# yuxiaoxiangyong/Multilateral-Temporal-view-Pyramid-Transformer-for-Video-Inpainting-Detection

Hardware: AMD Instinct MI355X
Metric: clips/sec fwd (B=8,T=5,224x224) (higher is better)
Workload: dtype f32; 1 GPU; full Mumpy forward (3 temporal views, pyramid decoder), B=8 clips/GPU, T=5, 224x224, fp32, tubelets (5,4,1); global_batch=8, launch=hipGraph replay, fork/join over HIP streams (independent branches co-scheduled), parallelism=batch-sharded x1, one metric all-reduce

## Files before the change

include/mumpy_hip.h:

```cpp
#ifndef MUMPY_HIP_H
#define MUMPY_HIP_H

#include <stdint.h>

#ifdef __cplusplus
extern "C" {
#endif

#define MUMPY_ABI_VERSION 2

#define MUMPY_EINVAL   (-1)
#define MUMPY_EALIGN   (-2)
#define MUMPY_ENULL    (-3)
#define MUMPY_ERANGE   (-4)

#define MUMPY_ACT_NONE 0
#define MUMPY_ACT_GELU 1
#define MUMPY_MATH_BF16 0x100
#define MUMPY_MATH_BF16X3 0x200
#define MUMPY_MATH_BF16X2 0x400

int         mumpy_abi_version(void);
const char* mumpy_last_error(void);
const char* mumpy_last_route(void);
int         mumpy_tuning_build(void);

int mumpy_workspace_status(const void* workspace, int* status);

int mumpy_linear_rd_fwd(const float* x, const float* W, const float* bias, const float* residual, float* y, int64_t M, int N, int K,
                        int act, void* stream);
int mumpy_window_attention_bg_fwd(const float* qkv, float* out, const float* bias, const float* mask_tab, const int32_t* mask_id,
                                  int n_mask, int B, int Hs, int W, int C, int shift, float scale, void* stream);

int mumpy_linear_ln_tiles(int64_t M, int N, int K);
int mumpy_linear_lnx_fwd(const float* x, const float* W, const float* bias, const float* residual, float* y, int64_t M, int N, int K,
                         int act, void* workspace, int64_t workspace_bytes, float* stats_out, const float* ln_stats, int ln_gn,
                         const float* ln_colsum, float ln_eps, void* stream);

int mumpy_deform_sample_kv_fwd(const float* x2, const float* pos, const float* Wkv, const float* bkv, float* kv, int B, int Hs2,
                               int W, int C, int nq, void* stream);

int mumpy_deform_out_combine_fwd(const float* o, const float* Wout, const float* bout, const float* x1, float* out, int B, int H,
                                 int W, int C, void* stream);

int mumpy_deform_sample_kv_mm16_fwd(const float* x2, const float* pos, const float* Wkv, const float* bkv, float* kv, int B, int Hs2,
                                    int W, int C, int nq, void* stream);
int mumpy_deform_out_combine_mm16_fwd(const float* o, const float* Wout, const float* bout, const float* x1, float* out, int B,
                                      int H, int W, int C, void* stream);

int mumpy_avgpool2_pad_nhwc_fwd(const float* x, float* out, int B, int H, int W, int C, int Cpad, int nchw_in, void* stream);

int mumpy_copy_rows_fwd(const float* src, int64_t src_stride, float* dst, int64_t dst_stride, int64_t rows, int cols, void* stream);

int mumpy_merge_views_fwd(const float* v1, const float* v2, const float* v3, float* out, int B, int T, int n, int C1, int C2,
                          int C3, int t1, int t2, int t3, void* stream);

int mumpy_trunk_head_fwd(const float* g, const float* f, const float* gcn, const float* freq, float* z, int B, int h, int w, int C,
                         void* stream);

int mumpy_layernorm_fwd(const float* x, const float* gamma, const float* beta, float* y,
                        int64_t rows, int C, float eps, void* stream);

int mumpy_layernorm_bf16_fwd(const float* x, const float* gamma, const float* beta, void* y,
                             int64_t rows, int C, float eps, void* stream);

int mumpy_linear_fwd(const float* x, const float* W, const float* bias, const float* residual, float* y,
                     int64_t M, int N, int K, int act, void* stream);

int64_t mumpy_linear_workspace_bytes(int64_t M, int N, int K);
int mumpy_linear_ws_fwd(const float* x, const float* W, const float* bias, const float* residual, float* y,
                        int64_t M, int N, int K, int act, void* workspace, int64_t workspace_bytes, void* stream);

int mumpy_linear_wsz_fwd(const float* x, const float* W, const float* bias, const float* residual, float* y,
                         int64_t M, int N, int K, int act, void* workspace, int64_t workspace_bytes, void* stream);

int mumpy_linear_bf16s_fwd(const void* x, const void* W, const float* bias, const float* residual, void* y,
                           int64_t M, int N, int K, int act, int out_bf16, void* stream);

int mumpy_linear_rows_fwd(const float* x, int64_t rows_per_block, int64_t block_stride, const float* W,
                          const float* bias, const float* residual, float* y, int64_t M, int N, int K, int act,
                          void* workspace, int64_t workspace_bytes, void* stream);

int mumpy_linear_rows_kseg_fwd(const float* x, int64_t rows_per_block, int64_t block_stride, int kseg, int kstride, const float* W,
                               const float* bias, const float* residual, float* y, int64_t M, int N, int K, int act,
                               void* workspace, int64_t workspace_bytes, void* stream);

int64_t mumpy_conv2d_workspace_bytes(int B, int H, int W, int Cin, int Cout, int kh, int kw);
int mumpy_conv2d_nhwc_fwd(const float* x, const float* w_krsc, const float* bias, const float* residual, float* y,
                          int B, int H, int W, int Cin, int Cout, int kh, int kw, int act, void* workspace,
                          int64_t workspace_bytes, void* stream);

int mumpy_window_attention_fwd(const float* qkv, float* out, const float* bias, const float* mask_tab,
                               const int32_t* mask_id, int n_mask, int B, int Hs, int W, int C, int shift,
                               float scale, void* stream);

int mumpy_window_attention_bf16_fwd(const void* qkv, void* out, const float* bias, const float* mask_tab,
                                    const int32_t* mask_id, int n_mask, int B, int Hs, int W, int C, int shift,
                                    float scale, void* stream);

int mumpy_window_attention_bf16mm_fwd(const void* qkv, void* out, const float* bias, const float* mask_tab,
                                      const int32_t* mask_id, int n_mask, int B, int Hs, int W, int C, int shift,
                                      float scale, void* stream);

int mumpy_window_attention_mm16_fwd(const float* qkv, float* out, const float* bias, const float* mask_tab,
                                    const int32_t* mask_id, int n_mask, int B, int Hs, int W, int C, int shift,
                                    float scale, void* stream);


int mumpy_deform_offsets_fwd(const float* q, const float* dw_w, const float* dw_b, const float* ln_g,
                             const float* ln_b, const float* pw_w, float* pos, int B, int H, int W, int C,
                             void* stream);

int mumpy_deform_sample_fwd(const float* x2, const float* pos, float* out, int B, int Hs2, int W, int C,
                            int nq, void* stream);

int mumpy_deform_attention_fwd(const float* q, const float* kv, const float* padmask, float* out, int B, int H,
                               int W, int C, int r, float scale, void* stream);

int mumpy_deform_attention_mm16_fwd(const float* q, const float* kv, const float* padmask, float* out, int B, int H,
                                    int W, int C, int r, float scale, void* stream);

int mumpy_deform_combine_fwd(const float* x1, const float* Yt, float* out, int B, int H, int W, int C,
                             void* stream);

int mumpy_faf_fwd(const float* x, const float* D, const float* Dt, float* scratch, float* out, int B, int T,
                  int frame, int lo_hi, int mid_lo, int mid_hi, void* stream);

int mumpy_patch_embed_fwd(const float* x, const float* Wt, const float* bias, const float* gamma,
                          const float* beta, float* out, int B, int T, int H, int W, int t, int C,
                          float eps, void* stream);

int mumpy_patch_merge_ln_fwd(const float* x, const float* gamma, const float* beta, float* out, int B, int Hs,
                             int W, int C, float eps, void* stream);

int mumpy_temporal_attention_fwd(const float* qkv, float* out, int64_t S, int T, int C, int heads,
                                 float scale, void* stream);
int mumpy_temporal_attention_q_fwd(const float* qkv, float* out, int64_t S, int T, int Tq, int C, int heads, float scale, void* stream);

int mumpy_attention_probs_fwd(const float* q, const float* k, float* out, int64_t outer, int heads, int nq, int nk, int d,
                              int64_t q_outer_stride, int64_t q_row_stride, int64_t k_outer_stride, int64_t k_row_stride,
                              int64_t q_mod, float scale, void* stream);

int mumpy_gn_stats_nhwc_fwd(const float* x, float* partial, int B, int64_t HW, int C, int G, int nsplit,
                            void* stream);

int mumpy_gn_apply_resample_nhwc_fwd(const float* x, const float* partial, int nsplit, const float* gamma,
                                     const float* beta, int G, float eps, int act, int mean4, int scale,
                                     int align_corners, int ep_mode, const float* ep_a, const float* ep_b,
                                     float* out, int out_ctot, int out_coff, int B, int H, int W, int C,
                                     void* stream);

int mumpy_final_conv_fwd(const float* x, const float* w_krsc, const float* bias, float* logits, uint8_t* mask, int B,
                         int H, int W, int C, float thr, void* stream);

int64_t mumpy_final_conv_bwd_workspace_bytes(int B, int H, int W);
int mumpy_final_conv_bwd(const float* x, const float* w_krsc, const float* dy, float* dx, float* dw, float* db, void* workspace,
                         int64_t workspace_bytes, int B, int H, int W, int C, void* stream);

int mumpy_sigmoid_threshold_fwd(const float* logits, uint8_t* mask, int64_t n, float thr, void* stream);

int mumpy_normalize_u8_fwd(const uint8_t* frames, float* out, int64_t nframes, int H, int W, const float* mean3,
                           const float* std3, void* stream);

int mumpy_resize_nearest_table(int src, int dst, int32_t* table_host);
int mumpy_resize_normalize_u8_fwd(const uint8_t* frames, float* out, const int32_t* ytab, const int32_t* xtab,
                                  int64_t nframes, int Hs, int Ws, int H, int W, const float* mean3, const float* std3,
                                  void* stream);

int mumpy_add_fwd(const float* a, const float* b, float* out, int64_t n, void* stream);

int64_t mumpy_mask_loss_workspace_bytes(int B, int64_t P);
int mumpy_mask_loss_fwd_bwd(const float* logits, const float* target, float* dlogits, float* loss3, void* workspace,
                            int64_t workspace_bytes, int B, int64_t P, float eps, float loss_scale, void* stream);

int mumpy_adamw_step(float* param, const float* grad, float* exp_avg, float* exp_avg_sq, int64_t n, double lr,
                     double beta1, double beta2, double eps, double weight_decay, int step, double grad_scale,
                     void* stream);

int mumpy_adamw_hyper(float* out8_host, double lr, double beta1, double beta2, double eps, double weight_decay, int step,
                      double grad_scale);
int mumpy_adamw_step_dev(float* param, const float* grad, float* exp_avg, float* exp_avg_sq, int64_t n,
                         const float* hyper_dev, void* stream);

int mumpy_sgd_step(float* param, const float* grad, float* momentum_buf, int64_t n, double lr, double momentum,
                   double dampening, double weight_decay, int nesterov, double grad_scale, void* stream);
int mumpy_sgd_hyper(float* out4_host, double lr, double momentum, double dampening, double weight_decay, int nesterov,
                    double grad_scale);
int mumpy_sgd_step_dev(float* param, const float* grad, float* momentum_buf, int64_t n, const float* hyper_dev, int nesterov,
                       void* stream);

int mumpy_rmsprop_step(float* param, const float* grad, float* square_avg, float* momentum_buf, int64_t n, double lr,
                       double alpha, double eps, double weight_decay, double momentum, double grad_scale, void* stream);
int mumpy_rmsprop_hyper(float* out8_host, double lr, double alpha, double eps, double weight_decay, double momentum,
                        double grad_scale);
int mumpy_rmsprop_step_dev(float* param, const float* grad, float* square_avg, float* momentum_buf, int64_t n,
                           const float* hyper_dev, void* stream);

int64_t mumpy_layernorm_bwd_workspace_bytes(int64_t rows, int C);
int mumpy_layernorm_bwd(const float* x, const float* gamma, const float* dy, const float* dx_add, float* dx, float* dgamma,
                        float* dbeta, void* workspace, int64_t workspace_bytes, int64_t rows, int C, float eps, int accumulate,
                        void* stream);

int mumpy_gelu_fwd(const float* x, float* y, int64_t n, void* stream);
int mumpy_gelu_bwd(const float* x, const float* dy, float* dx, int64_t n, void* stream);

int mumpy_transpose_fwd(const float* in, float* out, int64_t R, int64_t C, void* stream);

int64_t mumpy_col_sum_workspace_bytes(int64_t R, int C);
int mumpy_col_sum_fwd(const float* x, float* out, void* workspace, int64_t workspace_bytes, int64_t R, int C, void* stream);

int64_t mumpy_linear_bwd_workspace_bytes(int64_t M, int N, int K);
int mumpy_linear_bwd(const float* x, const float* W, const float* dy, float* dx, float* dW, float* db, int64_t M, int N, int K,
                     int accumulate, void* workspace, int64_t workspace_bytes, void* stream);

int mumpy_patch_gather_fwd(const float* in, float* out, int64_t B, int H, int W, int C, int inverse, void* stream);

int mumpy_conv_weight_dgrad_fwd(const float* w_krsc, float* out, int Cout, int Cin, int kh, int kw, void* stream);

int64_t mumpy_conv2d_wgrad_workspace_bytes(int B, int H, int W, int Cin, int Cout, int kh, int kw);
int mumpy_conv2d_wgrad_nhwc(const float* x, const float* dy, float* dW, int B, int H, int W, int Cin, int Cout, int kh, int kw,
                            int accumulate, void* workspace, int64_t workspace_bytes, void* stream);

int64_t mumpy_window_attention_bwd_workspace_bytes(int B, int Hs, int W, int C);
int mumpy_window_attention_bwd(const float* qkv, const float* dout, const float* bias, const float* mask_tab,
                               const int32_t* mask_id, int n_mask, const int32_t* rel_index, float* dqkv, float* dtable,
                               void* workspace, int64_t workspace_bytes, int B, int Hs, int W, int C, int shift, float scale,
                               int accumulate, void* stream);
int mumpy_window_attention_bwd_csr(const float* qkv, const float* dout, const float* bias, const float* mask_tab,
                                   const int32_t* mask_id, int n_mask, const int32_t* rel_index, const int32_t* rel_csr, float* dqkv,
                                   float* dtable, void* workspace, int64_t workspace_bytes, int B, int Hs, int W, int C, int shift,
                                   float scale, int accumulate, void* stream);
int64_t mumpy_window_attention_mm16_bwd_workspace_bytes(int B, int Hs, int W, int C);
int mumpy_window_attention_mm16_bwd(const float* qkv, const float* dout, const float* bias, const float* mask_tab,
                                    const int32_t* mask_id, int n_mask, const int32_t* rel_index, const int32_t* rel_csr, float* dqkv,
                                    float* dtable, void* workspace, int64_t workspace_bytes, int B, int Hs, int W, int C, int shift,
                                    float scale, int accumulate, void* stream);

int mumpy_relpos_bias_expand_fwd(const float* table, const int32_t* rel_index, float* out, int nH, void* stream);

#define MUMPY_GN_ACCUMULATE 0x100
int64_t mumpy_gn_bwd_workspace_bytes(int B, int64_t HW, int C);
int mumpy_gn_bwd_nhwc(const float* z, const float* stats_partial, int nsplit_stats, const float* gamma, const float* beta,
                      const float* dy, float* dz, float* dgamma, float* dbeta, void* workspace, int64_t workspace_bytes,
                      int B, int64_t HW, int C, int G, float eps, int relu, void* stream);

int mumpy_temporal_attention_bwd(const float* qkv, const float* dout, float* dqkv, int64_t S, int T, int C, int heads,
                                 float scale, void* stream);

int mumpy_scale_samples_fwd(const float* x, const float* scale, float* out, int B, int64_t per_sample, void* stream);

int mumpy_upsample_bwd_nhwc(const float* dy, float* dx, int B, int H, int W, int C, int scale, int align_corners, void* stream);

int mumpy_dwconv5_window_fwd(const float* x, const float* w, const float* b, float* u, int64_t N, int C, void* stream);
int64_t mumpy_dwconv5_window_bwd_workspace_bytes(int64_t N, int C);
int mumpy_dwconv5_window_bwd(const float* x, const float* w, const float* du, float* dx, float* dw, float* db,
                             void* workspace, int64_t workspace_bytes, int64_t N, int C, void* stream);

int64_t mumpy_deform_attention_bwd_workspace_bytes(int64_t B2w, int C);
int mumpy_deform_attention_bwd(const float* q, const float* kv, const float* dout, float* dq_part, float* dkv, void* workspace,
                               int64_t workspace_bytes, int64_t B1w, int r, int C, float scale, void* stream);

int mumpy_deform_sample_bwd(const float* x2, const float* pos, const float* dsampled, float* dx2, float* dpos_part,
                            int64_t B2, int C, int nq, void* stream);

#ifdef __cplusplus
}
#endif
#endif
```

multilateral-temporal-view-pyramid-transformer-for-video-inpainting-detection_amd/csrc/abi.cpp:

```cpp
#include <stdarg.h>
#include <stdio.h>
#include "common.h"

namespace mumpy {
static thread_local char g_err[512] = "";
void set_error(const char* fmt, ...) {
    va_list ap;
    va_start(ap, fmt);
    vsnprintf(g_err, sizeof(g_err), fmt, ap);
    va_end(ap);
}
thread_local Route g_route;
static thread_local char g_route_text[160] = "";
static const char* format_route() {
    static const char* const addr[] = {"dense", "rows", "kseg", "conv"};
    static const char* const ln[] = {"none", "producer", "consumer"};
    static const char* const red[] = {"none", "one", "two-in-one", "taps"};
    const Route& r = g_route;
    char* t = g_route_text;
    const size_t n = sizeof(g_route_text);
    switch (r.family) {
    case Route::TILED: snprintf(t, n, "tiled tile=%d ks=%d np=%d addr=%s", r.tile, r.ks, r.np, addr[r.addr & 3]); break;
    case Route::TILED16: snprintf(t, n, "tiled16 tile=%d ks=%d np=%d addr=%s", r.tile, r.ks, r.np, addr[r.addr & 3]); break;
    case Route::WS:
        snprintf(t, n, "ws sched=%s P=%d ln=%s addr=%s", r.split ? "split" : "whole", r.passes, ln[r.ln < 3 ? r.ln : 0], addr[r.addr & 3]);
        break;
    case Route::WS64: snprintf(t, n, "ws64 P=%d addr=dense", r.passes); break;
    case Route::WS16: snprintf(t, n, "ws16 P=%d addr=dense", r.passes); break;
    case Route::XGEMM: {
        char dx[24] = "-", dw[24] = "-";
        if (r.prod[0].wt) snprintf(dx, sizeof(dx), "%dx%d", r.prod[0].wt, r.prod[0].ks);
        if (r.prod[1].wt) snprintf(dw, sizeof(dw), "%dx%d", r.prod[1].wt, r.prod[1].ks);
        snprintf(t, n, "xgemm np=%d addr=%s dx=%s dw=%s reduce=%s", r.np, addr[r.addr & 3], dx, dw, red[r.reduce & 3]);
        break;
    }
    default: snprintf(t, n, "none");
    }
    return t;
}
#ifdef MUMPY_TUNING
#include <stdlib.h>
int tune_int(const char* name, int dflt) {
    const char* v = getenv(name);
    return v ? atoi(v) : dflt;
}
const char* tune_str(const char* name) { return getenv(name); }
#endif
}

extern "C" int mumpy_tuning_build(void) {
#ifdef MUMPY_TUNING
    return 1;
#else
    return 0;
#endif
}

extern "C" int mumpy_abi_version(void) { return MUMPY_ABI_VERSION; }
extern "C" const char* mumpy_last_error(void) { return mumpy::g_err; }
extern "C" const char* mumpy_last_route(void) { return mumpy::format_route(); }
```

multilateral-temporal-view-pyramid-transformer-for-video-inpainting-detection_amd/csrc/common.h:

```cpp
#pragma once
#include <hip/hip_runtime.h>
#include <stdint.h>
#include <stdio.h>
#include "../../include/mumpy_hip.h"

namespace mumpy {

typedef float f32x4 __attribute__((ext_vector_type(4)));
typedef float f32x16 __attribute__((ext_vector_type(16)));

constexpr int WAVE = 64;
constexpr int WS = 7;
constexpr int WT = 49;
constexpr int HD = 32;

void set_error(const char* fmt, ...);

#ifdef MUMPY_TUNING
int tune_int(const char* name, int dflt);
const char* tune_str(const char* name);
#else
inline int tune_int(const char*, int dflt) { return dflt; }
inline const char* tune_str(const char*) { return nullptr; }
#endif

struct Route {
    enum Family : uint8_t { NONE, TILED, TILED16, WS, WS64, WS16, XGEMM };
    enum Addr : uint8_t { DENSE, ROWS, KSEG, CONV };
    enum Reduce : uint8_t { R_NONE, R_ONE, R_TWO_IN_ONE, R_TAPS };
    uint8_t family = NONE;
    uint8_t tile = 0;
    uint8_t np = 0;
    uint8_t addr = DENSE;
    uint8_t split = 0;
    uint8_t passes = 0;
    uint8_t ln = 0;
    uint8_t reduce = R_NONE;
    int ks = 1;
    struct { int wt, ks; } prod[2] = {{0, 0}, {0, 0}};
};
extern thread_local Route g_route;

inline hipStream_t as_stream(void* s) { return reinterpret_cast<hipStream_t>(s); }
inline bool aligned16(const void* p) { return (reinterpret_cast<uintptr_t>(p) & 15u) == 0; }

#define MUMPY_CHECK_LAUNCH(name)                                                     \
    do {                                                                             \
        hipError_t e_ = hipGetLastError();                                           \
        if (e_ != hipSuccess) {                                                      \
            mumpy::set_error("%s: launch failed: %s", name, hipGetErrorString(e_));  \
            return (int)e_;                                                          \
        }                                                                            \
    } while (0)

#define MUMPY_REQUIRE(cond, code, ...)                                               \
    do {                                                                             \
        if (!(cond)) {                                                               \
            mumpy::set_error(__VA_ARGS__);                                           \
            return code;                                                             \
        }                                                                            \
    } while (0)

__device__ __forceinline__ unsigned xcd_major_id(unsigned orig, unsigned nwg) {
    const unsigned xcd = orig & 7, q8 = nwg >> 3, r8 = nwg & 7;
    return (xcd < r8 ? xcd * (q8 + 1) : r8 * (q8 + 1) + (xcd - r8) * q8) + (orig >> 3);
}

template <int CTRL>
__device__ __forceinline__ float dpp_f(float v) {
    return __builtin_bit_cast(float, __builtin_amdgcn_update_dpp(0, __builtin_bit_cast(int, v), CTRL, 0xF, 0xF, true));
}
__device__ __forceinline__ float swz_xor16(float v) {
    return __builtin_bit_cast(float, __builtin_amdgcn_ds_swizzle(__builtin_bit_cast(int, v), (16 << 10) | 0x1f));
}

__device__ __forceinline__ float wave_sum(float v, int width) {
    if (width > 1) v += dpp_f<0xB1>(v);
    if (width > 2) v += dpp_f<0x4E>(v);
    if (width > 4) v += dpp_f<0x141>(v);
    if (width > 8) v += dpp_f<0x140>(v);
    if (width > 16) v += swz_xor16(v);
    if (width > 32) v += __shfl_xor(v, 32);
    return v;
}

template <typename T>
__device__ __forceinline__ T ordered_sum(T first, const T* __restrict__ p, int64_t stride, int n_more) {
    T s = first;
    int z = 0;
    for (; z + 8 <= n_more; z += 8) {
        T v[8];
#pragma unroll
        for (int u = 0; u < 8; ++u) v[u] = p[(int64_t)(z + u) * stride];
#pragma unroll
        for (int u = 0; u < 8; ++u) s += v[u];
    }
    for (; z < n_more; ++z) s += p[(int64_t)z * stride];
    return s;
}

__device__ __forceinline__ void gn_block_stats(const float* __restrict__ stats, int nsplit, int G, int b, int64_t HW, int cg, float eps,
                                               float* gm, float* gr, double (*red)[2]) {
    const int tid = threadIdx.x, nslice = 256 / G, g = tid % G, k = tid / G;
    const int64_t per = (HW + nsplit - 1) / nsplit;
    const float* base = stats + (int64_t)b * nsplit * G * 2 + g * 2;
    const double piv = (double)base[0] / (double)((per < HW ? per : HW) * cg);
    double s = 0.0, q = 0.0;
    if (k < nslice)
        for (int sp = k; sp < nsplit; sp += nslice) {
            const int64_t p0 = sp * per, cnt = ((p0 + per < HW) ? p0 + per : HW) - p0;
            if (cnt <= 0) continue;
            const float* o = base + (int64_t)sp * G * 2;
            const double ni = (double)(cnt * cg), dm = (double)o[0] / ni - piv;
            s += ni * dm; q += (double)o[1] + ni * dm * dm;
        }
    red[tid][0] = s; red[tid][1] = q;
    __syncthreads();
    if (tid < G) {
        double ss = 0.0, qq = 0.0;
        for (int j = 0; j < nslice; ++j) { ss += red[j * G + tid][0]; qq += red[j * G + tid][1]; }
        const double n = (double)HW * (double)cg, dm = ss / n;
        double var = qq / n - dm * dm;
        if (var < 0.0) var = 0.0;
        gm[tid] = (float)(piv + dm);
        gr[tid] = (float)(1.0 / sqrt(var + (double)eps));
    }
    __syncthreads();
}

__device__ __forceinline__ float erf_fast(float x) {
    const float ax = fabsf(x);
    const float t = __builtin_amdgcn_rcpf(fmaf(0.3275911f, ax, 1.0f));
    float p = fmaf(1.061405429f, t, -1.453152027f);
    p = fmaf(p, t, 1.421413741f);
    p = fmaf(p, t, -0.284496736f);
    p = fmaf(p, t, 0.254829592f);
    const float y = 1.0f - p * t * __expf(-ax * ax);
    return copysignf(y, x);
}

__device__ __forceinline__ float gelu_erf(float x) { return 0.5f * x * (1.0f + erf_fast(x * 0.70710678118654752440f)); }

__device__ __forceinline__ int window_token(int wy, int wx, int p, int Hs, int W, int shift) {
    int py = p / WS, px = p - py * WS;
    int y = wy * WS + py + shift;
    int x = wx * WS + px + shift;
    if (y >= Hs) y -= Hs;
    if (x >= W) x -= W;
    return y * W + x;
}

}
```

multilateral-temporal-view-pyramid-transformer-for-video-inpainting-detection_amd/csrc/gemm.hip:

```cpp
#include <stdlib.h>
#include <type_traits>
#include "common.h"
#include "gemm_ws.h"
#include "gemm_ws64.h"
using namespace mumpy;

namespace {

constexpr int BK = 32;
constexpr int LDR = 36;

struct ConvGeom {
    int H, W, Cin, kh, kw, ph, pw;
    int kseg, kstride;
};

__device__ __attribute__((aligned(128))) float g_zero_page[32];

template <int BM, int BN>
__device__ __forceinline__ void tile_of_block(int64_t M, unsigned gn, int ksplit, unsigned& tm, unsigned& tn, int& ks) {
    constexpr unsigned NG = (BN >= 128) ? 4 : 8;
    unsigned wgid = xcd_major_id(blockIdx.x, gridDim.x);
    ks = (int)(wgid % (unsigned)ksplit);
    wgid /= (unsigned)ksplit;
    const unsigned gm = (unsigned)((M + BM - 1) / BM);
    const unsigned full = (gn / NG) * NG;
    if (wgid < gm * full) {
        const unsigned grp = wgid / (gm * NG), rem = wgid - grp * gm * NG;
        tm = rem / NG;
        tn = grp * NG + rem % NG;
    } else {
        const unsigned wdt = gn - full, rem = wgid - gm * full;
        tm = rem / wdt;
        tn = full + rem % wdt;
    }
}

struct ConvTap {
    int dy, dx, off;
    __device__ __forceinline__ bool inside(const ConvGeom& cg, int yx) const {
        const int yy = (yx >> 16) + dy, xx = (yx & 0xffff) + dx;
        return (unsigned)yy < (unsigned)cg.H && (unsigned)xx < (unsigned)cg.W;
    }
};
__device__ __forceinline__ ConvTap conv_tap(const ConvGeom& cg, int k0) {
    const int tap = k0 / cg.Cin, c0 = k0 - tap * cg.Cin;
    const int dy = tap / cg.kw - cg.ph, dx = tap % cg.kw - cg.pw;
    return {dy, dx, (dy * cg.W + dx) * cg.Cin + c0};
}

template <int TM, int TN, int WM, int WN, bool OUT16 = false>
__device__ __forceinline__ void store_tile(const f32x16 (&acc)[TM][TN], int64_t m0, int n0, int wm, int wn, int c, int h,
                                           int64_t M, int N, const float* __restrict__ bias, const float* residual,
                                           float* Y, int act, int ksplit, int ks, float* slab) {
    const int wm_u = __builtin_amdgcn_readfirstlane(wm), wn_u = __builtin_amdgcn_readfirstlane(wn);
    const int64_t mw = m0 + wm_u * WM;
    const int64_t wbase = mw * N + n0 + wn_u * WN;
    const int rows_left = (int)((M - mw) < (int64_t)WM ? (M - mw) : (int64_t)WM);
    const uint32_t nb = 4u * (uint32_t)N;
    const uint32_t lane_off = 4u * h * nb + 4u * c;
    if (ksplit > 1) {
        char* S = reinterpret_cast<char*>(slab + (int64_t)ks * M * N + wbase);
#pragma unroll
        for (int j = 0; j < TN; ++j) {
            if (n0 + wn_u * WN + 32 * j + c >= N) continue;
#pragma unroll
            for (int i = 0; i < TM; ++i)
#pragma unroll
                for (int r = 0; r < 16; ++r) {
                    const int row = 32 * i + (r & 3) + 8 * (r >> 2);
                    if (row + 4 * h < rows_left) *reinterpret_cast<float*>(S + ((uint32_t)row * nb + lane_off + 128u * j)) = acc[i][j][r];
                }
        }
        return;
    }
    char* Yw = OUT16 ? reinterpret_cast<char*>(reinterpret_cast<__bf16*>(Y) + wbase) : reinterpret_cast<char*>(Y + wbase);
    const char* Rw = residual ? reinterpret_cast<const char*>(residual + wbase) : nullptr;
#pragma unroll
    for (int j = 0; j < TN; ++j) {
        const int n = n0 + wn_u * WN + 32 * j + c;
        if (n >= N) continue;
        const float bv = bias ? bias[n] : 0.f;
#pragma unroll
        for (int i = 0; i < TM; ++i)
#pragma unroll
            for (int r = 0; r < 16; ++r) {
                const int row = 32 * i + (r & 3) + 8 * (r >> 2);
                if (row + 4 * h >= rows_left) continue;
                const uint32_t off = (uint32_t)row * nb + lane_off + 128u * j;
                float v = acc[i][j][r] + bv;
                if (act == MUMPY_ACT_GELU) v = gelu_erf(v);
                if (Rw) v += *reinterpret_cast<const float*>(Rw + off);
                if (OUT16) *reinterpret_cast<__bf16*>(Yw + (off >> 1)) = (__bf16)v;
                else *reinterpret_cast<float*>(Yw + off) = v;
            }
    }
}

template <int BM, int BN, int WM, int WN, bool CONV, bool GLDS, bool PIPE = true>
__global__ __launch_bounds__(64 * (BM / WM) * (BN / WN), (BM * BN > 64 * 64) ? 2 : (CONV ? 3 : 4)) void linear_kernel(const float* __restrict__ X, const float* __restrict__ Wt,
                                                     const float* __restrict__ bias, const float* residual,
                                                     float* Y, int64_t M, int N, int K, int act, unsigned gn,
                                                     int ksplit, float* slab, int64_t rpb, int64_t bstride, ConvGeom cg) {
    constexpr int TM = WM / 32, TN = WN / 32;
    constexpr int WAVES_N = BN / WN;
    constexpr int NT = 64 * (BM / WM) * (BN / WN);
    constexpr int RPI = NT / 8;
    constexpr int A_LD = BM / RPI;
    constexpr int B_LD = BN / RPI;
    static_assert(BM % RPI == 0 && BN % RPI == 0, "tile rows must divide over the staging passes");
    constexpr int LD = GLDS ? 32 : LDR;
    __shared__ __attribute__((aligned(1024))) float lds[2][(BM + BN) * LD];

    const int tid = threadIdx.x, lane = tid & 63, wave = tid >> 6;
    const int c = lane & 31, h = lane >> 5;
    const int wm = wave / WAVES_N, wn = wave % WAVES_N;
    unsigned tm, tn;
    int ks;
    tile_of_block<BM, BN>(M, gn, ksplit, tm, tn, ks);
    const int64_t m0 = (int64_t)tm * BM;
    const int n0 = (int)tn * BN;
    const int kbeg = ks * (K / ksplit);

    const int ld_row = tid >> 3, ld_c4 = tid & 7;
    f32x4 areg[A_LD], breg[B_LD];

    const float* arow[A_LD];
    const float* brow[B_LD];
    int ayx[A_LD];
#pragma unroll
    for (int i = 0; i < A_LD; ++i) {
        int64_t m = m0 + ld_row + RPI * i;
        if (m > M - 1) m = M - 1;
        if (CONV) {
            const unsigned mu = (unsigned)m, qx = mu / (unsigned)cg.W;
            const int x = (int)(mu - qx * (unsigned)cg.W);
            const int y = (int)(qx % (unsigned)cg.H);
            ayx[i] = (y << 16) | x;
            arow[i] = X + m * cg.Cin + 4 * ld_c4;
        } else {
            ayx[i] = 0;
            if (rpb >= M && !cg.kseg) arow[i] = X + m * K + 4 * ld_c4;
            else {
                const unsigned mu = (unsigned)m, blk = mu / (unsigned)rpb;
                arow[i] = X + (int64_t)blk * bstride + (int64_t)(mu - blk * (unsigned)rpb) * (cg.kseg ? cg.kseg : K) + 4 * ld_c4;
            }
        }
    }
#pragma unroll
    for (int i = 0; i < B_LD; ++i) {
        int n = n0 + ld_row + RPI * i;
        if (n > N - 1) n = N - 1;
        brow[i] = Wt + (int64_t)n * K + 4 * ld_c4;
    }
    int asw[A_LD], bsw[B_LD];
#pragma unroll
    for (int i = 0; i < A_LD; ++i) asw[i] = 4 * ((ld_c4 ^ (((ld_row + RPI * i) >> 1) & 7)) - ld_c4);
#pragma unroll
    for (int i = 0; i < B_LD; ++i) bsw[i] = 4 * ((ld_c4 ^ (((ld_row + RPI * i) >> 1) & 7)) - ld_c4);
    typedef __attribute__((address_space(1))) const void* gptr_t;
    typedef __attribute__((address_space(3))) void* lptr_t;
    auto gdma = [&](int k0, int buf) {
        const int wave_row = (tid >> 6) * 8;
        if (CONV) {
            const int tap = k0 / cg.Cin, c0 = k0 - tap * cg.Cin;
            const int dy = tap / cg.kw - cg.ph, dx = tap % cg.kw - cg.pw;
            const int off = (dy * cg.W + dx) * cg.Cin + c0;
#pragma unroll
            for (int i = 0; i < A_LD; ++i) {
                const int yy = (ayx[i] >> 16) + dy, xx = (ayx[i] & 0xffff) + dx;
                const bool ok = (unsigned)yy < (unsigned)cg.H && (unsigned)xx < (unsigned)cg.W;
                const float* src = ok ? arow[i] + off + asw[i] : g_zero_page + 4 * ld_c4;
                __builtin_amdgcn_global_load_lds((gptr_t)src, (lptr_t)&lds[buf][(wave_row + RPI * i) * LD], 16, 0, 0);
            }
        } else {
            const int ka = cg.kseg ? (k0 / cg.kseg) * cg.kstride + k0 % cg.kseg : k0;
#pragma unroll
            for (int i = 0; i < A_LD; ++i)
                __builtin_amdgcn_global_load_lds((gptr_t)(arow[i] + ka + asw[i]), (lptr_t)&lds[buf][(wave_row + RPI * i) * LD], 16, 0, 0);
        }
#pragma unroll
        for (int i = 0; i < B_LD; ++i)
            __builtin_amdgcn_global_load_lds((gptr_t)(brow[i] + k0 + bsw[i]), (lptr_t)&lds[buf][(BM + wave_row + RPI * i) * LD], 16, 0, 0);
    };
    auto gload = [&](int k0) {
        if (CONV) {
            const ConvTap t = conv_tap(cg, k0);
#pragma unroll
            for (int i = 0; i < A_LD; ++i) {
                const bool ok = t.inside(cg, ayx[i]);
                const f32x4 v = *reinterpret_cast<const f32x4*>(arow[i] + (ok ? t.off : 0));
                areg[i] = ok ? v : f32x4{0, 0, 0, 0};
            }
        } else {
            const int ka = cg.kseg ? (k0 / cg.kseg) * cg.kstride + k0 % cg.kseg : k0;
#pragma unroll
            for (int i = 0; i < A_LD; ++i) areg[i] = *reinterpret_cast<const f32x4*>(arow[i] + ka);
        }
#pragma unroll
        for (int i = 0; i < B_LD; ++i) breg[i] = *reinterpret_cast<const f32x4*>(brow[i] + k0);
    };
    auto lstore = [&](int buf) {
#pragma unroll
        for (int i = 0; i < A_LD; ++i)
            *reinterpret_cast<f32x4*>(&lds[buf][(ld_row + RPI * i) * LD + 4 * ld_c4]) = areg[i];
#pragma unroll
        for (int i = 0; i < B_LD; ++i)
            *reinterpret_cast<f32x4*>(&lds[buf][(BM + ld_row + RPI * i) * LD + 4 * ld_c4]) = breg[i];
    };
    auto fread = [&](int buf, f32x4 (&af)[TM][4], f32x4 (&bf)[TN][4]) {
#pragma unroll
        for (int i = 0; i < TM; ++i) {
            const int R = wm * WM + 32 * i + c;
#pragma unroll
            for (int q = 0; q < 4; ++q) {
                const int col = GLDS ? 4 * ((4 * h + q) ^ ((R >> 1) & 7)) : 16 * h + 4 * q;
                af[i][q] = *reinterpret_cast<const f32x4*>(&lds[buf][R * LD + col]);
            }
        }
#pragma unroll
        for (int j = 0; j < TN; ++j) {
            const int R = wn * WN + 32 * j + c;
#pragma unroll
            for (int q = 0; q < 4; ++q) {
                const int col = GLDS ? 4 * ((4 * h + q) ^ ((R >> 1) & 7)) : 16 * h + 4 * q;
                bf[j][q] = *reinterpret_cast<const f32x4*>(&lds[buf][(BM + R) * LD + col]);
            }
        }
    };

    f32x16 acc[TM][TN];
#pragma unroll
    for (int i = 0; i < TM; ++i)
#pragma unroll
        for (int j = 0; j < TN; ++j)
#pragma unroll
            for (int r = 0; r < 16; ++r) acc[i][j][r] = 0.f;
    auto mma = [&](const f32x4 (&af)[TM][4], const f32x4 (&bf)[TN][4]) {
#pragma unroll
        for (int s = 0; s < 16; ++s)
#pragma unroll
            for (int i = 0; i < TM; ++i)
#pragma unroll
                for (int j = 0; j < TN; ++j)
                    acc[i][j] = __builtin_amdgcn_mfma_f32_32x32x2f32(af[i][s >> 2][s & 3], bf[j][s >> 2][s & 3], acc[i][j], 0, 0, 0);
    };

    const int nk = K / ksplit / BK;
    f32x4 afA[TM][4], bfA[TN][4];
    if (GLDS && !PIPE) {
        gdma(kbeg, 0);
        if (nk > 1) gdma(kbeg + BK, 1);
        for (int kc = 0; kc < nk; ++kc) {
            __syncthreads();
            fread(kc & 1, afA, bfA);
            __syncthreads();
            if (kc + 2 < nk) gdma(kbeg + (kc + 2) * BK, kc & 1);
            mma(afA, bfA);
        }
    } else if (GLDS) {
        f32x4 afB[TM][4], bfB[TN][4];
        gdma(kbeg, 0);
        if (nk > 1) gdma(kbeg + BK, 1);
        __syncthreads();
        fread(0, afA, bfA);
        __syncthreads();
        if (nk > 2) gdma(kbeg + 2 * BK, 0);
        int kc = 0;
        for (; kc + 1 < nk; kc += 2) {
            fread(1, afB, bfB);
            mma(afA, bfA);
            __syncthreads();
            if (kc + 3 < nk) gdma(kbeg + (kc + 3) * BK, 1);
            if (kc + 2 < nk) fread(0, afA, bfA);
            mma(afB, bfB);
            __syncthreads();
            if (kc + 4 < nk) gdma(kbeg + (kc + 4) * BK, 0);
        }
        if (kc < nk) mma(afA, bfA);
    } else {
    f32x4 afB[TM][4], bfB[TN][4];
    gload(kbeg);
    lstore(0);
    if (nk > 1) gload(kbeg + BK);
    __syncthreads();
    fread(0, afA, bfA);
    if (nk > 1) lstore(1);
    if (nk > 2) gload(kbeg + 2 * BK);
    __syncthreads();
    int kc = 0;
    for (; kc + 1 < nk; kc += 2) {
        fread(1, afB, bfB);
        mma(afA, bfA);
        if (kc + 2 < nk) lstore(0);
        if (kc + 3 < nk) gload(kbeg + (kc + 3) * BK);
        __syncthreads();
        if (kc + 2 < nk) fread(0, afA, bfA);
        mma(afB, bfB);
        if (kc + 3 < nk) lstore(1);
        if (kc + 4 < nk) gload(kbeg + (kc + 4) * BK);
        __syncthreads();
    }
    if (kc < nk) mma(afA, bfA);
    }
    store_tile<TM, TN, WM, WN>(acc, m0, n0, wm, wn, c, h, M, N, bias, residual, Y, act, ksplit, ks, slab);
}

typedef __bf16 bf16x8 __attribute__((ext_vector_type(8)));
typedef __bf16 bf16x2 __attribute__((ext_vector_type(2)));
typedef float f32x2 __attribute__((ext_vector_type(2)));
constexpr int LDH = 20;

template <int BM, int BN, int WM, int WN, bool CONV, int NP = 1, int NBUF = 2, bool IN16 = false, bool OUT16 = false>
__global__ __launch_bounds__(256, 2) void linear_bf16_kernel(const float* __restrict__ X, const float* __restrict__ Wt,
                                                            const float* __restrict__ bias, const float* residual,
                                                            float* Y, int64_t M, int N, int K, int act, unsigned gn,
                                                            int ksplit, float* slab, int64_t rpb, int64_t bstride,
                                                            ConvGeom cg) {
    constexpr int TM = WM / 32, TN = WN / 32;
    constexpr int WAVES_N = BN / WN;
    static_assert((BM / WM) * (BN / WN) == 4, "4 waves per block");
    constexpr int RPI = 32, A_LD = BM / RPI, B_LD = BN / RPI;
    constexpr int PL = (BM + BN) * LDH;
    static_assert(NBUF * NP * PL * 4 <= 65536, "LDS tile exceeds the static limit");
    __shared__ __attribute__((aligned(16))) uint32_t lds[NBUF][NP * PL];
    const int tid = threadIdx.x, lane = tid & 63, wave = tid >> 6;
    const int c = lane & 31, h = lane >> 5;
    const int wm = wave / WAVES_N, wn = wave % WAVES_N;
    unsigned tm, tn;
    int ks;
    tile_of_block<BM, BN>(M, gn, ksplit, tm, tn, ks);
    const int64_t m0 = (int64_t)tm * BM;
    const int n0 = (int)tn * BN;
    const int kbeg = ks * (K / ksplit);
    const int ld_row = tid >> 3, ld_c4 = tid & 7;
    static_assert(!(IN16 || OUT16) || (NP == 1 && !CONV), "bf16 storage: plain bf16 products on dense operands only");
    f32x4 areg[A_LD], breg[B_LD];
    uint2 areg16[IN16 ? A_LD : 1], breg16[IN16 ? B_LD : 1];
    const float* arow[A_LD];
    const float* brow[B_LD];
    int ayx[A_LD];
#pragma unroll
    for (int i = 0; i < A_LD; ++i) {
        int64_t m = m0 + ld_row + RPI * i;
        if (m > M - 1) m = M - 1;
        if (IN16) {
            ayx[i] = 0;
            arow[i] = reinterpret_cast<const float*>(reinterpret_cast<const __bf16*>(X) + m * K + 4 * ld_c4);
            continue;
        }
        if (CONV) {
            const unsigned mu = (unsigned)m, qx = mu / (unsigned)cg.W;
            ayx[i] = ((int)(qx % (unsigned)cg.H) << 16) | (int)(mu - qx * (unsigned)cg.W);
            arow[i] = X + m * cg.Cin + 4 * ld_c4;
        } else {
            ayx[i] = 0;
            if (rpb >= M && !cg.kseg) arow[i] = X + m * K + 4 * ld_c4;
            else {
                const unsigned mu = (unsigned)m, blk = mu / (unsigned)rpb;
                arow[i] = X + (int64_t)blk * bstride + (int64_t)(mu - blk * (unsigned)rpb) * (cg.kseg ? cg.kseg : K) + 4 * ld_c4;
            }
        }
    }
#pragma unroll
    for (int i = 0; i < B_LD; ++i) {
        int n = n0 + ld_row + RPI * i;
        if (n > N - 1) n = N - 1;
        if (IN16) brow[i] = reinterpret_cast<const float*>(reinterpret_cast<const __bf16*>(Wt) + (int64_t)n * K + 4 * ld_c4);
        else brow[i] = Wt + (int64_t)n * K + 4 * ld_c4;
    }
    auto gload = [&](int k0) {
        if (IN16) {
#pragma unroll
            for (int i = 0; i < A_LD; ++i) areg16[i] = *reinterpret_cast<const uint2*>(reinterpret_cast<const __bf16*>(arow[i]) + k0);
#pragma unroll
            for (int i = 0; i < B_LD; ++i) breg16[i] = *reinterpret_cast<const uint2*>(reinterpret_cast<const __bf16*>(brow[i]) + k0);
            return;
        }
        if (CONV) {
            const ConvTap t = conv_tap(cg, k0);
#pragma unroll
            for (int i = 0; i < A_LD; ++i) {
                const bool ok = t.inside(cg, ayx[i]);
                const f32x4 v = *reinterpret_cast<const f32x4*>(arow[i] + (ok ? t.off : 0));
                areg[i] = ok ? v : f32x4{0, 0, 0, 0};
            }
        } else {
            const int ka = cg.kseg ? (k0 / cg.kseg) * cg.kstride + k0 % cg.kseg : k0;
#pragma unroll
            for (int i = 0; i < A_LD; ++i) areg[i] = *reinterpret_cast<const f32x4*>(arow[i] + ka);
        }
#pragma unroll
        for (int i = 0; i < B_LD; ++i) breg[i] = *reinterpret_cast<const f32x4*>(brow[i] + k0);
    };
    auto lstore_row = [&](uint32_t* dst, f32x4 r) {
#pragma unroll
        for (int p = 0; p < NP; ++p) {
            const bf16x2 lo = __builtin_convertvector(f32x2{r.x, r.y}, bf16x2), hi = __builtin_convertvector(f32x2{r.z, r.w}, bf16x2);
            const uint2 u = {*reinterpret_cast<const uint32_t*>(&lo), *reinterpret_cast<const uint32_t*>(&hi)};
            *reinterpret_cast<uint2*>(dst + p * PL) = u;
            if (p + 1 < NP)
                r -= f32x4{__uint_as_float(u.x << 16), __uint_as_float(u.x & 0xffff0000u), __uint_as_float(u.y << 16),
                           __uint_as_float(u.y & 0xffff0000u)};
        }
    };
    auto lstore = [&](int buf) {
        if (IN16) {
#pragma unroll
            for (int i = 0; i < A_LD; ++i) *reinterpret_cast<uint2*>(&lds[buf][(ld_row + RPI * i) * LDH + 2 * ld_c4]) = areg16[i];
#pragma unroll
            for (int i = 0; i < B_LD; ++i) *reinterpret_cast<uint2*>(&lds[buf][(BM + ld_row + RPI * i) * LDH + 2 * ld_c4]) = breg16[i];
            return;
        }
#pragma unroll
        for (int i = 0; i < A_LD; ++i) lstore_row(&lds[buf][(ld_row + RPI * i) * LDH + 2 * ld_c4], areg[i]);
#pragma unroll
        for (int i = 0; i < B_LD; ++i) lstore_row(&lds[buf][(BM + ld_row + RPI * i) * LDH + 2 * ld_c4], breg[i]);
    };
    f32x16 acc[TM][TN];
#pragma unroll
    for (int i = 0; i < TM; ++i)
#pragma unroll
        for (int j = 0; j < TN; ++j)
#pragma unroll
            for (int r = 0; r < 16; ++r) acc[i][j][r] = 0.f;
    constexpr int NPROD = (NP == 3) ? 6 : (NP == 2) ? 3 : 1;
    constexpr int PA[6] = {NP == 3 ? 2 : 1, 0, NP == 3 ? 1 : 0, 1, 0, 0}, PB[6] = {0, NP == 3 ? 2 : 1, NP == 3 ? 1 : 0, 0, 1, 0};
    const int nk = K / ksplit / BK;
    bf16x8 af[TM][2][NP], bf[TN][2][NP];
    auto fread = [&](int buf) {
#pragma unroll
        for (int i = 0; i < TM; ++i)
#pragma unroll
            for (int st = 0; st < 2; ++st)
#pragma unroll
                for (int p = 0; p < NP; ++p)
                    af[i][st][p] = *reinterpret_cast<const bf16x8*>(&lds[buf][p * PL + (wm * WM + 32 * i + c) * LDH + 8 * st + 4 * h]);
#pragma unroll
        for (int j = 0; j < TN; ++j)
#pragma unroll
            for (int st = 0; st < 2; ++st)
#pragma unroll
                for (int p = 0; p < NP; ++p)
                    bf[j][st][p] = *reinterpret_cast<const bf16x8*>(&lds[buf][p * PL + (BM + wn * WN + 32 * j + c) * LDH + 8 * st + 4 * h]);
    };
    auto mma = [&]() {
#pragma unroll
        for (int st = 0; st < 2; ++st)
#pragma unroll
            for (int q = 0; q < NPROD; ++q)
#pragma unroll
                for (int i = 0; i < TM; ++i)
#pragma unroll
                    for (int j = 0; j < TN; ++j)
                        acc[i][j] = __builtin_amdgcn_mfma_f32_32x32x16_bf16(af[i][st][NP > 1 ? PA[q] : 0],
                                                                            bf[j][st][NP > 1 ? PB[q] : 0], acc[i][j], 0, 0, 0);
    };
    const int klast = kbeg + (nk - 1) * BK;
    if (NBUF == 2) {
        gload(kbeg);
        lstore(0);
        __syncthreads();
        for (int kc = 0; kc + 1 < nk; ++kc) {
            gload(kbeg + (kc + 1) * BK);
            __builtin_amdgcn_sched_barrier(0);
            fread(kc & 1);
            mma();
            lstore((kc & 1) ^ 1);
            __syncthreads();
        }
        fread((nk - 1) & 1);
        mma();
    } else {
        gload(kbeg);
        lstore(0);
        gload(nk > 1 ? kbeg + BK : kbeg);
        __syncthreads();
        for (int kc = 0; kc + 1 < nk; ++kc) {
            fread(0);
            __syncthreads();
            lstore(0);
            const int knext = kbeg + (kc + 2) * BK;
            gload(knext < klast ? knext : klast);
            mma();
            __syncthreads();
        }
        fread(0);
        mma();
    }
    store_tile<TM, TN, WM, WN, OUT16>(acc, m0, n0, wm, wn, c, h, M, N, bias, residual, Y, act, ksplit, ks, slab);
}

__global__ __launch_bounds__(256) void splitk_reduce_kernel(const float* __restrict__ slab, const float* __restrict__ bias,
                                                            const float* residual, float* Y, int64_t MN4, int N,
                                                            int ksplit, int act) {
    for (int64_t i = (int64_t)blockIdx.x * 256 + threadIdx.x; i < MN4; i += (int64_t)gridDim.x * 256) {
        f32x4 v = ordered_sum(reinterpret_cast<const f32x4*>(slab)[i], reinterpret_cast<const f32x4*>(slab) + MN4 + i, MN4, ksplit - 1);
        const int n = (int)((i * 4) % N);
        if (bias) v += *reinterpret_cast<const f32x4*>(bias + n);
        if (act == MUMPY_ACT_GELU) {
#pragma unroll
            for (int e = 0; e < 4; ++e) v[e] = gelu_erf(v[e]);
        }
        if (residual) v += reinterpret_cast<const f32x4*>(residual)[i];
        reinterpret_cast<f32x4*>(Y)[i] = v;
    }
}

struct Plan {
    int tile;
    int ksplit;
    unsigned gn;
    int64_t gm;
};

constexpr int NUM_CU = 256;

int fit_ksplit(int K, int want, int min_slice, int max_ks) {
    int ks = want;
    if (ks > K / min_slice) ks = K / min_slice;
    if (ks > max_ks) ks = max_ks;
    while (ks > 1 && (K % (32 * ks)) != 0) --ks;
    return ks < 1 ? 1 : ks;
}

Plan make_plan_x3(int64_t M, int N, int K, bool allow_split) {
    Plan p;
    const int64_t gm128 = (M + 127) / 128, gm64 = (M + 63) / 64;
    const unsigned gn128 = (N + 127) / 128, gn64 = (N + 63) / 64;
    const int64_t b128 = gm128 * gn128, b64 = gm64 * gn64;
    auto fit = [&](int want) { return allow_split ? fit_ksplit(K, want, 384, 16) : 1; };
    const int ksw = fit((int)((448 + b128 / 2) / b128));
    if (b128 * ksw >= 240) {
        p.tile = 0; p.ksplit = ksw; p.gm = gm128; p.gn = gn128;
    } else {
        p.tile = 2; p.ksplit = (b64 < 2 * 256 && K >= 768) ? fit((int)((3 * 256 + b64 - 1) / b64)) : 1;
        p.gm = gm64; p.gn = gn64;
    }
    return p;
}

Plan make_plan(int64_t M, int N, int K, bool allow_split, bool x3 = false) {
    static const char* force = tune_str("MUMPY_GEMM_FORCE");
    if (x3 && !force) return make_plan_x3(M, N, K, allow_split);
    Plan p;
    const int64_t gm128 = (M + 127) / 128, gm64 = (M + 63) / 64;
    const unsigned gn128 = (N + 127) / 128, gn64 = (N + 63) / 64;
    const int64_t b128 = gm128 * gn128, b64 = gm64 * gn64;
    const double nk = (double)K / BK;
    const double t128 = (double)((b128 + NUM_CU - 1) / NUM_CU) * (nk + 2.0) / nk;
    double t64 = (double)((b64 + NUM_CU - 1) / NUM_CU) * 0.272;
    if (t64 < 0.357) t64 = 0.357;
    t64 *= (nk + 0.5) / nk;
    int tile = (t128 <= t64) ? 0 : 2;
    if (tile == 0 && b128 > NUM_CU && K >= 512) tile = 3;
    int ks = 1;
    static const int min_slice = tune_int("MUMPY_GEMM_MINSLICE", 384), max_ks = tune_int("MUMPY_GEMM_MAXKS", 16),
                     min_k = tune_int("MUMPY_GEMM_SPLIT_MINK", 768);
    if (tile == 2 && allow_split && b64 < 2 * NUM_CU && K >= min_k) ks = fit_ksplit(K, (int)((3 * NUM_CU + b64 - 1) / b64), min_slice, max_ks);
    if (force) {
        int ft = -1, fk = -1;
        if (sscanf(force, "%d,%d", &ft, &fk) >= 1 && ft >= 0 && ft <= 3) {
            tile = ft;
            if (fk >= 1 && allow_split && K % (32 * fk) == 0) ks = fk; else if (fk >= 1) ks = 1;
        }
    }
    p.tile = tile; p.ksplit = ks;
    p.gm = (tile == 0 || tile == 3) ? gm128 : gm64;
    p.gn = (tile == 2) ? gn64 : gn128;
    return p;
}

int device_cus() {
    static int num_cu = 0;
    if (!num_cu) {
        int dev = 0;
        hipDeviceProp_t prop;
        if (hipGetDevice(&dev) == hipSuccess && hipGetDeviceProperties(&prop, dev) == hipSuccess) num_cu = prop.multiProcessorCount;
        else num_cu = NUM_CU;
    }
    return num_cu;
}

int ws_plan(int64_t M, int N, int K, bool have_ws, bool conv) {
    static const int ws_mode = tune_int("MUMPY_GEMM_WS", 2);
    const int num_cu = device_cus();
    const int64_t tiles = ((M + 127) / 128) * ((N + 127) / 128);
    const int nk = K / 32;
    const double rounds = (double)tiles / num_cu, eff = rounds / (double)((tiles + num_cu - 1) / num_cu);
    const double per_cu = (double)tiles * nk / num_cu;
    int how = 0;
    if (ws_mode == 1) how = 1;
    else if (ws_mode == 3) how = have_ws ? 2 : 1;
    else if (ws_mode == 2 && conv) {
        if (have_ws && eff < 0.86 && per_cu >= 24.0 && (double)nk / per_cu <= 3.0) how = 2;
        else if (tiles >= (int64_t)(0.75 * num_cu) && eff >= 0.75 && K >= 128) how = 1;
    } else if (ws_mode == 2) {
        if (tiles >= (int64_t)(0.75 * num_cu) && eff >= 0.86 && K >= 128 && !(K >= 1024 && rounds >= 1.8)) how = 1;
        else if (have_ws && eff < 0.86 && per_cu >= 24.0 && (double)nk / per_cu <= 3.0 && !(K >= 1024 && rounds >= 1.8)) how = 2;
    }
    return how;
}

struct LinearArgs {
    const float *x, *W, *bias, *residual;
    float* y;
    int64_t M;
    int N, K, act;
    hipStream_t s;
    float* ws = nullptr;
    int64_t ws_bytes = 0;
    bool ws_clean = false;
    int64_t rpb = 0, bstride = 0;
    int kseg = 0, kstride = 0;
    const ConvGeom* conv = nullptr;
    const gemm_ws::LnArgs* ln = nullptr;
};

struct TiledArgs {
    const float *x, *W, *bias, *residual;
    float* y;
    int64_t M;
    int N, K, act;
    unsigned gn;
    int ksplit;
    float* slab;
    int64_t rpb, bstride;
    ConvGeom cg;
    int64_t grid;
    hipStream_t s;
};

template <class Kern>
void launch_tiled(Kern kern, unsigned threads, const TiledArgs& t) {
    hipLaunchKernelGGL(kern, dim3((unsigned)t.grid), dim3(threads), 0, t.s, t.x, t.W, t.bias, t.residual, t.y, t.M, t.N, t.K, t.act,
                       t.gn, t.ksplit, t.slab, t.rpb, t.bstride, t.cg);
}

template <class F>
void with_bool(bool b, F&& f) {
    if (b) f(std::true_type{});
    else f(std::false_type{});
}

void launch_tiled_fp32(int tile, bool conv, bool glds, const TiledArgs& t) {
    with_bool(conv, [&](auto cv) {
        constexpr bool CV = decltype(cv)::value;
        if (tile == 3) return launch_tiled(linear_kernel<128, 128, 64, 64, CV, true, false>, 256, t);
        with_bool(glds, [&](auto gl) {
            constexpr bool GL = decltype(gl)::value;
            if (tile == 0) launch_tiled(linear_kernel<128, 128, 64, 32, CV, GL>, 512, t);
            else if (tile == 1) launch_tiled(linear_kernel<64, 128, 32, 64, CV, GL>, 256, t);
            else launch_tiled(linear_kernel<64, 64, 32, 32, CV, GL>, 256, t);
        });
    });
}

template <int NP, bool IN16 = false>
void launch_tiled_bf16(bool wide, bool flag, const TiledArgs& t) {
    with_bool(wide, [&](auto wd) {
        with_bool(flag, [&](auto fl) {
            constexpr int T = decltype(wd)::value ? 128 : 64, NBUF = (T == 128 && NP > 1) ? 1 : 2;
            constexpr bool FL = decltype(fl)::value;
            launch_tiled(linear_bf16_kernel<T, T, T / 2, T / 2, !IN16 && FL, NP, NBUF, IN16, IN16 && FL>, 256, t);
        });
    });
}

int launch_linear(const LinearArgs& a) {
    const int64_t M = a.M, rpb = a.rpb > 0 ? a.rpb : M, bstride = a.rpb > 0 ? a.bstride : 0;
    const int N = a.N, K = a.K, act = a.act & 0xff;
    const ConvGeom* conv = a.conv;
    ConvGeom cg = conv ? *conv : ConvGeom{0, 0, 0, 0, 0, 0, 0, 0, 0};
    cg.kseg = a.kseg; cg.kstride = a.kstride;
    const bool math_bf16 = (a.act & MUMPY_MATH_BF16) != 0;
    const bool math_x2 = (a.act & MUMPY_MATH_BF16X2) != 0;
    const bool math_x3 = (a.act & MUMPY_MATH_BF16X3) != 0 || math_x2;
    float* ws = a.ws;
    int64_t ws_bytes = a.ws_bytes;
    const gemm_ws::Conv cvd{cg.H, cg.W, cg.Cin, cg.kh, cg.kw};
    if (a.ln && (rpb < M || math_bf16 || math_x3 || conv || !gemm_ws::eligible(M, N, K) ||
                 !ws_plan(M, N, K, ws && ws_bytes >= gemm_ws::workspace_bytes(device_cus()), false))) {
        set_error("linear: LayerNorm folding needs a shape the persistent 128x128 kernel takes (mumpy_linear_ln_tiles) in fp32 mode");
        return MUMPY_EINVAL;
    }
    if (rpb >= M && !a.kseg && !math_bf16 && !math_x3 && (conv ? gemm_ws::conv_eligible(M, N, cvd) : gemm_ws::eligible(M, N, K))) {
        const int num_cu = device_cus();
        const bool have_ws = ws && ws_bytes >= gemm_ws::workspace_bytes(num_cu);
        const int how = ws_plan(M, N, K, have_ws, conv != nullptr);
        const int nk = K / 32;
        static const int ws64_mode = tune_int("MUMPY_GEMM_WS64", 1);
        if (!how && !conv && ws64_mode) {
            const int64_t t64 = ((M + 63) / 64) * ((N + 63) / 64);
            const double r64 = (double)t64 / (2.0 * num_cu);
            const bool fits = ws64_mode == 2 || (act != MUMPY_ACT_GELU && nk <= 32 && t64 >= 64 && (r64 <= 1.0 || r64 >= 2.5 || nk <= 12));
            if (fits) {
                if (int rc = gemm_ws64::launch(a.x, a.W, a.bias, a.residual, a.y, M, N, K, act, num_cu, a.s)) return rc;
                MUMPY_CHECK_LAUNCH("linear(ws64)");
                return 0;
            }
        }
        if (how) {
            if (int rc = gemm_ws::launch(a.x, a.W, a.bias, a.residual, a.y, M, N, K, act, num_cu, a.s, ws, ws_bytes, how == 2 ? 1 : 0, nullptr,
                                         a.ws_clean, conv ? &cvd : nullptr, a.ln)) return rc;
            MUMPY_CHECK_LAUNCH("linear(ws)");
            return 0;
        }
    }
    Plan p = make_plan(M, N, K, ws != nullptr, math_x3);
    if (ws) { ws += 1024; ws_bytes -= 4096; }
    if (p.ksplit > 1 && (int64_t)p.ksplit * M * N * (int64_t)sizeof(float) > ws_bytes) p.ksplit = 1;
    if (math_bf16 || math_x3) {
        if (p.tile == 3) p.tile = 0;
        if (p.tile == 1) { p.tile = 2; p.gn = (unsigned)((N + 63) / 64); }
    }
    const int64_t grid = p.gm * p.gn * p.ksplit;
    MUMPY_REQUIRE(grid < (1ll << 31), MUMPY_ERANGE, "linear: too many tiles");
    static const bool use_glds = tune_int("MUMPY_GEMM_GLDS", 0) != 0;
    const bool wide = (p.tile == 0 || p.tile == 3);
    const TiledArgs t{a.x, a.W, a.bias, a.residual, a.y, M, N, K, act, p.gn, p.ksplit, ws, rpb, bstride, cg, grid, a.s};
    g_route = Route{};
    g_route.family = Route::TILED; g_route.tile = (uint8_t)p.tile; g_route.ks = p.ksplit;
    g_route.np = math_x2 ? 2 : math_x3 ? 3 : math_bf16 ? 1 : 0;
    g_route.addr = conv ? Route::CONV : a.kseg ? Route::KSEG : rpb < M ? Route::ROWS : Route::DENSE;
    if (math_x2) launch_tiled_bf16<2>(wide, conv != nullptr, t);
    else if (math_x3) launch_tiled_bf16<3>(wide, conv != nullptr, t);
    else if (math_bf16) launch_tiled_bf16<1>(wide, conv != nullptr, t);
    else launch_tiled_fp32(p.tile, conv != nullptr, use_glds, t);
    MUMPY_CHECK_LAUNCH("linear");
    if (p.ksplit > 1) {
        const int64_t mn4 = M * N / 4;
        int64_t g = (mn4 + 255) / 256;
        if (g > 2048) g = 2048;
        hipLaunchKernelGGL(splitk_reduce_kernel, dim3((unsigned)g), dim3(256), 0, a.s, ws, a.bias, a.residual, a.y, mn4, N,
                           p.ksplit, act);
        MUMPY_CHECK_LAUNCH("linear(split-K reduce)");
    }
    return 0;
}

}

static int check_linear_args(const char* who, const void* x, const void* W, const float* residual, const void* y, int64_t M, int N,
                             int K, int act) {
    MUMPY_REQUIRE(x && W && y, MUMPY_ENULL, "%s: null pointer", who);
    MUMPY_REQUIRE(aligned16(x) && aligned16(W) && aligned16(y) && aligned16(residual), MUMPY_EALIGN,
                  "%s: pointers must be 16-byte aligned", who);
    MUMPY_REQUIRE(M < (1ll << 31) - 256 && (int64_t)N * 4 * 128 < (1ll << 32), MUMPY_ERANGE,
                  "%s: M=%lld rows / N=%d columns beyond the 32-bit row index / tile byte offsets", who, (long long)M, N);
    MUMPY_REQUIRE(M >= 0 && N > 0 && K > 0 && K % BK == 0 && N % 32 == 0, MUMPY_EINVAL,
                  "%s: need K %% 32 == 0 and N %% 32 == 0 (got M=%lld N=%d K=%d)", who, (long long)M, N, K);
    MUMPY_REQUIRE((act & 0xff) == MUMPY_ACT_NONE || (act & 0xff) == MUMPY_ACT_GELU, MUMPY_EINVAL, "%s: unknown act %d", who, act);
    constexpr int math_bits = MUMPY_MATH_BF16 | MUMPY_MATH_BF16X3 | MUMPY_MATH_BF16X2;
    MUMPY_REQUIRE((act & ~(0xff | math_bits)) == 0, MUMPY_EINVAL, "%s: unknown flag bits in act 0x%x", who, act);
    MUMPY_REQUIRE(((act & math_bits) & ((act & math_bits) - 1)) == 0, MUMPY_EINVAL, "%s: the MUMPY_MATH_* modes are exclusive", who);
    return 0;
}

static LinearArgs linear_args(const float* x, const float* W, const float* bias, const float* residual, float* y, int64_t M, int N,
                              int K, int act, void* workspace, int64_t workspace_bytes, void* stream) {
    LinearArgs a{x, W, bias, residual, y, M, N, K, act, as_stream(stream)};
    a.ws = static_cast<float*>(workspace);
    a.ws_bytes = workspace ? workspace_bytes : 0;
    return a;
}

extern "C" int mumpy_linear_fwd(const float* x, const float* W, const float* bias, const float* residual, float* y,
                                int64_t M, int N, int K, int act, void* stream) {
    if (M == 0) return 0;
    if (int rc = check_linear_args("linear", x, W, residual, y, M, N, K, act)) return rc;
    return launch_linear(linear_args(x, W, bias, residual, y, M, N, K, act, nullptr, 0, stream));
}

extern "C" int64_t mumpy_linear_workspace_bytes(int64_t M, int N, int K) {
    if (M <= 0 || N <= 0 || K <= 0 || K % BK) return 0;
    const Plan p = make_plan(M, N, K, true), q = make_plan(M, N, K, true, true);
    const int ks = p.ksplit > q.ksplit ? p.ksplit : q.ksplit;
    int64_t bytes = ks > 1 ? (int64_t)ks * M * N * (int64_t)sizeof(float) + 4096 : 0;
    if (gemm_ws::eligible(M, N, K)) {
        const int64_t tiles = ((M + 127) / 128) * ((N + 127) / 128);
        const double per_cu = (double)tiles * (K / 32) / NUM_CU;
        const int64_t need = gemm_ws::workspace_bytes(2 * NUM_CU);
        if (per_cu >= 16.0 && bytes < need) bytes = need;
    }
    return bytes;
}

extern "C" int mumpy_linear_ws_fwd(const float* x, const float* W, const float* bias, const float* residual, float* y,
                                   int64_t M, int N, int K, int act, void* workspace, int64_t workspace_bytes,
                                   void* stream) {
    if (M == 0) return 0;
    if (int rc = check_linear_args("linear", x, W, residual, y, M, N, K, act)) return rc;
    MUMPY_REQUIRE(aligned16(workspace), MUMPY_EALIGN, "linear: workspace must be 16-byte aligned");
    return launch_linear(linear_args(x, W, bias, residual, y, M, N, K, act, workspace, workspace_bytes, stream));
}

extern "C" int mumpy_linear_bf16s_fwd(const void* x, const void* W, const float* bias, const float* residual, void* y,
                                      int64_t M, int N, int K, int act, int out_bf16, void* stream) {
    if (M == 0) return 0;
    if (int rc = check_linear_args("linear_bf16s", x, W, residual, y, M, N, K, act)) return rc;
    MUMPY_REQUIRE((act & ~0xff) == 0, MUMPY_EINVAL, "linear_bf16s: unknown act %d", act);
    MUMPY_REQUIRE(!(out_bf16 && residual), MUMPY_EINVAL, "linear_bf16s: a bf16 output takes no residual");
    hipStream_t s = as_stream(stream);
    static const int ws16 = tune_int("MUMPY_GEMM_WS16", 2);
    const int64_t gm128 = (M + 127) / 128, gm64 = (M + 63) / 64;
    const unsigned gn128 = (N + 127) / 128, gn64 = (N + 63) / 64;
    if (ws16 && gemm_ws::eligible16(M, N, K)) {
        const int num_cu = device_cus();
        const int64_t tiles = gm128 * gn128;
        const double rounds = (double)tiles / num_cu, eff = rounds / (double)((tiles + num_cu - 1) / num_cu);
        if (ws16 == 2 || (tiles >= (int64_t)(0.75 * num_cu) && eff >= 0.75)) {
            if (int rc = gemm_ws::launch16(x, W, bias, residual, y, M, N, K, act, out_bf16 != 0, num_cu, s)) return rc;
            MUMPY_CHECK_LAUNCH("linear_bf16s(ws)");
            return 0;
        }
    }
    const bool wide = gm128 * gn128 >= 200;
    const unsigned gn = wide ? gn128 : gn64;
    const int64_t grid = (wide ? gm128 : gm64) * gn;
    MUMPY_REQUIRE(grid < (1ll << 31), MUMPY_ERANGE, "linear_bf16s: too many tiles");
    const TiledArgs t{static_cast<const float*>(x), static_cast<const float*>(W), bias, residual, static_cast<float*>(y), M, N, K, act,
                      gn, 1, nullptr, M, 0, ConvGeom{0, 0, 0, 0, 0, 0, 0, 0, 0}, grid, s};
    g_route = Route{};
    g_route.family = Route::TILED16; g_route.tile = wide ? 0 : 2; g_route.np = 1;
    launch_tiled_bf16<1, true>(wide, out_bf16 != 0, t);
    MUMPY_CHECK_LAUNCH("linear_bf16s");
    return 0;
}

extern "C" int mumpy_linear_wsz_fwd(const float* x, const float* W, const float* bias, const float* residual, float* y,
                                    int64_t M, int N, int K, int act, void* workspace, int64_t workspace_bytes,
                                    void* stream) {
    if (M == 0) return 0;
    if (int rc = check_linear_args("linear", x, W, residual, y, M, N, K, act)) return rc;
    MUMPY_REQUIRE(aligned16(workspace), MUMPY_EALIGN, "linear: workspace must be 16-byte aligned");
    LinearArgs a = linear_args(x, W, bias, residual, y, M, N, K, act, workspace, workspace_bytes, stream);
    a.ws_clean = true;
    return launch_linear(a);
}

extern "C" int mumpy_workspace_status(const void* workspace, int* status) {
    MUMPY_REQUIRE(workspace && status, MUMPY_ENULL, "workspace_status: null pointer");
    unsigned w[2] = {0, 0};
    static_assert(gemm_ws::LN_GUARD_WORD + 1 == gemm_ws::STATUS_WORD, "status words must be adjacent");
    hipError_t e = hipMemcpy(w, static_cast<const unsigned*>(workspace) + gemm_ws::LN_GUARD_WORD, sizeof(w), hipMemcpyDeviceToHost);
    if (e != hipSuccess) { set_error("workspace_status: %s", hipGetErrorString(e)); return (int)e; }
    *status = w[1] ? (int)w[1] : (w[0] ? -1 : 0);
    return 0;
}

extern "C" int mumpy_linear_ln_tiles(int64_t M, int N, int K) {
    if (M <= 0 || N <= 0 || K <= 0 || K % BK || N % 32 || !gemm_ws::eligible(M, N, K)) return 0;
    return ws_plan(M, N, K, true, false) ? (N + 127) / 128 : 0;
}

extern "C" int mumpy_linear_lnx_fwd(const float* x, const float* W, const float* bias, const float* residual, float* y, int64_t M,
                                    int N, int K, int act, void* workspace, int64_t workspace_bytes, float* stats_out,
                                    const float* ln_stats, int ln_gn, const float* ln_colsum, float ln_eps, void* stream) {
    if (M == 0) return 0;
    if (int rc = check_linear_args("linear", x, W, residual, y, M, N, K, act)) return rc;
    MUMPY_REQUIRE((act & ~0xff) == 0, MUMPY_EINVAL, "linear_lnx: fp32 matrix math only");
    MUMPY_REQUIRE(aligned16(workspace) && workspace, MUMPY_EALIGN, "linear_lnx: needs the kept (zeroed) workspace of mumpy_linear_wsz_fwd");
    MUMPY_REQUIRE((stats_out != nullptr) != (ln_stats != nullptr), MUMPY_EINVAL, "linear_lnx: exactly one of stats_out (producer) / ln_stats (consumer)");
    MUMPY_REQUIRE(!ln_stats || (ln_colsum && bias && !residual && ln_gn == (K + 127) / 128 && ln_gn <= 16 && ln_eps > 0.f), MUMPY_EINVAL,
                  "linear_lnx: the consumer takes W gamma, colsum, bias = W beta + b, no residual, and ln_gn = ceil(K / 128) tiles (got %d)", ln_gn);
    MUMPY_REQUIRE(aligned16(stats_out) && aligned16(ln_stats) && aligned16(ln_colsum), MUMPY_EALIGN, "linear_lnx: pointers must be 16-byte aligned");
    MUMPY_REQUIRE(M * (int64_t)((N + 127) / 128) * 8 < (1ll << 31) && M * (int64_t)(ln_gn > 0 ? ln_gn : 1) * 8 < (1ll << 31), MUMPY_ERANGE,
                  "linear_lnx: statistics buffer beyond 2 GiB");
    const gemm_ws::LnArgs ln{stats_out, ln_stats, ln_colsum, ln_gn, K, ln_eps};
    LinearArgs a = linear_args(x, W, bias, residual, y, M, N, K, act, workspace, workspace_bytes, stream);
    a.ws_clean = true;
    a.ln = &ln;
    return launch_linear(a);
}

extern "C" int mumpy_linear_rows_fwd(const float* x, int64_t rows_per_block, int64_t block_stride, const float* W,
                                     const float* bias, const float* residual, float* y, int64_t M, int N, int K, int act,
                                     void* workspace, int64_t workspace_bytes, void* stream) {
    if (M == 0) return 0;
    if (int rc = check_linear_args("linear", x, W, residual, y, M, N, K, act)) return rc;
    MUMPY_REQUIRE(rows_per_block > 0 && M % rows_per_block == 0 && block_stride % 4 == 0, MUMPY_EINVAL,
                  "linear_rows: M=%lld must be a multiple of rows_per_block=%lld and block_stride %% 4 == 0",
                  (long long)M, (long long)rows_per_block);
    LinearArgs a = linear_args(x, W, bias, residual, y, M, N, K, act, workspace, workspace_bytes, stream);
    a.rpb = rows_per_block; a.bstride = block_stride;
    return launch_linear(a);
}

extern "C" int mumpy_linear_rows_kseg_fwd(const float* x, int64_t rows_per_block, int64_t block_stride, int kseg, int kstride,
                                          const float* W, const float* bias, const float* residual, float* y, int64_t M, int N, int K,
                                          int act, void* workspace, int64_t workspace_bytes, void* stream) {
    if (M == 0) return 0;
    if (int rc = check_linear_args("linear", x, W, residual, y, M, N, K, act)) return rc;
    MUMPY_REQUIRE(rows_per_block > 0 && M % rows_per_block == 0 && block_stride % 4 == 0, MUMPY_EINVAL,
                  "linear_rows_kseg: M=%lld must be a multiple of rows_per_block=%lld and block_stride %% 4 == 0",
                  (long long)M, (long long)rows_per_block);
    MUMPY_REQUIRE(kseg > 0 && kseg % 32 == 0 && K % kseg == 0 && kstride % 4 == 0 && kstride >= 0, MUMPY_EINVAL,
                  "linear_rows_kseg: need kseg %% 32 == 0, K %% kseg == 0, kstride %% 4 == 0 (got kseg=%d K=%d kstride=%d)", kseg, K, kstride);
    LinearArgs a = linear_args(x, W, bias, residual, y, M, N, K, act, workspace, workspace_bytes, stream);
    a.rpb = rows_per_block; a.bstride = block_stride;
    a.kseg = kseg; a.kstride = kstride;
    return launch_linear(a);
}

extern "C" int64_t mumpy_conv2d_workspace_bytes(int B, int H, int W, int Cin, int Cout, int kh, int kw) {
    return mumpy_linear_workspace_bytes((int64_t)B * H * W, Cout, kh * kw * Cin);
}

extern "C" int mumpy_conv2d_nhwc_fwd(const float* x, const float* w_krsc, const float* bias, const float* residual,
                                     float* y, int B, int H, int W, int Cin, int Cout, int kh, int kw, int act,
                                     void* workspace, int64_t workspace_bytes, void* stream) {
    MUMPY_REQUIRE(B > 0 && H > 0 && W > 0 && H < 32768 && W < 32768, MUMPY_EINVAL, "conv2d: bad image size %dx%d", H, W);
    MUMPY_REQUIRE(kh > 0 && kw > 0 && (kh & 1) && (kw & 1), MUMPY_EINVAL, "conv2d: kernel %dx%d must be odd (same padding)", kh, kw);
    MUMPY_REQUIRE(Cin % 32 == 0 && Cout % 32 == 0, MUMPY_EINVAL, "conv2d: Cin=%d and Cout=%d must be multiples of 32", Cin, Cout);
    const int64_t M = (int64_t)B * H * W;
    const int K = kh * kw * Cin;
    if (int rc = check_linear_args("linear", x, w_krsc, residual, y, M, Cout, K, act)) return rc;
    MUMPY_REQUIRE(aligned16(workspace), MUMPY_EALIGN, "conv2d: workspace must be 16-byte aligned");
    const ConvGeom cg{H, W, Cin, kh, kw, kh / 2, kw / 2, 0, 0};
    LinearArgs a = linear_args(x, w_krsc, bias, residual, y, M, Cout, K, act, workspace, workspace_bytes, stream);
    a.conv = &cg;
    return launch_linear(a);
}
```

multilateral-temporal-view-pyramid-transformer-for-video-inpainting-detection_amd/csrc/norm.hip:

```cpp
#include "common.h"
using namespace mumpy;

namespace {

constexpr int MAXNV = 16;

template <typename SRC, bool OUT16 = false>
__global__ __launch_bounds__(256) void ln_rows_kernel(SRC src, const float* __restrict__ gamma,
                                                      const float* __restrict__ beta, float* __restrict__ y,
                                                      int64_t rows, int C, int lpr, int nv, float eps) {
    const int lane = threadIdx.x & 63;
    const int wave = threadIdx.x >> 6;
    const int rpw = 64 / lpr;
    const int sub = lane / lpr, l = lane % lpr;
    const int64_t row = ((int64_t)blockIdx.x * 4 + wave) * rpw + sub;
    const bool live = row < rows;
    f32x4 v[MAXNV];
    float s = 0.f;
#pragma unroll
    for (int i = 0; i < MAXNV; ++i) {
        if (i < nv) {
            v[i] = live ? *reinterpret_cast<const f32x4*>(src(row, l + i * lpr)) : f32x4{0, 0, 0, 0};
            s += (v[i].x + v[i].y) + (v[i].z + v[i].w);
        }
    }
    s = wave_sum(s, lpr);
    const float mean = s / (float)C;
    float q = 0.f;
#pragma unroll
    for (int i = 0; i < MAXNV; ++i) {
        if (i < nv) {
            f32x4 d = v[i] - mean;
            q += (d.x * d.x + d.y * d.y) + (d.z * d.z + d.w * d.w);
        }
    }
    q = wave_sum(q, lpr);
    const float rstd = rsqrtf(q / (float)C + eps);
    if (!live) return;
    float* yr = y + row * (int64_t)C;
#pragma unroll
    for (int i = 0; i < MAXNV; ++i) {
        if (i < nv) {
            const int c4 = l + i * lpr;
            const f32x4 g = *reinterpret_cast<const f32x4*>(gamma + 4 * c4);
            const f32x4 b = *reinterpret_cast<const f32x4*>(beta + 4 * c4);
            const f32x4 o = (v[i] - mean) * rstd * g + b;
            if (OUT16) {
                typedef __bf16 bf16x4v __attribute__((ext_vector_type(4)));
                *reinterpret_cast<bf16x4v*>(reinterpret_cast<__bf16*>(y) + row * (int64_t)C + 4 * c4) = __builtin_convertvector(o, bf16x4v);
            } else {
                *reinterpret_cast<f32x4*>(yr + 4 * c4) = o;
            }
        }
    }
}

struct PlainRows {
    const float* x;
    int C;
    __device__ const float* operator()(int64_t row, int c4) const { return x + row * (int64_t)C + 4 * c4; }
};

struct MergeRows {
    const float* x;
    int Hs, W, C;
    __device__ const float* operator()(int64_t row, int c4) const {
        const int w2 = W >> 1, h2 = Hs >> 1;
        const int j = (int)(row % w2);
        const int64_t t = row / w2;
        const int i = (int)(t % h2);
        const int64_t b = t / h2;
        const int seg = (4 * c4) / C;
        const int c = 4 * c4 - seg * C;
        const int dy = seg & 1, dx = seg >> 1;
        const int64_t tok = (b * Hs + (2 * i + dy)) * (int64_t)W + (2 * j + dx);
        return x + tok * C + c;
    }
};

bool pick_split(int C, int* lpr, int* nv) {
    if (C % 4 || C > 4096 || C < 4) return false;
    const int n4 = C / 4;
    int l = 64;
    while (l > 1 && ((n4 % l) || n4 / l < 3)) l >>= 1;
    if (n4 / l > MAXNV) return false;
    *lpr = l;
    *nv = n4 / l;
    return true;
}

}

extern "C" int mumpy_layernorm_fwd(const float* x, const float* gamma, const float* beta, float* y, int64_t rows,
                                   int C, float eps, void* stream) {
    if (rows == 0) return 0;
    MUMPY_REQUIRE(x && gamma && beta && y, MUMPY_ENULL, "layernorm: null pointer");
    MUMPY_REQUIRE(aligned16(x) && aligned16(y) && aligned16(gamma) && aligned16(beta), MUMPY_EALIGN,
                  "layernorm: pointers must be 16-byte aligned");
    int lpr, nv;
    MUMPY_REQUIRE(rows >= 0 && pick_split(C, &lpr, &nv), MUMPY_EINVAL, "layernorm: unsupported C=%d", C);
    if (rows == 0) return 0;
    const int rows_per_block = 4 * (64 / lpr);
    const int64_t grid = (rows + rows_per_block - 1) / rows_per_block;
    hipLaunchKernelGGL(ln_rows_kernel<PlainRows>, dim3((unsigned)grid), dim3(256), 0, as_stream(stream),
                       PlainRows{x, C}, gamma, beta, y, rows, C, lpr, nv, eps);
    MUMPY_CHECK_LAUNCH("layernorm");
    return 0;
}

extern "C" int mumpy_layernorm_bf16_fwd(const float* x, const float* gamma, const float* beta, void* y, int64_t rows,
                                        int C, float eps, void* stream) {
    if (rows == 0) return 0;
    MUMPY_REQUIRE(x && gamma && beta && y, MUMPY_ENULL, "layernorm_bf16: null pointer");
    MUMPY_REQUIRE(aligned16(x) && aligned16(y) && aligned16(gamma) && aligned16(beta), MUMPY_EALIGN,
                  "layernorm_bf16: pointers must be 16-byte aligned");
    int lpr, nv;
    MUMPY_REQUIRE(rows >= 0 && pick_split(C, &lpr, &nv), MUMPY_EINVAL, "layernorm_bf16: unsupported C=%d", C);
    const int rows_per_block = 4 * (64 / lpr);
    const int64_t grid = (rows + rows_per_block - 1) / rows_per_block;
    hipLaunchKernelGGL((ln_rows_kernel<PlainRows, true>), dim3((unsigned)grid), dim3(256), 0, as_stream(stream),
                       PlainRows{x, C}, gamma, beta, static_cast<float*>(y), rows, C, lpr, nv, eps);
    MUMPY_CHECK_LAUNCH("layernorm_bf16");
    return 0;
}

extern "C" int mumpy_patch_merge_ln_fwd(const float* x, const float* gamma, const float* beta, float* out, int B,
                                        int Hs, int W, int C, float eps, void* stream) {
    MUMPY_REQUIRE(x && gamma && beta && out, MUMPY_ENULL, "patch_merge_ln: null pointer");
    MUMPY_REQUIRE(aligned16(x) && aligned16(out) && aligned16(gamma) && aligned16(beta), MUMPY_EALIGN,
                  "patch_merge_ln: pointers must be 16-byte aligned");
    MUMPY_REQUIRE(B > 0 && Hs > 0 && W > 0 && (Hs % 2 == 0) && (W % 2 == 0), MUMPY_EINVAL,
                  "patch_merge_ln: grid (%d,%d) must be even (swin:353)", Hs, W);
    int lpr, nv;
    MUMPY_REQUIRE(C % 4 == 0 && pick_split(4 * C, &lpr, &nv), MUMPY_EINVAL, "patch_merge_ln: unsupported C=%d", C);
    const int64_t rows = (int64_t)B * (Hs / 2) * (W / 2);
    const int rows_per_block = 4 * (64 / lpr);
    const int64_t grid = (rows + rows_per_block - 1) / rows_per_block;
    hipLaunchKernelGGL(ln_rows_kernel<MergeRows>, dim3((unsigned)grid), dim3(256), 0, as_stream(stream),
                       MergeRows{x, Hs, W, C}, gamma, beta, out, rows, 4 * C, lpr, nv, eps);
    MUMPY_CHECK_LAUNCH("patch_merge_ln");
    return 0;
}

namespace {
__global__ __launch_bounds__(256) void sigmoid_thr_kernel(const float* __restrict__ z, uint8_t* __restrict__ m,
                                                          int64_t n, float thr) {
    int64_t i = (int64_t)blockIdx.x * blockDim.x + threadIdx.x;
    const int64_t stride = (int64_t)gridDim.x * blockDim.x;
    for (; i < n; i += stride) m[i] = (1.0f / (1.0f + __expf(-z[i])) > thr) ? 1 : 0;
}
}

extern "C" int mumpy_sigmoid_threshold_fwd(const float* logits, uint8_t* mask, int64_t n, float thr, void* stream) {
    MUMPY_REQUIRE(logits && mask, MUMPY_ENULL, "sigmoid_threshold: null pointer");
    MUMPY_REQUIRE(n >= 0, MUMPY_EINVAL, "sigmoid_threshold: n < 0");
    if (n == 0) return 0;
    int64_t grid = (n + 255) / 256;
    if (grid > 2048) grid = 2048;
    hipLaunchKernelGGL(sigmoid_thr_kernel, dim3((unsigned)grid), dim3(256), 0, as_stream(stream), logits, mask, n, thr);
    MUMPY_CHECK_LAUNCH("sigmoid_threshold");
    return 0;
}

namespace {
__global__ __launch_bounds__(256) void normalize_u8_kernel(const uint8_t* __restrict__ src, float* __restrict__ dst,
                                                           int64_t nframes, int64_t HW, float m0, float m1, float m2,
                                                           float s0, float s1, float s2) {
    const int64_t q4 = HW >> 2;
    const int64_t total = nframes * 3 * q4;
    for (int64_t i = (int64_t)blockIdx.x * 256 + threadIdx.x; i < total; i += (int64_t)gridDim.x * 256) {
        const int64_t p4 = i % q4;
        const int64_t t = i / q4;
        const int ch = (int)(t % 3);
        const int64_t f = t / 3;
        const float mean = ch == 0 ? m0 : (ch == 1 ? m1 : m2);
        const float stdv = ch == 0 ? s0 : (ch == 1 ? s1 : s2);
        const uint8_t* s = src + (f * HW + 4 * p4) * 3 + ch;
        f32x4 v;
#pragma unroll
        for (int k = 0; k < 4; ++k) v[k] = ((float)s[3 * k] / 255.0f - mean) / stdv;
        *reinterpret_cast<f32x4*>(dst + (f * 3 + ch) * HW + 4 * p4) = v;
    }
}
}

extern "C" int mumpy_resize_nearest_table(int src, int dst, int32_t* table_host) {
    MUMPY_REQUIRE(table_host, MUMPY_ENULL, "resize_nearest_table: null pointer");
    MUMPY_REQUIRE(src > 0 && dst > 0, MUMPY_EINVAL, "resize_nearest_table: bad sizes %d -> %d", src, dst);
    const double a = (double)src / dst;
    double xo = a * 0.5;
    for (int x = 0; x < dst; ++x) {
        int xin = xo < 0.0 ? -1 : (int)xo;
        if (xin > src - 1) xin = src - 1;
        table_host[x] = xin;
        xo += a;
    }
    return 0;
}

namespace {
__global__ __launch_bounds__(256) void resize_normalize_u8_kernel(const uint8_t* __restrict__ src, float* __restrict__ dst,
                                                                  const int32_t* __restrict__ ytab, const int32_t* __restrict__ xtab,
                                                                  int64_t nframes, int Hs, int Ws, int H, int W, float m0, float m1,
                                                                  float m2, float s0, float s1, float s2) {
    const int q4 = W >> 2;
    const int64_t total = nframes * 3 * H * q4;
    for (int64_t i = (int64_t)blockIdx.x * 256 + threadIdx.x; i < total; i += (int64_t)gridDim.x * 256) {
        const int x4 = (int)(i % q4);
        int64_t t = i / q4;
        const int y = (int)(t % H); t /= H;
        const int ch = (int)(t % 3);
        const int64_t f = t / 3;
        const float mean = ch == 0 ? m0 : (ch == 1 ? m1 : m2);
        const float stdv = ch == 0 ? s0 : (ch == 1 ? s1 : s2);
        const uint8_t* row = src + ((f * Hs + ytab[y]) * (int64_t)Ws) * 3 + ch;
        const int4 xi = *reinterpret_cast<const int4*>(xtab + 4 * x4);
        f32x4 v;
        v[0] = ((float)row[3 * (int64_t)xi.x] / 255.0f - mean) / stdv;
        v[1] = ((float)row[3 * (int64_t)xi.y] / 255.0f - mean) / stdv;
        v[2] = ((float)row[3 * (int64_t)xi.z] / 255.0f - mean) / stdv;
        v[3] = ((float)row[3 * (int64_t)xi.w] / 255.0f - mean) / stdv;
        *reinterpret_cast<f32x4*>(dst + ((f * 3 + ch) * H + y) * (int64_t)W + 4 * x4) = v;
    }
}
}

extern "C" int mumpy_resize_normalize_u8_fwd(const uint8_t* frames, float* out, const int32_t* ytab, const int32_t* xtab,
                                             int64_t nframes, int Hs, int Ws, int H, int W, const float* mean3,
                                             const float* std3, void* stream) {
    MUMPY_REQUIRE(frames && out && mean3 && std3 && ytab && xtab, MUMPY_ENULL, "resize_normalize_u8: null pointer");
    MUMPY_REQUIRE(nframes >= 0 && Hs > 0 && Ws > 0 && H > 0 && W > 0 && W % 4 == 0, MUMPY_EINVAL,
                  "resize_normalize_u8: bad sizes %dx%d -> %dx%d (output width must be a multiple of 4)", Hs, Ws, H, W);
    MUMPY_REQUIRE(aligned16(out) && aligned16(xtab), MUMPY_EALIGN, "resize_normalize_u8: out and xtab must be 16-byte aligned");
    MUMPY_REQUIRE(std3[0] != 0.f && std3[1] != 0.f && std3[2] != 0.f, MUMPY_EINVAL, "resize_normalize_u8: zero std");
    if (nframes == 0) return 0;
    const int64_t total = nframes * 3 * (int64_t)H * (W / 4);
    int64_t grid = (total + 255) / 256;
    if (grid > 4096) grid = 4096;
    hipLaunchKernelGGL(resize_normalize_u8_kernel, dim3((unsigned)grid), dim3(256), 0, as_stream(stream), frames, out, ytab, xtab,
                       nframes, Hs, Ws, H, W, mean3[0], mean3[1], mean3[2], std3[0], std3[1], std3[2]);
    MUMPY_CHECK_LAUNCH("resize_normalize_u8");
    return 0;
}

extern "C" int mumpy_normalize_u8_fwd(const uint8_t* frames, float* out, int64_t nframes, int H, int W, const float* mean3,
                                      const float* std3, void* stream) {
    MUMPY_REQUIRE(frames && out && mean3 && std3, MUMPY_ENULL, "normalize_u8: null pointer");
    MUMPY_REQUIRE(nframes >= 0 && H > 0 && W > 0 && ((int64_t)H * W) % 4 == 0, MUMPY_EINVAL, "normalize_u8: H*W must be a multiple of 4");
    MUMPY_REQUIRE(aligned16(out), MUMPY_EALIGN, "normalize_u8: out must be 16-byte aligned");
    MUMPY_REQUIRE(std3[0] != 0.f && std3[1] != 0.f && std3[2] != 0.f, MUMPY_EINVAL, "normalize_u8: zero std");
    if (nframes == 0) return 0;
    const int64_t total = nframes * 3 * ((int64_t)H * W / 4);
    int64_t grid = (total + 255) / 256;
    if (grid > 4096) grid = 4096;
    hipLaunchKernelGGL(normalize_u8_kernel, dim3((unsigned)grid), dim3(256), 0, as_stream(stream), frames, out, nframes,
                       (int64_t)H * W, mean3[0], mean3[1], mean3[2], std3[0], std3[1], std3[2]);
    MUMPY_CHECK_LAUNCH("normalize_u8");
    return 0;
}
```

multilateral-temporal-view-pyramid-transformer-for-video-inpainting-detection_amd/models/encoder/multiTemporalViewEncoder.py:

```python
import torch
import torch.nn as nn

from models.modules.blocks import Block
from models.modules.dct import FAF
from models.modules.deformableAttention import SwinDAttention
from models.modules.layers import Derived, DropPath, refuse_stochastic_depth, to_2tuple, trunc_normal_
from models.modules.swinTransformer import Mlp, SwinTransformerBlock, ThreeViewPatchMerging, WindowAttention
from mumpy_hip import ops
from mumpy_hip.streams import run_parallel


class CVAModule(nn.Module):
    def __init__(self, dim1, num_heads, window_size=7, temporal_dims=[], qkv_bias=True, qk_scale=None, drop=0.0,
                 attn_drop=0.0, drop_path=0.0, cur_stage=0):
        super().__init__()
        self.crossattn = SwinDAttention(dim1, num_heads, attn_drop, n_groups=3)
        self.drop_path = DropPath(drop_path) if drop_path > 0.0 else nn.Identity()

    def forward(self, x1, x2, mask=None, return_attention=False):
        if return_attention:
            return self.crossattn(x1, x2, return_attention=True)[1]
        y, _ = self.crossattn(x1, x2)
        return ops.add(x1, y), None


class CrossSwinBlock(nn.Module):
    def __init__(self, dim1, dim2, input_resolution, num_heads, window_size=7, shift_size=0, mlp_ratio=4.0, qkv_bias=True,
                 qk_scale=None, drop=0.0, attn_drop=0.0, drop_path=0.0, act_layer=nn.GELU, norm_layer=nn.LayerNorm,
                 fused_window_process=False, last_view=False, temporal_dims=1, cur_stage=0):
        super().__init__()
        if shift_size != 0:
            raise NotImplementedError("cross blocks are always un-shifted (mTVE:310,323,336)")
        self.dim, self.input_resolution, self.num_heads = dim1, tuple(input_resolution), num_heads
        self.window_size = min(window_size, min(self.input_resolution))
        self.shift_size, self.mlp_ratio = 0, mlp_ratio
        self.last_view, self.temporal_dims, self.cur_stage = last_view, temporal_dims, cur_stage
        self.norm1 = norm_layer(dim1)
        self.attn = WindowAttention(dim1, to_2tuple(self.window_size), num_heads, qkv_bias, qk_scale, attn_drop, drop)
        self.drop_path = DropPath(drop_path) if drop_path > 0.0 else nn.Identity()
        self.norm2 = norm_layer(dim1)
        self.mlp = Mlp(dim1, int(dim1 * mlp_ratio), act_layer=act_layer, drop=drop)
        if last_view:
            self.pre, self.cva = nn.Identity(), nn.Identity()
        else:
            self.pre = nn.Linear(dim2, dim1)
            trunc_normal_(self.pre.weight, std=0.02)
            nn.init.zeros_(self.pre.bias)
            self.cva = CVAModule(dim1, num_heads, to_2tuple(self.window_size), temporal_dims, qkv_bias, qk_scale, drop,
                                 attn_drop, drop_path, cur_stage)
        self.register_buffer("attn_mask", None)

    def msa(self, x1, need_out=True):
        h, w = self.input_resolution
        b, l1, c1 = x1.shape
        if self.training:
            refuse_stochastic_depth(self)
        if ops.storage() == "bf16":
            from models.modules.swinTransformer import _w16
            a = self.attn.attend(ops.layernorm_bf16(x1, self.norm1.weight, self.norm1.bias, self.norm1.eps), b, l1 // w, w, 0, None)
            out = ops.linear_bf16s(a, _w16(self.attn, "proj"), self.attn.proj.bias, out_bf16=False)
            return ops.add(x1, out), out
        a = self.attn.attend(ops.layernorm(x1, self.norm1.weight, self.norm1.bias, self.norm1.eps), b, l1 // w, w, 0, None)
        if not need_out:
            return ops.linear(a, self.attn.proj.weight, self.attn.proj.bias, residual=x1), None
        out = ops.linear(a, self.attn.proj.weight, self.attn.proj.bias)
        return ops.add(x1, out), out

    def prep(self, x1):
        if self.last_view:
            return None
        h, w = self.input_resolution
        b, l1, _ = x1.shape
        return self.cva.crossattn._prep(x1, (b, l1 // w, w))

    def tail(self, x1, x2, prep=None):
        h, w = self.input_resolution
        b, l1, c1 = x1.shape
        hs1 = l1 // w
        if not self.last_view:
            hs2 = x2.shape[1] // w
            x2p = ops.linear(x2, self.pre.weight, self.pre.bias)
            x1 = self.cva.crossattn.attend_combine(x1, x2p, b, hs1, w, hs2, prep)
        if ops.storage() == "bf16":
            return self.mlp.forward_bf16(ops.layernorm_bf16(x1, self.norm2.weight, self.norm2.bias, self.norm2.eps), x1)
        m = b * l1
        emit = ops.linear_ln_tiles(m, c1, self.mlp.fc2.in_features) > 0 and ops.linear_ln_tiles(m, 3 * c1, c1) > 0
        return self.mlp(ops.layernorm(x1, self.norm2.weight, self.norm2.bias, self.norm2.eps), residual=x1, emit_stats=emit)

    def forward(self, x1, x2):
        x1, out = self.msa(x1)
        return self.tail(x1, x2), out


class CrossThreeViewSwinBlock(nn.Module):
    def __init__(self, view_configs, input_resolution, cur_stage, mlp_ratio=4.0, qkv_bias=True, qk_scale=None, drop=0.0,
                 attn_drop=0.0, drop_path=0.0, norm_layer=nn.LayerNorm, fused_window_process=False):
        super().__init__()
        kw = dict(shift_size=0, mlp_ratio=mlp_ratio, qkv_bias=qkv_bias, qk_scale=qk_scale, drop=drop, attn_drop=attn_drop,
                  drop_path=drop_path, cur_stage=cur_stage)
        hid = [view_configs[v]["hidden_size"][cur_stage] for v in range(3)]
        heads = [view_configs[v]["num_heads"][cur_stage] for v in range(3)]
        ws = [view_configs[v]["window_size"] for v in range(3)]
        self.block1 = CrossSwinBlock(hid[0], hid[1], input_resolution[0], heads[0], window_size=ws[0],
                                     temporal_dims=view_configs[0]["temporal_ratio"], **kw)
        self.block2 = CrossSwinBlock(hid[1], hid[2], input_resolution[1], heads[1], window_size=ws[1],
                                     temporal_dims=view_configs[0]["temporal_ratio"], **kw)
        self.block3 = CrossSwinBlock(hid[2], hid[2], input_resolution[2], heads[2], window_size=ws[2], last_view=True,
                                     temporal_dims=3, **kw)

    def forward(self, x):
        from mumpy_hip import streams
        if streams.SERIAL:
            x3, out3 = self.block3(x[2], x[2])
            x2, out2 = self.block2(x[1], out3)
            x1, _ = self.block1(x[0], out2)
            return [x1, x2, x3]
        main = torch.cuda.current_stream()
        sa, sb = streams._side_stream(main.device, 0), streams._side_stream(main.device, 1)
        fork, e3, e2 = torch.cuda.Event(), torch.cuda.Event(), torch.cuda.Event()
        fork.record(main)
        streams._DEPTH[0] += 1
        try:
            x3a, out3 = self.block3.msa(x[2])
            e3.record(main)
            sa.wait_event(fork)
            x[1].record_stream(sa)
            with torch.cuda.stream(sa):
                x2a, out2 = self.block2.msa(x[1])
                e2.record(sa)
                prep2 = self.block2.prep(x2a)
                sa.wait_event(e3)
                out3.record_stream(sa)
                x2 = self.block2.tail(x2a, out3, prep2)
            sb.wait_event(fork)
            x[0].record_stream(sb)
            with torch.cuda.stream(sb):
                x1a, _ = self.block1.msa(x[0], need_out=False)
                prep1 = self.block1.prep(x1a)
                sb.wait_event(e2)
                out2.record_stream(sb)
                x1 = self.block1.tail(x1a, out2, prep1)
            x3 = self.block3.tail(x3a, None)
        finally:
            streams._DEPTH[0] -= 1
        main.wait_stream(sa)
        main.wait_stream(sb)
        x2.record_stream(main)
        x1.record_stream(main)
        return [x1, x2, x3]


class OriginalThreeViewSwinBlock(nn.Module):
    def __init__(self, view_configs, input_resolution, cur_stage, cur_lyr, mlp_ratio=4.0, qkv_bias=True, qk_scale=None,
                 drop=0.0, attn_drop=0.0, drop_path=0.0, norm_layer=nn.LayerNorm, fused_window_process=False):
        super().__init__()
        shift = 0 if cur_lyr % 2 == 0 else view_configs[0]["window_size"] // 2
        for v in range(3):
            if cur_lyr < view_configs[v]["depths"][cur_stage]:
                blk = SwinTransformerBlock(view_configs[v]["hidden_size"][cur_stage], input_resolution[v],
                                           view_configs[v]["num_heads"][cur_stage], view_configs[v]["window_size"], shift,
                                           mlp_ratio, qkv_bias, qk_scale, drop, attn_drop, drop_path,
                                           norm_layer=norm_layer, temporal_dim=view_configs[v]["temporal_dim"])
            else:
                blk = nn.Identity()
            setattr(self, f"block{v + 1}", blk)

    def forward(self, x):
        return [self.block1(x[0]), self.block2(x[1]), self.block3(x[2])]


class MultiViewBasicLayer(nn.Module):
    def __init__(self, view_configs, cur_stage, depth, mlp_ratio=4.0, qkv_bias=True, qk_scale=None, drop=0.0,
                 attn_drop=0.0, drop_path=0.0, norm_layer=nn.LayerNorm, downsample=None, fused_window_process=False):
        super().__init__()
        res = [view_configs[k]["input_resolution"][cur_stage] for k in range(3)]
        blocks = []
        for i in range(depth):
            dp = drop_path[i] if isinstance(drop_path, list) else drop_path
            kw = dict(mlp_ratio=mlp_ratio, qkv_bias=qkv_bias, qk_scale=qk_scale, drop=drop, attn_drop=attn_drop,
                      drop_path=dp, norm_layer=norm_layer)
            blocks.append(CrossThreeViewSwinBlock(view_configs, res, cur_stage, **kw) if i == 0 else
                          OriginalThreeViewSwinBlock(view_configs, res, cur_stage, i, **kw))
        self.blocks = nn.ModuleList(blocks)
        self.downsample = downsample(view_configs, cur_stage) if downsample is not None else None

    def _view_chain(self, v, x):
        for blk in self.blocks[1:]:
            x = getattr(blk, f"block{v + 1}")(x)
        out = x
        if self.downsample is not None:
            x = getattr(self.downsample, f"downsample{v + 1}")(x)
        return x, out

    def forward(self, x):
        x = self.blocks[0](x)
        def bg(v):
            from mumpy_hip import streams
            if streams.SERIAL:
                return self._view_chain(v, x[v])
            with ops.background():
                return self._view_chain(v, x[v])
        res = run_parallel([lambda: bg(0), lambda: bg(1), lambda: self._view_chain(2, x[2])], [(x[0],), (x[1],), (x[2],)])
        return [r[0] for r in res], [r[1] for r in res]


class CreateStages(nn.Module):
    def __init__(self, view_configs, depths=[2, 2, 18, 2], mlp_ratio=4.0, qkv_bias=True, qk_scale=None, stages=4,
                 drop_rate=0.0, attn_drop_rate=0.0, drop_path_rate=0.0, norm_layer=nn.LayerNorm, ape=False,
                 patch_norm=True, use_checkpoint=False, fused_window_process=False):
        super().__init__()
        dpr = torch.linspace(0, drop_path_rate, sum(depths)).tolist()
        self.layers = nn.ModuleList([
            MultiViewBasicLayer(view_configs, i, depths[i], mlp_ratio, qkv_bias, qk_scale, drop_rate, attn_drop_rate,
                                dpr[sum(depths[:i]):sum(depths[:i + 1])], norm_layer,
                                ThreeViewPatchMerging if i < stages - 1 else None)
            for i in range(stages)])

    def forward(self, x):
        outs = []
        for layer in self.layers:
            x, o = layer(x)
            outs.append(o)
        return x, outs


class CrossThreeViewTokenize(nn.Module):

    def __init__(self, view_configs):
        super().__init__()
        for v in range(3):
            size = view_configs[v]["patches"].size
            k = (size[-1], size[0], size[1])
            c = view_configs[v]["hidden_size"][0]
            setattr(self, f"project{v + 1}", nn.Conv3d(3, c, kernel_size=k, stride=k, padding=0))
        for v in range(3):
            setattr(self, f"norm{v + 1}", nn.LayerNorm(view_configs[v]["hidden_size"][0]))
        self._wt = [Derived(), Derived(), Derived()]

    def _view(self, v, x):
        proj, norm = getattr(self, f"project{v + 1}"), getattr(self, f"norm{v + 1}")
        w = proj.weight
        if tuple(w.shape[3:]) != (4, 4):
            raise NotImplementedError("tokenizer kernel is built for 4x4 spatial patches")
        wt = self._wt[v].get((w,), lambda: w.reshape(w.shape[0], -1).t().contiguous())
        return ops.patch_embed(x, wt, proj.bias, norm.weight, norm.bias, w.shape[2], norm.eps)

    def forward(self, x):
        return run_parallel([lambda: self._view(0, x), lambda: self._view(1, x), lambda: self._view(2, x)], [(x,), (x,), (x,)])


class CreateGlobalBlocks(nn.Module):
    def __init__(self, global_encoder_config, dpr, dropout_rate):
        super().__init__()
        g = global_encoder_config
        self.blocks = nn.ModuleList([Block(g["hidden_size"], g["num_heads"], g["mlp_dim"], dropout_rate, dpr[i])
                                     for i in range(g["num_layers"])])

    def forward(self, x, keep_t=None):
        last = len(self.blocks) - 1
        for i, blk in enumerate(self.blocks):
            x = blk(x, keep_t=keep_t) if (i == last and keep_t is not None) else blk(x)
        return x


class ThreeViewSwinTransformer(nn.Module):
    def __init__(self, view_configs, input_token_temporal_dims, global_encoder_config, depths=[2, 2, 18, 2], mlp_ratio=4.0,
                 qkv_bias=True, qk_scale=None, stages=4, drop_rate=0.0, attn_drop_rate=0.0, drop_path_rate=0.2,
                 norm_layer=nn.LayerNorm, ape=False, patch_norm=True, use_checkpoint=False, fused_window_process=False):
        super().__init__()
        self.faf = FAF()
        self.tokenize = CrossThreeViewTokenize(view_configs)
        self.input_token_temporal_dims = list(input_token_temporal_dims)
        self.layers = CreateStages(view_configs, depths, mlp_ratio, qkv_bias, qk_scale, stages, drop_rate, attn_drop_rate,
                                   drop_path_rate, norm_layer)
        self.pos_drop = nn.Dropout(p=drop_rate)
        self.globalembedding = nn.Linear(2560, 768)
        self.global_dpr = torch.linspace(0, drop_path_rate, global_encoder_config["num_layers"]).tolist()
        self.globalblocks = CreateGlobalBlocks(global_encoder_config, self.global_dpr, drop_rate)

    def merge_views_along_channel_axis(self, tokens):
        tmax = max(self.input_token_temporal_dims)
        parts = []
        for v, x in enumerate(tokens):
            b, l, c = x.shape
            t = self.input_token_temporal_dims[v]
            x = x.reshape(b, t, l // t, c)
            parts.append(x.expand(b, tmax, l // t, c) if t == 1 else x.repeat(1, tmax // t, 1, 1))
        return torch.cat(parts, dim=-1)

    def forward_stages(self, x):
        (ffinfo,), (views, stage_out) = run_parallel(
            [lambda: (self.faf.forward_frame(x, 1),), lambda: self.layers(self.tokenize(x))], [(x,), (x,)])
        return views, [[v.unsqueeze(1) for v in stage] for stage in stage_out], ffinfo

    def forward_global(self, views, dense=True):
        b = views[0].shape[0]
        t = max(self.input_token_temporal_dims)
        g = ops.merge_views(views, self.input_token_temporal_dims).reshape(b * 49, t, -1)
        g = ops.linear(g, self.globalembedding.weight, self.globalembedding.bias)
        if t < 3:
            raise RuntimeError("ThreeViewSwinTransformer: the encoder tail takes temporal slices 0,1,2 (mTVE:745): T >= 3")
        g = self.globalblocks(g, keep_t=3)
        tk = g.shape[1]
        g = g.reshape(b, 49, tk * 768)
        if tk == 3:
            return g
        if not dense:
            return g[:, :, :3 * 768]
        out = torch.empty(b, 49, 3 * 768, device=g.device, dtype=torch.float32)
        ops.copy_rows(g, tk * 768, out, 3 * 768, b * 49, 3 * 768)
        return out

    def forward(self, x):
        views, out_x, ffinfo = self.forward_stages(x)
        return self.forward_global(views), out_x, ffinfo
```

multilateral-temporal-view-pyramid-transformer-for-video-inpainting-detection_amd/models/modules/swinTransformer.py:

```python
import torch
import torch.nn as nn

from models.modules.layers import Derived, DropPath, refuse_stochastic_depth, to_2tuple, trunc_normal_
from mumpy_hip import ops


def window_partition(x, window_size):
    b, h, w, c = x.shape
    x = x.reshape(b, h // window_size, window_size, w // window_size, window_size, c)
    return x.permute(0, 1, 3, 2, 4, 5).reshape(-1, window_size, window_size, c)


def window_reverse(windows, window_size, H, W):
    H, W = int(H), int(W)
    b = windows.shape[0] // ((H // window_size) * (W // window_size))
    x = windows.reshape(b, H // window_size, W // window_size, window_size, window_size, -1)
    return x.permute(0, 1, 3, 2, 4, 5).reshape(b, H, W, -1)


def build_shift_mask(hs, w, window_size, shift_size):
    region = torch.zeros(hs, w)
    cuts = (slice(0, -window_size), slice(-window_size, -shift_size), slice(-shift_size, None))
    k = 0
    for rs in cuts:
        for cs in cuts:
            region[rs, cs] = k
            k += 1
    ids = window_partition(region.view(1, hs, w, 1), window_size).reshape(-1, window_size * window_size)
    diff = ids[:, None, :] - ids[:, :, None]
    return torch.where(diff != 0, torch.full_like(diff, -100.0), torch.zeros_like(diff))


def relative_position_index(ws_h, ws_w):
    ys, xs = torch.meshgrid(torch.arange(ws_h), torch.arange(ws_w), indexing="ij")
    coords = torch.stack([ys.flatten(), xs.flatten()])
    rel = coords[:, :, None] - coords[:, None, :]
    return (rel[0] + ws_h - 1) * (2 * ws_w - 1) + (rel[1] + ws_w - 1)


def _w16(module, name):
    lin = getattr(module, name)
    cache = module.__dict__.setdefault("_w16_cache", {})
    d = cache.get(name)
    if d is None:
        d = cache[name] = Derived()
    return d.get((lin.weight,), lambda: lin.weight.detach().to(torch.bfloat16).contiguous())


class Mlp(nn.Module):
    def __init__(self, in_features, hidden_features=None, out_features=None, act_layer=nn.GELU, drop=0.0):
        super().__init__()
        if act_layer is not nn.GELU:
            raise NotImplementedError("the GEMM epilogue implements exact-erf GELU only")
        self.fc1 = nn.Linear(in_features, hidden_features or in_features)
        self.act = act_layer()
        self.fc2 = nn.Linear(hidden_features or in_features, out_features or in_features)
        self.drop = nn.Dropout(drop)

    def forward(self, x, residual=None, emit_stats=False):
        h = ops.linear(x, self.fc1.weight, self.fc1.bias, act=ops.ACT_GELU)
        return ops.linear(h, self.fc2.weight, self.fc2.bias, residual=residual, emit_stats=emit_stats)

    def forward_ln(self, x, stats, norm, emit_stats=False):
        d = self.__dict__.setdefault("_ln_fold", Derived())
        wg, cs, bp = d.get((self.fc1.weight, self.fc1.bias, norm.weight, norm.bias),
                           lambda: ops.fold_ln_weights(self.fc1.weight, self.fc1.bias, norm.weight, norm.bias))
        h = ops.linear_ln(x, stats, wg, cs, bp, norm.eps, act=ops.ACT_GELU)
        return ops.linear(h, self.fc2.weight, self.fc2.bias, residual=x, emit_stats=emit_stats)

    def forward_bf16(self, x16, residual):
        w1, w2 = _w16(self, "fc1"), _w16(self, "fc2")
        h = ops.linear_bf16s(x16, w1, self.fc1.bias, act=ops.ACT_GELU, out_bf16=True)
        return ops.linear_bf16s(h, w2, self.fc2.bias, residual=residual, out_bf16=False)


class WindowAttention(nn.Module):
    def __init__(self, dim, window_size, num_heads, qkv_bias=True, qk_scale=None, attn_drop=0.0, proj_drop=0.0):
        super().__init__()
        self.dim, self.window_size, self.num_heads = dim, tuple(window_size), num_heads
        if self.window_size != (7, 7) or dim // num_heads != 32:
            raise NotImplementedError("HIP window attention is built for 7x7 windows and 32-wide heads "
                                      f"(got window {self.window_size}, head width {dim // num_heads})")
        self.scale = qk_scale or (dim // num_heads) ** -0.5
        self.relative_position_bias_table = nn.Parameter(torch.zeros(13 * 13, num_heads))
        self.register_buffer("relative_position_index", relative_position_index(7, 7))
        self.qkv = nn.Linear(dim, dim * 3, bias=qkv_bias)
        self.attn_drop = nn.Dropout(attn_drop)
        self.proj = nn.Linear(dim, dim)
        self.proj_drop = nn.Dropout(proj_drop)
        trunc_normal_(self.relative_position_bias_table, std=0.02)
        self._bias = Derived()
        self._mask = Derived()

    def padded_bias(self):
        return self._bias.get((self.relative_position_bias_table, self.relative_position_index),
                              lambda: ops.expand_relpos_bias(self.relative_position_bias_table,
                                                             self.relative_position_index))

    def mask_pack(self, mask):
        if mask is None:
            return None, None
        return self._mask.get((mask,), lambda: ops.compact_attn_mask(mask))

    def attend(self, x_normed, b, hs, w, shift, mask):
        tab, ids = self.mask_pack(mask)
        if x_normed.dtype == torch.bfloat16:
            qkv = ops.linear_bf16s(x_normed, _w16(self, "qkv"), self.qkv.bias, out_bf16=True)
            return ops.window_attention_bf16(qkv, self.padded_bias(), b, hs, w, self.dim, shift, self.scale, tab, ids)
        qkv = ops.linear(x_normed, self.qkv.weight, self.qkv.bias)
        return ops.window_attention(qkv, self.padded_bias(), b, hs, w, self.dim, shift, self.scale, tab, ids)

    def attend_ln(self, x, stats, norm, b, hs, w, shift, mask):
        tab, ids = self.mask_pack(mask)
        d = self.__dict__.setdefault("_ln_fold", Derived())
        wg, cs, bp = d.get((self.qkv.weight, self.qkv.bias, norm.weight, norm.bias),
                           lambda: ops.fold_ln_weights(self.qkv.weight, self.qkv.bias, norm.weight, norm.bias))
        qkv = ops.linear_ln(x, stats, wg, cs, bp, norm.eps)
        return ops.window_attention(qkv, self.padded_bias(), b, hs, w, self.dim, shift, self.scale, tab, ids)

    def forward(self, x, mask=None):
        b_ = x.shape[0]
        a = self.attend(x, b_, 7, 7, 0, mask)
        return ops.linear(a, self.proj.weight, self.proj.bias)

    def extra_repr(self):
        return f"dim={self.dim}, window_size={self.window_size}, num_heads={self.num_heads}"


class SwinTransformerBlock(nn.Module):
    def __init__(self, dim, input_resolution, num_heads, window_size=7, shift_size=0, mlp_ratio=4.0, qkv_bias=True,
                 qk_scale=None, drop=0.0, attn_drop=0.0, drop_path=0.0, act_layer=nn.GELU, norm_layer=nn.LayerNorm,
                 temporal_dim=1, fused_window_process=False):
        super().__init__()
        self.dim, self.input_resolution, self.num_heads = dim, tuple(input_resolution), num_heads
        self.window_size, self.shift_size, self.mlp_ratio, self.temporal_dim = window_size, shift_size, mlp_ratio, temporal_dim
        if min(self.input_resolution) <= self.window_size:
            self.shift_size = 0
            self.window_size = min(self.input_resolution)
        assert 0 <= self.shift_size < self.window_size, "shift_size must in 0-window_size"
        self.norm1 = norm_layer(dim)
        self.attn = WindowAttention(dim, to_2tuple(self.window_size), num_heads, qkv_bias, qk_scale, attn_drop, drop)
        self.drop_path = DropPath(drop_path) if drop_path > 0.0 else nn.Identity()
        self.norm2 = norm_layer(dim)
        self.mlp = Mlp(dim, int(dim * mlp_ratio), act_layer=act_layer, drop=drop)
        mask = None
        if self.shift_size > 0:
            h, w = self.input_resolution
            mask = build_shift_mask(h * temporal_dim, w, self.window_size, self.shift_size)
        self.register_buffer("attn_mask", mask)

    def forward(self, x):
        h, w = self.input_resolution
        b, l, c = x.shape
        assert l % (h * w) == 0, "input feature has wrong size"
        hs = l // w
        if self.training:
            refuse_stochastic_depth(self)
        if ops.storage() == "bf16":
            a = self.attn.attend(ops.layernorm_bf16(x, self.norm1.weight, self.norm1.bias, self.norm1.eps), b, hs, w,
                                 self.shift_size, self.attn_mask)
            x = ops.linear_bf16s(a, _w16(self.attn, "proj"), self.attn.proj.bias, residual=x, out_bf16=False)
            return self.mlp.forward_bf16(ops.layernorm_bf16(x, self.norm2.weight, self.norm2.bias, self.norm2.eps), x)
        m = b * l
        st = ops.ln_stats_of(x)
        fold1 = st is not None and ops.linear_ln_tiles(m, 3 * c, c) > 0
        fold2 = ops.linear_ln_tiles(m, c, c) > 0 and ops.linear_ln_tiles(m, self.mlp.fc1.out_features, c) > 0
        if fold1:
            a = self.attn.attend_ln(x, st, self.norm1, b, hs, w, self.shift_size, self.attn_mask)
        else:
            a = self.attn.attend(ops.layernorm(x, self.norm1.weight, self.norm1.bias, self.norm1.eps), b, hs, w,
                                 self.shift_size, self.attn_mask)
        x = ops.linear(a, self.attn.proj.weight, self.attn.proj.bias, residual=x, emit_stats=fold2)
        st = ops.ln_stats_of(x)
        emit = ops.linear_ln_tiles(m, c, self.mlp.fc2.in_features) > 0 and ops.linear_ln_tiles(m, 3 * c, c) > 0
        if st is not None:
            return self.mlp.forward_ln(x, st, self.norm2, emit_stats=emit)
        return self.mlp(ops.layernorm(x, self.norm2.weight, self.norm2.bias, self.norm2.eps), residual=x, emit_stats=emit)

    def extra_repr(self):
        return (f"dim={self.dim}, input_resolution={self.input_resolution}, num_heads={self.num_heads}, "
                f"window_size={self.window_size}, shift_size={self.shift_size}, temporal_dim={self.temporal_dim}")


class PatchMerging(nn.Module):
    def __init__(self, input_resolution, dim, norm_layer=nn.LayerNorm):
        super().__init__()
        self.input_resolution, self.dim = tuple(input_resolution), dim
        self.reduction = nn.Linear(4 * dim, 2 * dim, bias=False)
        self.norm = norm_layer(4 * dim)

    def forward(self, x):
        h, w = self.input_resolution
        b, l, c = x.shape
        assert l == h * w, "input feature has wrong size"
        assert h % 2 == 0 and w % 2 == 0, f"x size ({h}*{w}) are not even."
        g = ops.patch_merge_ln(x, self.norm.weight, self.norm.bias, b, h, w, c, self.norm.eps)
        return ops.linear(g, self.reduction.weight)

    def extra_repr(self):
        return f"input_resolution={self.input_resolution}, dim={self.dim}"


class ThreeViewPatchMerging(nn.Module):
    def __init__(self, view_configs, cur_stage):
        super().__init__()
        for v in range(3):
            side = view_configs[v]["input_resolution"][cur_stage][0]
            merge = PatchMerging((view_configs[v]["temporal_dim"] * side, side), view_configs[v]["hidden_size"][cur_stage])
            setattr(self, f"downsample{v + 1}", merge)

    def forward(self, x):
        return [self.downsample1(x[0]), self.downsample2(x[1]), self.downsample3(x[2])]


class BaselineTokenize(nn.Module):

    def __init__(self, view_configs):
        super().__init__()
        size = view_configs["patches"].size
        self.patch_size = size[0]
        self.patches_resolution = view_configs["input_resolution"][0]
        self.num_patches = self.patches_resolution[0] * self.patches_resolution[1]
        k = (size[-1], size[0], size[1])
        self.proj = nn.Conv3d(3, view_configs["hidden_size"][0], kernel_size=k, stride=k, padding=0)
        self.norm = nn.LayerNorm(view_configs["hidden_size"][0])
        self._wt = Derived()

    def forward(self, x):
        w = self.proj.weight
        wt = self._wt.get((w,), lambda: w.reshape(w.shape[0], -1).t().contiguous())
        y = ops.patch_embed(x, wt, self.proj.bias, self.norm.weight, self.norm.bias, w.shape[2], self.norm.eps)
        if y.shape[1] != self.num_patches:
            raise RuntimeError("BaselineTokenize expects the tubelet to span the whole clip (squeeze(-3), swin:29)")
        return y


class BasicLayer(nn.Module):
    def __init__(self, dim, input_resolution, depth, num_heads, window_size, mlp_ratio=4.0, qkv_bias=True, qk_scale=None,
                 drop=0.0, attn_drop=0.0, drop_path=0.0, norm_layer=nn.LayerNorm, downsample=None, use_checkpoint=False,
                 fused_window_process=False):
        super().__init__()
        self.dim, self.input_resolution, self.depth = dim, input_resolution, depth
        self.blocks = nn.ModuleList([
            SwinTransformerBlock(dim, input_resolution, num_heads, window_size, 0 if i % 2 == 0 else window_size // 2,
                                 mlp_ratio, qkv_bias, qk_scale, drop, attn_drop,
                                 drop_path[i] if isinstance(drop_path, list) else drop_path, norm_layer=norm_layer)
            for i in range(depth)])
        self.downsample = downsample(input_resolution, dim=dim, norm_layer=norm_layer) if downsample is not None else None

    def forward(self, x):
        for blk in self.blocks:
            x = blk(x)
        return self.downsample(x) if self.downsample is not None else x


class SwinTransformer(nn.Module):

    def __init__(self, view_configs, img_size=224, patch_size=4, in_chans=3, num_classes=1000, embed_dim=96,
                 depths=[2, 2, 6, 2], num_heads=[3, 6, 12, 24], window_size=7, mlp_ratio=4.0, qkv_bias=True, qk_scale=None,
                 drop_rate=0.0, attn_drop_rate=0.0, drop_path_rate=0.1, norm_layer=nn.LayerNorm, ape=False,
                 patch_norm=True, use_checkpoint=False, fused_window_process=False, **kwargs):
        super().__init__()
        if ape:
            raise NotImplementedError("absolute position embedding is off in every reference config")
        self.num_classes, self.num_layers, self.embed_dim = num_classes, len(depths), embed_dim
        self.num_features = int(embed_dim * 2 ** (self.num_layers - 1))
        self.patch_embed = BaselineTokenize(view_configs)
        self.patches_resolution = res = self.patch_embed.patches_resolution
        self.pos_drop = nn.Dropout(p=drop_rate)
        dpr = torch.linspace(0, drop_path_rate, sum(depths)).tolist()
        self.layers = nn.ModuleList()
        for i in range(self.num_layers):
            self.layers.append(BasicLayer(int(embed_dim * 2 ** i), (res[0] // 2 ** i, res[1] // 2 ** i), depths[i],
                                          num_heads[i], window_size, mlp_ratio, qkv_bias, qk_scale, drop_rate,
                                          attn_drop_rate, dpr[sum(depths[:i]):sum(depths[:i + 1])], norm_layer,
                                          PatchMerging if i < self.num_layers - 1 else None))
        self.norm = norm_layer(self.num_features)
        self.avgpool = nn.AdaptiveAvgPool1d(1)
        self.head = nn.Linear(self.num_features, num_classes) if num_classes > 0 else nn.Identity()
        self.apply(self._init_weights)

    @staticmethod
    def _init_weights(m):
        if isinstance(m, nn.Linear):
            trunc_normal_(m.weight, std=0.02)
            if m.bias is not None:
                nn.init.zeros_(m.bias)
        elif isinstance(m, nn.LayerNorm):
            nn.init.zeros_(m.bias)
            nn.init.ones_(m.weight)

    def forward_features(self, x):
        x = self.patch_embed(x)
        for layer in self.layers:
            x = layer(x)
        return ops.layernorm(x, self.norm.weight, self.norm.bias, self.norm.eps)

    def forward(self, x):
        x = self.forward_features(x)
        if isinstance(self.head, nn.Linear):
            x = ops.linear(x, self.head.weight, self.head.bias)
        return x
```

multilateral-temporal-view-pyramid-transformer-for-video-inpainting-detection_amd/mumpy_hip/lib.py:

```python
import ctypes
import os
import subprocess

_HERE = os.path.dirname(os.path.abspath(__file__))
_PKG = os.path.dirname(_HERE)
_LIB = None

c_f = ctypes.c_void_p
c_i = ctypes.c_int
c_l = ctypes.c_int64
c_fl = ctypes.c_float
c_d = ctypes.c_double

SIGNATURES = {
    "mumpy_layernorm_fwd": [c_f, c_f, c_f, c_f, c_l, c_i, c_fl, c_f],
    "mumpy_layernorm_bf16_fwd": [c_f, c_f, c_f, c_f, c_l, c_i, c_fl, c_f],
    "mumpy_linear_fwd": [c_f, c_f, c_f, c_f, c_f, c_l, c_i, c_i, c_i, c_f],
    "mumpy_linear_bf16s_fwd": [c_f, c_f, c_f, c_f, c_f, c_l, c_i, c_i, c_i, c_i, c_f],
    "mumpy_window_attention_bf16_fwd": [c_f, c_f, c_f, c_f, c_f, c_i, c_i, c_i, c_i, c_i, c_i, c_fl, c_f],
    "mumpy_window_attention_bf16mm_fwd": [c_f, c_f, c_f, c_f, c_f, c_i, c_i, c_i, c_i, c_i, c_i, c_fl, c_f],
    "mumpy_linear_ws_fwd": [c_f, c_f, c_f, c_f, c_f, c_l, c_i, c_i, c_i, c_f, c_l, c_f],
    "mumpy_linear_wsz_fwd": [c_f, c_f, c_f, c_f, c_f, c_l, c_i, c_i, c_i, c_f, c_l, c_f],
    "mumpy_linear_rd_fwd": [c_f, c_f, c_f, c_f, c_f, c_l, c_i, c_i, c_i, c_f],
    "mumpy_window_attention_bg_fwd": [c_f, c_f, c_f, c_f, c_f, c_i, c_i, c_i, c_i, c_i, c_i, c_fl, c_f],
    "mumpy_linear_workspace_bytes": [c_l, c_i, c_i],
    "mumpy_tuning_build": [],
    "mumpy_workspace_status": [c_f, ctypes.POINTER(ctypes.c_int)],
    "mumpy_linear_ln_tiles": [c_l, c_i, c_i],
    "mumpy_linear_lnx_fwd": [c_f, c_f, c_f, c_f, c_f, c_l, c_i, c_i, c_i, c_f, c_l, c_f, c_f, c_i, c_f, c_fl, c_f],
    "mumpy_linear_rows_fwd": [c_f, c_l, c_l, c_f, c_f, c_f, c_f, c_l, c_i, c_i, c_i, c_f, c_l, c_f],
    "mumpy_linear_rows_kseg_fwd": [c_f, c_l, c_l, c_i, c_i, c_f, c_f, c_f, c_f, c_l, c_i, c_i, c_i, c_f, c_l, c_f],
    "mumpy_gn_stats_nhwc_fwd": [c_f, c_f, c_i, c_l, c_i, c_i, c_i, c_f],
    "mumpy_gn_apply_resample_nhwc_fwd": [c_f, c_f, c_i, c_f, c_f, c_i, c_fl, c_i, c_i, c_i, c_i, c_i, c_f, c_f, c_f, c_i, c_i,
                                         c_i, c_i, c_i, c_i, c_f],
    "mumpy_conv2d_nhwc_fwd": [c_f, c_f, c_f, c_f, c_f, c_i, c_i, c_i, c_i, c_i, c_i, c_i, c_i, c_f, c_l, c_f],
    "mumpy_conv2d_workspace_bytes": [c_i, c_i, c_i, c_i, c_i, c_i, c_i],
    "mumpy_avgpool2_pad_nhwc_fwd": [c_f, c_f, c_i, c_i, c_i, c_i, c_i, c_i, c_f],
    "mumpy_copy_rows_fwd": [c_f, c_l, c_f, c_l, c_l, c_i, c_f],
    "mumpy_merge_views_fwd": [c_f, c_f, c_f, c_f, c_i, c_i, c_i, c_i, c_i, c_i, c_i, c_i, c_i, c_f],
    "mumpy_trunk_head_fwd": [c_f, c_f, c_f, c_f, c_f, c_i, c_i, c_i, c_i, c_f],
    "mumpy_final_conv_fwd": [c_f, c_f, c_f, c_f, c_f, c_i, c_i, c_i, c_i, c_fl, c_f],
    "mumpy_window_attention_fwd": [c_f, c_f, c_f, c_f, c_f, c_i, c_i, c_i, c_i, c_i, c_i, c_fl, c_f],
    "mumpy_deform_offsets_fwd": [c_f, c_f, c_f, c_f, c_f, c_f, c_f, c_i, c_i, c_i, c_i, c_f],
    "mumpy_deform_sample_fwd": [c_f, c_f, c_f, c_i, c_i, c_i, c_i, c_i, c_f],
    "mumpy_deform_attention_fwd": [c_f, c_f, c_f, c_f, c_i, c_i, c_i, c_i, c_i, c_fl, c_f],
    "mumpy_deform_sample_kv_fwd": [c_f, c_f, c_f, c_f, c_f, c_i, c_i, c_i, c_i, c_i, c_f],
    "mumpy_deform_out_combine_fwd": [c_f, c_f, c_f, c_f, c_f, c_i, c_i, c_i, c_i, c_f],
    "mumpy_deform_attention_mm16_fwd": [c_f, c_f, c_f, c_f, c_i, c_i, c_i, c_i, c_i, c_fl, c_f],
    "mumpy_deform_sample_kv_mm16_fwd": [c_f, c_f, c_f, c_f, c_f, c_i, c_i, c_i, c_i, c_i, c_f],
    "mumpy_deform_out_combine_mm16_fwd": [c_f, c_f, c_f, c_f, c_f, c_i, c_i, c_i, c_i, c_f],
    "mumpy_deform_combine_fwd": [c_f, c_f, c_f, c_i, c_i, c_i, c_i, c_f],
    "mumpy_faf_fwd": [c_f, c_f, c_f, c_f, c_f, c_i, c_i, c_i, c_i, c_i, c_i, c_f],
    "mumpy_patch_embed_fwd": [c_f, c_f, c_f, c_f, c_f, c_f, c_i, c_i, c_i, c_i, c_i, c_i, c_fl, c_f],
    "mumpy_patch_merge_ln_fwd": [c_f, c_f, c_f, c_f, c_i, c_i, c_i, c_i, c_fl, c_f],
    "mumpy_temporal_attention_fwd": [c_f, c_f, c_l, c_i, c_i, c_i, c_fl, c_f],
    "mumpy_attention_probs_fwd": [c_f, c_f, c_f, c_l, c_i, c_i, c_i, c_i, c_l, c_l, c_l, c_l, c_l, c_fl, c_f],
    "mumpy_temporal_attention_q_fwd": [c_f, c_f, c_l, c_i, c_i, c_i, c_i, c_fl, c_f],
    "mumpy_sigmoid_threshold_fwd": [c_f, c_f, c_l, c_fl, c_f],
    "mumpy_add_fwd": [c_f, c_f, c_f, c_l, c_f],
    "mumpy_normalize_u8_fwd": [c_f, c_f, c_l, c_i, c_i, ctypes.POINTER(ctypes.c_float), ctypes.POINTER(ctypes.c_float), c_f],
    "mumpy_resize_nearest_table": [c_i, c_i, ctypes.POINTER(ctypes.c_int32)],
    "mumpy_resize_normalize_u8_fwd": [c_f, c_f, c_f, c_f, c_l, c_i, c_i, c_i, c_i, ctypes.POINTER(ctypes.c_float), ctypes.POINTER(ctypes.c_float), c_f],
    "mumpy_mask_loss_workspace_bytes": [c_i, c_l],
    "mumpy_mask_loss_fwd_bwd": [c_f, c_f, c_f, c_f, c_f, c_l, c_i, c_l, c_fl, c_fl, c_f],
    "mumpy_layernorm_bwd_workspace_bytes": [c_l, c_i],
    "mumpy_layernorm_bwd": [c_f, c_f, c_f, c_f, c_f, c_f, c_f, c_f, c_l, c_l, c_i, c_fl, c_i, c_f],
    "mumpy_gelu_fwd": [c_f, c_f, c_l, c_f],
    "mumpy_gelu_bwd": [c_f, c_f, c_f, c_l, c_f],
    "mumpy_transpose_fwd": [c_f, c_f, c_l, c_l, c_f],
    "mumpy_col_sum_workspace_bytes": [c_l, c_i],
    "mumpy_col_sum_fwd": [c_f, c_f, c_f, c_l, c_l, c_i, c_f],
    "mumpy_final_conv_bwd_workspace_bytes": [c_i, c_i, c_i],
    "mumpy_final_conv_bwd": [c_f, c_f, c_f, c_f, c_f, c_f, c_f, c_l, c_i, c_i, c_i, c_i, c_f],
    "mumpy_patch_gather_fwd": [c_f, c_f, c_l, c_i, c_i, c_i, c_i, c_f],
    "mumpy_conv_weight_dgrad_fwd": [c_f, c_f, c_i, c_i, c_i, c_i, c_f],
    "mumpy_conv2d_wgrad_workspace_bytes": [c_i, c_i, c_i, c_i, c_i, c_i, c_i],
    "mumpy_conv2d_wgrad_nhwc": [c_f, c_f, c_f, c_i, c_i, c_i, c_i, c_i, c_i, c_i, c_i, c_f, c_l, c_f],
    "mumpy_linear_bwd_workspace_bytes": [c_l, c_i, c_i],
    "mumpy_linear_bwd": [c_f, c_f, c_f, c_f, c_f, c_f, c_l, c_i, c_i, c_i, c_f, c_l, c_f],
    "mumpy_window_attention_bwd_workspace_bytes": [c_i, c_i, c_i, c_i],
    "mumpy_window_attention_bwd": [c_f, c_f, c_f, c_f, c_f, c_i, c_f, c_f, c_f, c_f, c_l, c_i, c_i, c_i, c_i, c_i, c_fl, c_i, c_f],
    "mumpy_window_attention_bwd_csr": [c_f, c_f, c_f, c_f, c_f, c_i, c_f, c_f, c_f, c_f, c_f, c_l, c_i, c_i, c_i, c_i, c_i, c_fl, c_i, c_f],
    "mumpy_window_attention_mm16_fwd": [c_f, c_f, c_f, c_f, c_f, c_i, c_i, c_i, c_i, c_i, c_i, c_fl, c_f],
    "mumpy_window_attention_mm16_bwd_workspace_bytes": [c_i, c_i, c_i, c_i],
    "mumpy_window_attention_mm16_bwd": [c_f, c_f, c_f, c_f, c_f, c_i, c_f, c_f, c_f, c_f, c_f, c_l, c_i, c_i, c_i, c_i, c_i, c_fl, c_i, c_f],
    "mumpy_relpos_bias_expand_fwd": [c_f, c_f, c_f, c_i, c_f],
    "mumpy_gn_bwd_workspace_bytes": [c_i, c_l, c_i],
    "mumpy_gn_bwd_nhwc": [c_f, c_f, c_i, c_f, c_f, c_f, c_f, c_f, c_f, c_f, c_l, c_i, c_l, c_i, c_i, c_fl, c_i, c_f],
    "mumpy_upsample_bwd_nhwc": [c_f, c_f, c_i, c_i, c_i, c_i, c_i, c_i, c_f],
    "mumpy_temporal_attention_bwd": [c_f, c_f, c_f, c_l, c_i, c_i, c_i, c_fl, c_f],
    "mumpy_scale_samples_fwd": [c_f, c_f, c_f, c_i, c_l, c_f],
    "mumpy_dwconv5_window_fwd": [c_f, c_f, c_f, c_f, c_l, c_i, c_f],
    "mumpy_dwconv5_window_bwd_workspace_bytes": [c_l, c_i],
    "mumpy_dwconv5_window_bwd": [c_f, c_f, c_f, c_f, c_f, c_f, c_f, c_l, c_l, c_i, c_f],
    "mumpy_deform_attention_bwd_workspace_bytes": [c_l, c_i],
    "mumpy_deform_attention_bwd": [c_f, c_f, c_f, c_f, c_f, c_f, c_l, c_l, c_i, c_i, c_fl, c_f],
    "mumpy_deform_sample_bwd": [c_f, c_f, c_f, c_f, c_f, c_l, c_i, c_i, c_f],
    "mumpy_adamw_hyper": [ctypes.POINTER(ctypes.c_float), c_d, c_d, c_d, c_d, c_d, c_i, c_d],
    "mumpy_adamw_step_dev": [c_f, c_f, c_f, c_f, c_l, c_f, c_f],
    "mumpy_adamw_step": [c_f, c_f, c_f, c_f, c_l, c_d, c_d, c_d, c_d, c_d, c_i, c_d, c_f],
    "mumpy_sgd_step": [c_f, c_f, c_f, c_l, c_d, c_d, c_d, c_d, c_i, c_d, c_f],
    "mumpy_sgd_hyper": [ctypes.POINTER(ctypes.c_float), c_d, c_d, c_d, c_d, c_i, c_d],
    "mumpy_sgd_step_dev": [c_f, c_f, c_f, c_l, c_f, c_i, c_f],
    "mumpy_rmsprop_step": [c_f, c_f, c_f, c_f, c_l, c_d, c_d, c_d, c_d, c_d, c_d, c_f],
    "mumpy_rmsprop_hyper": [ctypes.POINTER(ctypes.c_float), c_d, c_d, c_d, c_d, c_d, c_d],
    "mumpy_rmsprop_step_dev": [c_f, c_f, c_f, c_f, c_l, c_f, c_f],
}
ABI_VERSION = 2


def library_path() -> str:
    if "MUMPY_HIP_LIB" in os.environ:
        return os.environ["MUMPY_HIP_LIB"]
    name = "libmumpy_hip_tuning.so" if os.environ.get("MUMPY_TUNING", "0") == "1" else "libmumpy_hip.so"
    return os.path.join(_PKG, "lib", name)


def tuning_library_path() -> str:
    return os.path.join(_PKG, "lib", "libmumpy_hip_tuning.so")


def build_library(verbose: bool = False) -> str:
    r = subprocess.run(["make", "-C", os.path.join(_PKG, "csrc"), "-j8", "all", "tuning"], capture_output=True, text=True)
    if verbose or r.returncode:
        print(r.stdout[-4000:], r.stderr[-4000:])
    if r.returncode:
        raise RuntimeError("building libmumpy_hip.so failed (see output above)")
    return library_path()


def load_library():
    global _LIB
    if _LIB is not None:
        return _LIB
    path = library_path()
    if not os.path.exists(path):
        raise RuntimeError(
            f"libmumpy_hip.so not found at {path}: the HIP kernels are the only implementation of this package "
            "(no CPU/torch fallback). Build it with `python __graft_entry__.py` or `make -C <pkg>/csrc`.")
    lib = ctypes.CDLL(path)
    lib.mumpy_abi_version.restype = c_i
    lib.mumpy_last_error.restype = ctypes.c_char_p
    lib.mumpy_last_route.restype = ctypes.c_char_p
    lib.mumpy_last_route.argtypes = []
    if lib.mumpy_abi_version() != ABI_VERSION:
        raise RuntimeError(f"{path}: ABI version {lib.mumpy_abi_version()} != binding {ABI_VERSION}; rebuild")
    for name, args in SIGNATURES.items():
        fn = getattr(lib, name)
        fn.argtypes = args
        fn.restype = c_l if name.endswith("_bytes") else c_i
    _LIB = lib
    return lib
```

multilateral-temporal-view-pyramid-transformer-for-video-inpainting-detection_amd/mumpy_hip/ops.py:

```python
import math
import os
from typing import Optional

import torch

from .lib import load_library

ACT_NONE, ACT_GELU = 0, 1
MATH_FP32, MATH_BF16, MATH_BF16X3, MATH_BF16X2 = 0, 0x100, 0x200, 0x400
_MATH = MATH_FP32
_WS_BYTES = {}


def set_matrix_math(mode: str) -> None:
    global _MATH
    if mode not in _MODES:
        raise ValueError(f"unknown matrix math mode {mode!r}")
    _MATH = _MODES[mode]


_MODES = {"fp32": MATH_FP32, "bf16": MATH_BF16, "bf16x3": MATH_BF16X3, "bf16x2": MATH_BF16X2}


def matrix_math() -> str:
    return {v: k for k, v in _MODES.items()}[_MATH]


_STORAGE = "fp32"


def set_storage(mode: str) -> None:
    global _STORAGE
    if mode not in ("fp32", "bf16"):
        raise ValueError(f"unknown storage mode {mode!r}")
    _STORAGE = mode
    set_matrix_math("bf16" if mode == "bf16" else "fp32")


def storage() -> str:
    return _STORAGE


NEG = -1e30


def _lib():
    return load_library()


def _chk(t: torch.Tensor, name: str) -> torch.Tensor:
    if not t.is_cuda:
        raise RuntimeError(f"mumpy_hip: {name} is on {t.device}; the HIP kernels need a GPU tensor (there is no CPU path)")
    if t.dtype != torch.float32:
        raise RuntimeError(f"mumpy_hip: {name} must be float32, got {t.dtype}")
    return t if t.is_contiguous() else t.contiguous()


def _p(t: Optional[torch.Tensor]):
    return None if t is None else t.data_ptr()


def _stream():
    return torch.cuda.current_stream().cuda_stream


PROFILE = None


def _call(name, *args, work=0.0):
    lib = _lib()
    if PROFILE is not None:
        e0, e1 = torch.cuda.Event(enable_timing=True), torch.cuda.Event(enable_timing=True)
        e0.record()
        rc = getattr(lib, name)(*args)
        e1.record()
        PROFILE.setdefault(name, []).append((e0, e1, work))
    else:
        rc = getattr(lib, name)(*args)
    if rc != 0:
        raise RuntimeError(f"{name} failed (rc={rc}): {lib.mumpy_last_error().decode()}")


def _opt(t: Optional[torch.Tensor], name: str) -> Optional[torch.Tensor]:
    return None if t is None else _chk(t, name)


def _ws_bytes(key, fn_name, *args):
    wsb = _WS_BYTES.get(key)
    if wsb is None:
        wsb = _WS_BYTES[key] = int(getattr(_lib(), fn_name)(*args))
    return wsb


def _chk16(t: torch.Tensor, name: str) -> torch.Tensor:
    if not t.is_cuda or t.dtype != torch.bfloat16:
        raise RuntimeError(f"mumpy_hip: {name} must be a bfloat16 GPU tensor, got {t.dtype} on {t.device}")
    return t if t.is_contiguous() else t.contiguous()


def layernorm_bf16(x, gamma, beta, eps=1e-5):
    x = _chk(x, "x")
    c = x.shape[-1]
    out = torch.empty(x.shape, device=x.device, dtype=torch.bfloat16)
    _call("mumpy_layernorm_bf16_fwd", _p(x), _p(_chk(gamma, "gamma")), _p(_chk(beta, "beta")), _p(out), x.numel() // c, c, eps,
          _stream(), work=6.0 * x.numel())
    return out


def linear_bf16s(x16, w16, bias=None, act=ACT_NONE, residual=None, out_bf16=True):
    x16, w16 = _chk16(x16, "x"), _chk16(w16, "weight")
    n, k = w16.shape[0], w16.numel() // w16.shape[0]
    if x16.shape[-1] != k:
        raise RuntimeError(f"linear_bf16s: x has {x16.shape[-1]} features, weight expects {k}")
    m = x16.numel() // k
    out = torch.empty(*x16.shape[:-1], n, device=x16.device, dtype=torch.bfloat16 if out_bf16 else torch.float32)
    if residual is not None:
        residual = _chk(residual, "residual")
        if residual.numel() != m * n or out_bf16:
            raise RuntimeError("linear_bf16s: the residual is fp32 and needs an fp32 output of the same shape")
    _call("mumpy_linear_bf16s_fwd", _p(x16), _p(w16), _p(_opt(bias, "bias")), _p(residual), _p(out),
          m, n, k, act, 1 if out_bf16 else 0, _stream(), work=2.0 * m * n * k)
    return out


def _attn_math_from_env() -> str:
    mode = os.environ.get("MUMPY_ATTN_MATH", "") or "fp32"
    if mode not in ("fp32", "bf16"):
        raise ValueError(f"MUMPY_ATTN_MATH: unknown attention math mode {mode!r}")
    return mode


_ATTN_MATH = _attn_math_from_env()


def set_attention_math(mode: str) -> None:
    global _ATTN_MATH
    if mode not in ("fp32", "bf16"):
        raise ValueError(f"unknown attention math mode {mode!r}")
    _ATTN_MATH = mode


def attention_math() -> str:
    return _ATTN_MATH


def _cva_math_from_env() -> str:
    mode = os.environ.get("MUMPY_CVA_MATH", "") or "fp32"
    if mode not in ("fp32", "bf16"):
        raise ValueError(f"MUMPY_CVA_MATH: unknown cross-view attention math mode {mode!r}")
    return mode


_CVA_MATH = _cva_math_from_env()


def set_cva_math(mode: str) -> None:
    global _CVA_MATH
    if mode not in ("fp32", "bf16"):
        raise ValueError(f"unknown cross-view attention math mode {mode!r}")
    _CVA_MATH = mode


def cva_math() -> str:
    return _CVA_MATH


def _mm16(entry, math):
    if math not in ("fp32", "bf16"):
        raise ValueError(f"unknown cross-view attention math mode {math!r}")
    return entry.replace("_fwd", "_mm16_fwd") if math == "bf16" else entry


def _window_attention(entry, chk, dtype, who, qkv, bias_pad, b, hs, w, c, shift, scale, mask_tab, mask_id, out=None):
    qkv = chk(qkv, "qkv")
    if qkv.numel() != b * hs * w * 3 * c:
        raise RuntimeError(f"{who}: qkv shape mismatch")
    out = torch.empty(b, hs * w, c, device=qkv.device, dtype=dtype) if out is None else out
    n_mask = 0 if mask_id is None else mask_id.numel()
    _call(entry, _p(qkv), _p(out), _p(_chk(bias_pad, "bias")), _p(mask_tab), _p(mask_id), n_mask,
          b, hs, w, c, shift, scale, _stream(), work=307328.0 * b * (hs // 7) * (w // 7) * (c // 32))
    return out


def window_attention_bf16(qkv16, bias_pad, b, hs, w, c, shift, scale, mask_tab=None, mask_id=None, math=None):
    if math is None:
        math = _ATTN_MATH
    elif math not in ("fp32", "bf16"):
        raise ValueError(f"unknown attention math mode {math!r}")
    return _window_attention("mumpy_window_attention_bf16mm_fwd" if math == "bf16" else "mumpy_window_attention_bf16_fwd", _chk16,
                             torch.bfloat16, "window_attention_bf16", qkv16, bias_pad, b, hs, w, c, shift, scale, mask_tab, mask_id)


def layernorm(x, gamma, beta, eps=1e-5, out=None):
    x = _chk(x, "x")
    c = x.shape[-1]
    out = torch.empty_like(x) if out is None else out
    _call("mumpy_layernorm_fwd", _p(x), _p(_chk(gamma, "gamma")), _p(_chk(beta, "beta")), _p(out), x.numel() // c, c,
          eps, _stream(), work=8.0 * x.numel())
    return out


def linear(x, weight, bias=None, act=ACT_NONE, residual=None, out=None, emit_stats=False):
    x = _chk(x, "x")
    weight = _chk(weight, "weight")
    n, k = weight.shape[0], weight.numel() // weight.shape[0]
    if x.shape[-1] != k:
        raise RuntimeError(f"linear: x has {x.shape[-1]} features, weight expects {k}")
    m = x.numel() // k
    if out is None:
        out = torch.empty(*x.shape[:-1], n, device=x.device, dtype=torch.float32)
    if residual is not None:
        residual = _chk(residual, "residual")
        if residual.numel() != m * n:
            raise RuntimeError("linear: residual shape mismatch")
    if _in_background():
        _call("mumpy_linear_rd_fwd", _p(x), _p(weight), _p(_opt(bias, "bias")), _p(residual), _p(out), m, n, k,
              act, _stream(), work=2.0 * m * n * k)
        return out
    wsb = _ws_bytes((m, n, k), "mumpy_linear_workspace_bytes", m, n, k)
    if emit_stats:
        gn = linear_ln_tiles(m, n, k) if k >= LN_FOLD_MIN_K else 0
        if gn:
            stats = torch.empty(m, gn, 2, device=x.device, dtype=torch.float32)
            ws = _kept_workspace(max(wsb, 4096), x.device)
            _call("mumpy_linear_lnx_fwd", _p(x), _p(weight), _p(_opt(bias, "bias")), _p(residual), _p(out), m, n, k,
                  act, _p(ws), ws.numel() * 4, _p(stats), None, 0, None, 0.0, _stream(), work=2.0 * m * n * k)
            out._mumpy_ln_stats = stats
            return out
    ws = _kept_workspace(wsb, x.device) if wsb else None
    _call("mumpy_linear_wsz_fwd", _p(x), _p(weight), _p(_opt(bias, "bias")), _p(residual),
          _p(out), m, n, k, act | _MATH, _p(ws), 0 if ws is None else ws.numel() * 4, _stream(), work=2.0 * m * n * k)
    return out


_BACKGROUND = [0]
BACKGROUND_ON = os.environ.get("MUMPY_BACKGROUND", "0") == "1"


class background:

    def __enter__(self):
        _BACKGROUND[0] += 1
        return self

    def __exit__(self, *exc):
        _BACKGROUND[0] -= 1
        return False


def _in_background():
    return _BACKGROUND[0] > 0 and BACKGROUND_ON and _MATH == MATH_FP32 and _STORAGE == "fp32"


LN_FOLD = os.environ.get("MUMPY_LN_FOLD", "1") != "0"
LN_FOLD_MIN_K = 512
_LN_TILES = {}


def linear_ln_tiles(m, n, k):
    if not LN_FOLD or _MATH != MATH_FP32 or _STORAGE != "fp32":
        return 0
    key = (m, n, k)
    t = _LN_TILES.get(key)
    if t is None:
        t = _LN_TILES[key] = int(_lib().mumpy_linear_ln_tiles(m, n, k))
    return t


def ln_stats_of(x):
    return getattr(x, "_mumpy_ln_stats", None)


def linear_ln(x, stats, wg, colsum, bprime, eps, act=ACT_NONE):
    x, wg = _chk(x, "x"), _chk(wg, "wg")
    n, k = wg.shape
    m = x.numel() // k
    out = torch.empty(*x.shape[:-1], n, device=x.device, dtype=torch.float32)
    wsb = _ws_bytes((m, n, k), "mumpy_linear_workspace_bytes", m, n, k)
    ws = _kept_workspace(max(wsb, 4096), x.device)
    _call("mumpy_linear_lnx_fwd", _p(x), _p(wg), _p(_chk(bprime, "bprime")), None, _p(out), m, n, k, act, _p(ws), ws.numel() * 4, None,
          _p(_chk(stats, "stats")), stats.shape[-2], _p(_chk(colsum, "colsum")), eps, _stream(), work=2.0 * m * n * k)
    return out


def fold_ln_weights(weight, bias, gamma, beta):
    w64 = weight.detach().double()
    wg = w64 * gamma.detach().double()[None, :]
    bp = w64 @ beta.detach().double()
    if bias is not None:
        bp = bp + bias.detach().double()
    return wg.float().contiguous(), wg.sum(1).float().contiguous(), bp.float().contiguous()


_KEPT_WS = {}
_RETIRED_WS = []


def _kept_workspace(nbytes, device):
    s = torch.cuda.current_stream(device)
    key = (str(device), s.cuda_stream)
    ws = _KEPT_WS.get(key)
    if ws is None or ws.numel() * 4 < nbytes:
        if torch.cuda.is_current_stream_capturing():
            return torch.zeros(nbytes // 4, device=device, dtype=torch.float32)
        if ws is not None:
            _RETIRED_WS.append(ws)
        ws = _KEPT_WS[key] = torch.zeros(max(nbytes // 4, 1024), device=device, dtype=torch.float32)
    return ws


def check_workspaces():
    import ctypes
    bad = []
    for key, ws in list(_KEPT_WS.items()):
        st = ctypes.c_int(0)
        rc = _lib().mumpy_workspace_status(ws.data_ptr(), ctypes.byref(st))
        if rc:
            raise RuntimeError(f"mumpy_workspace_status failed (rc={rc}): {_lib().mumpy_last_error().decode()}")
        if st.value == -1:
            global LN_FOLD
            LN_FOLD = False
            ws.view(torch.int32)[1022] = 0
            import warnings
            warnings.warn("mumpy_hip: a folded LayerNorm met a row with |mean| > 256 sigma; LayerNorm folding is now off "
                          "(ops.LN_FOLD = False) -- re-capture any hipGraph to apply it")
        elif st.value:
            bad.append((key, st.value))
    if bad:
        reset_workspaces()
        raise RuntimeError(f"mumpy_hip: split GEMM launch(es) timed out waiting for a partial tile {bad}; results since the last "
                           "check are invalid (workspaces re-zeroed)")


def reset_workspaces():
    for ws in list(_KEPT_WS.values()) + _RETIRED_WS:
        ws.zero_()


def linear_rows(x_view, weight, bias=None, residual=None, out=None):
    if not x_view.is_cuda or x_view.dtype != torch.float32:
        raise RuntimeError("mumpy_hip: linear_rows needs a float32 GPU tensor (there is no CPU path)")
    nblk, rows, k = x_view.shape
    if x_view.stride(2) != 1 or x_view.stride(1) != k:
        raise RuntimeError("linear_rows: rows of a block must be contiguous")
    weight = _chk(weight, "weight")
    n = weight.shape[0]
    m = nblk * rows
    if out is None:
        out = torch.empty(m, n, device=x_view.device, dtype=torch.float32)
    wsb = _ws_bytes((m, n, k), "mumpy_linear_workspace_bytes", m, n, k)
    ws = torch.empty(wsb // 4, device=x_view.device, dtype=torch.float32) if wsb else None
    _call("mumpy_linear_rows_fwd", x_view.data_ptr(), rows, x_view.stride(0), _p(weight),
          _p(_opt(bias, "bias")), _p(residual), _p(out), m, n, k, ACT_NONE | _MATH, _p(ws), wsb, _stream(),
          work=2.0 * m * n * k)
    return out


def linear_time_slices(x4, weight, bias=None, residual=None):
    x4, weight = _chk(x4, "x"), _chk(weight, "weight")
    b, t, n, c = x4.shape
    nout, k = weight.shape
    if k != t * c or c % 32:
        raise RuntimeError(f"linear_time_slices: weight expects K = T*C = {t * c} (got {k}); C % 32 == 0")
    m = b * n
    out = torch.empty(m, nout, device=x4.device, dtype=torch.float32)
    if residual is not None:
        residual = _chk(residual, "residual")
    wsb = _ws_bytes((m, nout, k), "mumpy_linear_workspace_bytes", m, nout, k)
    ws = torch.empty(wsb // 4, device=x4.device, dtype=torch.float32) if wsb else None
    _call("mumpy_linear_rows_kseg_fwd", _p(x4), n, t * n * c, c, n * c, _p(weight), _p(_opt(bias, "bias")),
          _p(residual), _p(out), m, nout, k, ACT_NONE | _MATH, _p(ws), wsb, _stream(), work=2.0 * m * nout * k)
    return out


def conv2d_nhwc(x, w_krsc, bias=None, act=ACT_NONE, residual=None):
    x = _nhwc(x, "x")
    b, cin, h, w = x.shape
    w_krsc = _chk(w_krsc, "weight")
    cout, kh, kw, cin2 = w_krsc.shape
    if cin2 != cin:
        raise RuntimeError(f"conv2d: input has {cin} channels, weight expects {cin2}")
    out = empty_nhwc(b, cout, h, w, x.device)
    if residual is not None:
        residual = _nhwc(residual, "residual")
    wsb = _ws_bytes(("conv", b, h, w, cin, cout, kh, kw), "mumpy_conv2d_workspace_bytes", b, h, w, cin, cout, kh, kw)
    ws = torch.empty(wsb // 4, device=x.device, dtype=torch.float32) if wsb else None
    _call("mumpy_conv2d_nhwc_fwd", _p(x), _p(w_krsc), _p(_opt(bias, "bias")), _p(residual), _p(out),
          b, h, w, cin, cout, kh, kw, act | _MATH, _p(ws), wsb, _stream(), work=2.0 * b * h * w * cout * kh * kw * cin)
    return out


def final_conv(x, w_krsc, bias, with_mask=False, thr=0.5):
    x = _nhwc(x, "x")
    b, c, h, w = x.shape
    if c % 32 or tuple(w_krsc.shape) != (1, 3, 3, c):
        raise RuntimeError(f"final_conv is built for Conv2d(32k, 1, 3, padding=1); got C={c}, weight {tuple(w_krsc.shape)}")
    logits = torch.empty(b, 1, h, w, device=x.device, dtype=torch.float32)
    mask = torch.empty(b, 1, h, w, device=x.device, dtype=torch.uint8) if with_mask else None
    _call("mumpy_final_conv_fwd", _p(x), _p(_chk(w_krsc, "weight")), _p(_chk(bias, "bias")), _p(logits), _p(mask), b, h, w, c, thr,
          _stream(), work=4.0 * (x.numel() + logits.numel()))
    return (logits, mask) if with_mask else logits


def _nhwc(t: torch.Tensor, name: str) -> torch.Tensor:
    if not t.is_cuda:
        raise RuntimeError(f"mumpy_hip: {name} is on {t.device}; the HIP kernels need a GPU tensor (there is no CPU path)")
    if t.dtype != torch.float32 or t.dim() != 4:
        raise RuntimeError(f"mumpy_hip: {name} must be a 4-D float32 tensor")
    b, c, h, w = t.shape
    if t.stride() != (h * w * c, 1, w * c, c):
        t = t.contiguous(memory_format=torch.channels_last)
        if t.stride() != (h * w * c, 1, w * c, c):
            t = t.permute(0, 2, 3, 1).contiguous().permute(0, 3, 1, 2)
    return t


def empty_nhwc(b, c, h, w, device):
    return torch.empty(b, h, w, c, device=device, dtype=torch.float32).permute(0, 3, 1, 2)


ACT_RELU, ACT_SIGMOID = 1, 2
EP_NONE, EP_ADD_MUL, EP_MUL = 0, 1, 2


def gn_stats(x, groups):
    x = _nhwc(x, "x")
    b, c, h, w = x.shape
    nsplit = max(1, min(256, (h * w * c) // 16384))
    partial = torch.empty(b, nsplit, groups, 2, device=x.device, dtype=torch.float32)
    _call("mumpy_gn_stats_nhwc_fwd", _p(x), _p(partial), b, h * w, c, groups, nsplit, _stream(), work=4.0 * x.numel())
    return x, partial, nsplit


def gn_apply_resample(x, gn=None, act=0, mean4=False, scale=1, align_corners=False, ep_mode=0, ep_a=None, ep_b=None,
                      out=None, out_coff=0):
    x = _nhwc(x, "x")
    b, c, h, w = x.shape
    cout = c // 4 if mean4 else c
    ho, wo = h * scale, w * scale
    if out is None:
        out = empty_nhwc(b, cout, ho, wo, x.device)
    else:
        assert out.shape[0] == b and out.shape[2] == ho and out.shape[3] == wo and out.stride(1) == 1
    if ep_a is not None:
        ep_a = _nhwc(ep_a, "ep_a")
        assert tuple(ep_a.shape) == (b, cout, ho, wo), "epilogue operand shape"
    if ep_b is not None:
        ep_b = _nhwc(ep_b, "ep_b")
        assert tuple(ep_b.shape) == (b, cout, ho, wo), "epilogue operand shape"
    partial, nsplit, gamma, beta, groups, eps = gn if gn is not None else (None, 0, None, None, 1, 0.0)
    _call("mumpy_gn_apply_resample_nhwc_fwd", _p(x), _p(partial), nsplit, _p(gamma), _p(beta), groups, eps, act,
          1 if mean4 else 0, scale, 1 if align_corners else 0, ep_mode, _p(ep_a), _p(ep_b), _p(out), out.shape[1], out_coff,
          b, h, w, c, _stream(), work=4.0 * (x.numel() + b * cout * ho * wo))
    return out


def avgpool2_pad(x, cpad=None, nchw_in=False):
    if nchw_in:
        x = _chk(x, "x")
    else:
        x = _nhwc(x, "x")
    b, c, h, w = x.shape
    cpad = c if cpad is None else cpad
    out = empty_nhwc(b, cpad, h // 2, w // 2, x.device)
    _call("mumpy_avgpool2_pad_nhwc_fwd", _p(x), _p(out), b, h, w, c, cpad, 1 if nchw_in else 0, _stream(),
          work=4.0 * (x.numel() + out.numel()))
    return out


def copy_rows(src, src_stride, dst, dst_stride, rows, cols):
    if not (src.is_cuda and dst.is_cuda and src.dtype == dst.dtype == torch.float32):
        raise RuntimeError("mumpy_hip: copy_rows needs float32 GPU tensors (there is no CPU path)")
    _call("mumpy_copy_rows_fwd", src.data_ptr(), src_stride, dst.data_ptr(), dst_stride, rows, cols, _stream(), work=8.0 * rows * cols)
    return dst


def set_channels(dst, coff, src):
    b, c, h, w = src.shape
    ctot = dst.shape[1]
    if dst.stride() != (h * w * ctot, 1, w * ctot, ctot) or tuple(dst.shape[2:]) != (h, w) or dst.shape[0] != b:
        raise RuntimeError("set_channels: dst must be a dense NHWC map of the same batch and size")
    pitch = src.stride(3)
    if src.stride(1) != 1 or src.stride(2) != w * pitch or (b > 1 and src.stride(0) != h * w * pitch) or pitch < c:
        src = _nhwc(src, "src")
        pitch = c
    return copy_rows(src, pitch, dst[:, coff:], ctot, b * h * w, c)


def merge_views(views, token_t, n=49):
    v = [_chk(t, "view") for t in views]
    b = v[0].shape[0]
    tmax = max(token_t)
    out = torch.empty(b * n * tmax, sum(t.shape[2] for t in v), device=v[0].device, dtype=torch.float32)
    _call("mumpy_merge_views_fwd", _p(v[0]), _p(v[1]), _p(v[2]), _p(out), b, tmax, n, v[0].shape[2], v[1].shape[2], v[2].shape[2],
          token_t[0], token_t[1], token_t[2], _stream(), work=8.0 * out.numel())
    return out


def trunk_head(g, f, gcn, freq):
    g, f, gcn, freq = _nhwc(g, "g"), _nhwc(f, "f"), _nhwc(gcn, "gcn"), _nhwc(freq, "freq")
    b, c4, h, w = g.shape
    c = c4 // 4
    if f.shape != g.shape or tuple(gcn.shape) != (b, c, 2 * h, 2 * w) or freq.shape != gcn.shape:
        raise RuntimeError("trunk_head: shape mismatch")
    z = empty_nhwc(b, c, 2 * h, 2 * w, g.device)
    _call("mumpy_trunk_head_fwd", _p(g), _p(f), _p(gcn), _p(freq), _p(z), b, h, w, c, _stream(), work=4.0 * (2 * g.numel() + 3 * z.numel()))
    return z


def add(a, b, out=None):
    a, b = _chk(a, "a"), _chk(b, "b")
    out = torch.empty_like(a) if out is None else out
    _call("mumpy_add_fwd", _p(a), _p(b), _p(out), a.numel(), _stream())
    return out


def rel_index32(index: torch.Tensor) -> torch.Tensor:
    t = getattr(index, "_mumpy_i32", None)
    if t is None or t.device != index.device or getattr(index, "_mumpy_i32_version", -1) != index._version:
        t = index.to(torch.int32).reshape(-1).contiguous()
        index._mumpy_i32, index._mumpy_i32_version = t, index._version
    return t


def expand_relpos_bias(table: torch.Tensor, index: torch.Tensor) -> torch.Tensor:
    table = _chk(table, "table")
    nh = table.shape[1]
    if not index.is_cuda:
        index = index.to(table.device)
    idx = index if index.dtype == torch.int32 and index.dim() == 1 else rel_index32(index)
    out = torch.empty(nh, 64, 64, device=table.device, dtype=torch.float32)
    _call("mumpy_relpos_bias_expand_fwd", _p(table), _p(idx), _p(out), nh, _stream())
    return out


_PAD_MASK = {}


def pad_mask(device=None) -> torch.Tensor:
    if device is None:
        m = torch.zeros(1, 64, 64, dtype=torch.float32)
        m[:, :, 49:] = NEG
        return m
    key = str(device)
    if key not in _PAD_MASK:
        _PAD_MASK[key] = pad_mask().to(device)
    return _PAD_MASK[key]


def compact_attn_mask(mask: torch.Tensor):
    m = mask.detach().float().cpu().reshape(mask.shape[0], -1)
    uniq, inv = torch.unique(m, dim=0, return_inverse=True)
    nz = [i for i in range(uniq.shape[0]) if bool((uniq[i] != 0).any())]
    remap = torch.full((uniq.shape[0],), -1, dtype=torch.int32)
    for j, i in enumerate(nz):
        remap[i] = j
    tab = torch.zeros(max(len(nz), 1), 64, 64)
    for j, i in enumerate(nz):
        tab[j, :49, :49] = uniq[i].reshape(49, 49)
    return tab.to(mask.device), remap[inv].to(torch.int32).to(mask.device)


def window_attention(qkv, bias_pad, b, hs, w, c, shift, scale, mask_tab=None, mask_id=None, out=None):
    return _window_attention("mumpy_window_attention_bg_fwd" if _in_background() else "mumpy_window_attention_fwd", _chk, torch.float32,
                             "window_attention", qkv, bias_pad, b, hs, w, c, shift, scale, mask_tab, mask_id, out)


def window_attention_mm16(qkv, bias_pad, b, hs, w, c, shift, scale, mask_tab=None, mask_id=None, out=None):
    return _window_attention("mumpy_window_attention_mm16_fwd", _chk, torch.float32, "window_attention_mm16", qkv, bias_pad, b, hs, w, c,
# ... 557 lines not shown
```

multilateral-temporal-view-pyramid-transformer-for-video-inpainting-detection_amd/mumpy_hip/streams.py:

```python
import os

import torch
import torch.distributed

_SIDE = {}
_DEPTH = [0]
SERIAL = os.environ.get("MUMPY_SERIAL", "0") == "1"


def new_distinct_stream(device, avoid=(), priority=0):
    taken = {int(h) for h in avoid} | {s.cuda_stream for s in _SIDE.values()}
    if priority == 0 and torch.distributed.is_available() and torch.distributed.is_initialized():
        priority = -1
    for _ in range(64):
        s = torch.cuda.Stream(device=device, priority=priority)
        if s.cuda_stream not in taken:
            return s
    raise RuntimeError("mumpy_hip.streams: torch's stream pool is exhausted (more than 32 concurrent side streams)")


def quiesce_collectives():
    torch.cuda.synchronize()
    if torch.distributed.is_available() and torch.distributed.is_initialized() and torch.distributed.get_backend() == "nccl":
        import time
        time.sleep(0.5)


def _side_stream(device, i, parent=None):
    key = (str(device), _DEPTH[0], i, None if parent is None else parent.cuda_stream)
    if key not in _SIDE:
        prio = int(os.environ.get("MUMPY_SIDE_PRIORITY", "0"))
        _SIDE[key] = new_distinct_stream(device, () if parent is None else (parent.cuda_stream,), prio)
    return _SIDE[key]


def _tensors(obj):
    if isinstance(obj, torch.Tensor):
        yield obj
    elif isinstance(obj, (list, tuple)):
        for o in obj:
            yield from _tensors(o)


def run_parallel(branches, inputs):
    if SERIAL or len(branches) == 1:
        return [fn() for fn in branches]
    main = torch.cuda.current_stream()
    if any(main.cuda_stream == s.cuda_stream for s in _SIDE.values()):
        return [fn() for fn in branches]
    fork = torch.cuda.Event()
    fork.record(main)
    outs = [None] * len(branches)
    sides = []
    for i in range(len(branches) - 1):
        sides.append(_side_stream(main.device, i, main))
    _DEPTH[0] += 1
    try:
        for i, fn in enumerate(branches[:-1]):
            s = sides[i]
            s.wait_event(fork)
            for t in _tensors(inputs[i]):
                t.record_stream(s)
            with torch.cuda.stream(s):
                outs[i] = fn()
        outs[-1] = branches[-1]()
    finally:
        _DEPTH[0] -= 1
    for i, s in enumerate(sides):
        main.wait_stream(s)
        for t in _tensors(outs[i]):
            t.record_stream(main)
    return outs
```

Before: 376.1 clips/s.

## Fuse next block's LayerNorm into split-K GEMM finish kernel

Adds a linear entry point that, when the GEMM uses split-K, reduces the partial slabs, applies bias/GELU/residual and also computes the following block's norm1 LayerNorm from registers in the same finish kernel. Model blocks pass the next block's norm so the next attention can reuse the precomputed normalized tensor instead of launching a separate LayerNorm pass over the activation. When split-K is not chosen it falls back to a separate LayerNorm call. This adds an extra output buffer and stream bookkeeping for the side tensor.

```diff
diff --git a/include/mumpy_hip.h b/include/mumpy_hip.h
--- a/include/mumpy_hip.h
+++ b/include/mumpy_hip.h
@@ -73,6 +73,10 @@
 
 int mumpy_linear_wsz_fwd(const float* x, const float* W, const float* bias, const float* residual, float* y,
                          int64_t M, int N, int K, int act, void* workspace, int64_t workspace_bytes, void* stream);
+
+int mumpy_linear_wsz_ln_fwd(const float* x, const float* W, const float* bias, const float* residual, float* y,
+                            int64_t M, int N, int K, int act, void* workspace, int64_t workspace_bytes,
+                            const float* ln_gamma, const float* ln_beta, float ln_eps, float* y_ln, void* stream);
 
 int mumpy_linear_bf16s_fwd(const void* x, const void* W, const float* bias, const float* residual, void* y,
                            int64_t M, int N, int K, int act, int out_bf16, void* stream);
diff --git a/multilateral-temporal-view-pyramid-transformer-for-video-inpainting-detection_amd/csrc/abi.cpp b/multilateral-temporal-view-pyramid-transformer-for-video-inpainting-detection_amd/csrc/abi.cpp
--- a/multilateral-temporal-view-pyramid-transformer-for-video-inpainting-detection_amd/csrc/abi.cpp
+++ b/multilateral-temporal-view-pyramid-transformer-for-video-inpainting-detection_amd/csrc/abi.cpp
@@ -20,7 +20,9 @@
     char* t = g_route_text;
     const size_t n = sizeof(g_route_text);
     switch (r.family) {
-    case Route::TILED: snprintf(t, n, "tiled tile=%d ks=%d np=%d addr=%s", r.tile, r.ks, r.np, addr[r.addr & 3]); break;
+    case Route::TILED:
+        snprintf(t, n, "tiled tile=%d ks=%d np=%d addr=%s%s", r.tile, r.ks, r.np, addr[r.addr & 3], r.finish_ln ? " finish=ln" : "");
+        break;
     case Route::TILED16: snprintf(t, n, "tiled16 tile=%d ks=%d np=%d addr=%s", r.tile, r.ks, r.np, addr[r.addr & 3]); break;
     case Route::WS:
         snprintf(t, n, "ws sched=%s P=%d ln=%s addr=%s", r.split ? "split" : "whole", r.passes, ln[r.ln < 3 ? r.ln : 0], addr[r.addr & 3]);
diff --git a/multilateral-temporal-view-pyramid-transformer-for-video-inpainting-detection_amd/csrc/common.h b/multilateral-temporal-view-pyramid-transformer-for-video-inpainting-detection_amd/csrc/common.h
--- a/multilateral-temporal-view-pyramid-transformer-for-video-inpainting-detection_amd/csrc/common.h
+++ b/multilateral-temporal-view-pyramid-transformer-for-video-inpainting-detection_amd/csrc/common.h
@@ -36,6 +36,7 @@
     uint8_t passes = 0;
     uint8_t ln = 0;
     uint8_t reduce = R_NONE;
+    uint8_t finish_ln = 0;
     int ks = 1;
     struct { int wt, ks; } prod[2] = {{0, 0}, {0, 0}};
 };
diff --git a/multilateral-temporal-view-pyramid-transformer-for-video-inpainting-detection_amd/csrc/gemm.hip b/multilateral-temporal-view-pyramid-transformer-for-video-inpainting-detection_amd/csrc/gemm.hip
--- a/multilateral-temporal-view-pyramid-transformer-for-video-inpainting-detection_amd/csrc/gemm.hip
+++ b/multilateral-temporal-view-pyramid-transformer-for-video-inpainting-detection_amd/csrc/gemm.hip
@@ -3,6 +3,7 @@
 #include "common.h"
 #include "gemm_ws.h"
 #include "gemm_ws64.h"
+#include "ln_rows.h"
 using namespace mumpy;
 
 namespace {
@@ -507,6 +508,62 @@
     }
 }
 
+template <int NV, int U>
+__global__ __launch_bounds__(256) void splitk_finish_ln_kernel(const float* __restrict__ slab, const float* __restrict__ bias,
+                                                               const float* residual, float* Y, int64_t rows, int N, int ksplit,
+                                                               int act, int lpr, int nv, const float* __restrict__ gamma,
+                                                               const float* __restrict__ beta, float eps, float* __restrict__ Yln) {
+    const int lane = threadIdx.x & 63;
+    const int wave = threadIdx.x >> 6;
+    const int rpw = 64 / lpr;
+    const int sub = lane / lpr, l = lane % lpr;
+    const int64_t row = ((int64_t)blockIdx.x * 4 + wave) * rpw + sub;
+    const bool live = row < rows;
+    const int n4 = N >> 2;
+    const int64_t MN4 = rows * n4, r4 = row * n4;
+    const f32x4* s4 = reinterpret_cast<const f32x4*>(slab);
+    f32x4 v[NV];
+    float s = 0.f;
+#pragma unroll
+    for (int i = 0; i < NV; ++i) v[i] = (live && i < nv) ? s4[r4 + l + i * lpr] : f32x4{0, 0, 0, 0};
+    if (live) {
+        for (int zb = 1; zb < ksplit; zb += U) {
+            f32x4 t[U][NV];
+#pragma unroll
+            for (int u = 0; u < U; ++u) {
+                if (zb + u < ksplit) {
+#pragma unroll
+                    for (int i = 0; i < NV; ++i)
+                        if (i < nv) t[u][i] = s4[(int64_t)(zb + u) * MN4 + r4 + l + i * lpr];
+                }
+            }
+#pragma unroll
+            for (int u = 0; u < U; ++u) {
+                if (zb + u < ksplit) {
+#pragma unroll
+                    for (int i = 0; i < NV; ++i)
+                        if (i < nv) v[i] += t[u][i];
+                }
+            }
+        }
+#pragma unroll
+        for (int i = 0; i < NV; ++i) {
+            if (i < nv) {
+                const int c4 = l + i * lpr;
+                if (bias) v[i] += *reinterpret_cast<const f32x4*>(bias + 4 * c4);
+                if (act == MUMPY_ACT_GELU) {
+#pragma unroll
+                    for (int e = 0; e < 4; ++e) v[i][e] = gelu_erf(v[i][e]);
+                }
+                if (residual) v[i] += reinterpret_cast<const f32x4*>(residual)[r4 + c4];
+                reinterpret_cast<f32x4*>(Y)[r4 + c4] = v[i];
+                s += ln_lane_sum(v[i]);
+            }
+        }
+    }
+    ln_row_from_regs<NV, false>(v, s, nv, lpr, l, live, row, N, gamma, beta, Yln, eps);
+}
+
 struct Plan {
     int tile;
     int ksplit;
@@ -602,6 +659,13 @@
     return how;
 }
 
+struct LnFinish {
+    const float *gamma, *beta;
+    float eps;
+    float* y_ln;
+    mutable bool done;
+};
+
 struct LinearArgs {
     const float *x, *W, *bias, *residual;
     float* y;
@@ -615,6 +679,7 @@
     int kseg = 0, kstride = 0;
     const ConvGeom* conv = nullptr;
     const gemm_ws::LnArgs* ln = nullptr;
+    const LnFinish* lnf = nullptr;
 };
 
 struct TiledArgs {
@@ -728,7 +793,21 @@
     else if (math_bf16) launch_tiled_bf16<1>(wide, conv != nullptr, t);
     else launch_tiled_fp32(p.tile, conv != nullptr, use_glds, t);
     MUMPY_CHECK_LAUNCH("linear");
-    if (p.ksplit > 1) {
+    int lpr = 0, nv = 0;
+    if (p.ksplit > 1 && a.lnf && pick_split(N, &lpr, &nv)) {
+        const int rows_per_block = 4 * (64 / lpr);
+        const unsigned g = (unsigned)((M + rows_per_block - 1) / rows_per_block);
+        const LnFinish& f = *a.lnf;
+        if (nv <= 4)
+            hipLaunchKernelGGL((splitk_finish_ln_kernel<4, 8>), dim3(g), dim3(256), 0, a.s, ws, a.bias, a.residual, a.y, M, N, p.ksplit, act,
+                               lpr, nv, f.gamma, f.beta, f.eps, f.y_ln);
+        else
+            hipLaunchKernelGGL((splitk_finish_ln_kernel<LN_MAXNV, 2>), dim3(g), dim3(256), 0, a.s, ws, a.bias, a.residual, a.y, M, N, p.ksplit,
+                               act, lpr, nv, f.gamma, f.beta, f.eps, f.y_ln);
+        MUMPY_CHECK_LAUNCH("linear(split-K finish + LayerNorm)");
+        g_route.finish_ln = 1;
+        f.done = true;
+    } else if (p.ksplit > 1) {
         const int64_t mn4 = M * N / 4;
         int64_t g = (mn4 + 255) / 256;
         if (g > 2048) g = 2048;
@@ -839,6 +918,23 @@
     return launch_linear(a);
 }
 
+extern "C" int mumpy_linear_wsz_ln_fwd(const float* x, const float* W, const float* bias, const float* residual, float* y,
+                                       int64_t M, int N, int K, int act, void* workspace, int64_t workspace_bytes,
+                                       const float* ln_gamma, const float* ln_beta, float ln_eps, float* y_ln, void* stream) {
+    if (M == 0) return 0;
+    if (int rc = check_linear_args("linear_ln", x, W, residual, y, M, N, K, act)) return rc;
+    MUMPY_REQUIRE(aligned16(workspace), MUMPY_EALIGN, "linear_ln: workspace must be 16-byte aligned");
+    MUMPY_REQUIRE(ln_gamma && ln_beta && y_ln, MUMPY_ENULL, "linear_ln: null pointer");
+    MUMPY_REQUIRE(aligned16(ln_gamma) && aligned16(ln_beta) && aligned16(y_ln), MUMPY_EALIGN, "linear_ln: pointers must be 16-byte aligned");
+    MUMPY_REQUIRE(y_ln != y && y_ln != residual, MUMPY_EINVAL, "linear_ln: y_ln must not alias y or the residual");
+    const LnFinish f{ln_gamma, ln_beta, ln_eps, y_ln, false};
+    LinearArgs a = linear_args(x, W, bias, residual, y, M, N, K, act, workspace, workspace_bytes, stream);
+    a.ws_clean = true;
+    a.lnf = &f;
+    if (int rc = launch_linear(a)) return rc;
+    return f.done ? 0 : mumpy_layernorm_fwd(y, ln_gamma, ln_beta, y_ln, M, N, ln_eps, stream);
+}
+
 extern "C" int mumpy_workspace_status(const void* workspace, int* status) {
     MUMPY_REQUIRE(workspace && status, MUMPY_ENULL, "workspace_status: null pointer");
     unsigned w[2] = {0, 0};
diff --git a/multilateral-temporal-view-pyramid-transformer-for-video-inpainting-detection_amd/csrc/ln_rows.h b/multilateral-temporal-view-pyramid-transformer-for-video-inpainting-detection_amd/csrc/ln_rows.h
--- /dev/null
+++ b/multilateral-temporal-view-pyramid-transformer-for-video-inpainting-detection_amd/csrc/ln_rows.h
@@ -0,0 +1,56 @@
+#pragma once
+#include "common.h"
+
+namespace mumpy {
+
+constexpr int LN_MAXNV = 16;
+
+inline bool pick_split(int C, int* lpr, int* nv) {
+    if (C % 4 || C > 4096 || C < 4) return false;
+    const int n4 = C / 4;
+    int l = 64;
+    while (l > 1 && ((n4 % l) || n4 / l < 3)) l >>= 1;
+    if (n4 / l > LN_MAXNV) return false;
+    *lpr = l;
+    *nv = n4 / l;
+    return true;
+}
+
+__device__ __forceinline__ float ln_lane_sum(f32x4 v) { return (v.x + v.y) + (v.z + v.w); }
+
+template <int NV, bool OUT16>
+__device__ __forceinline__ void ln_row_from_regs(const f32x4 (&v)[NV], float s, int nv, int lpr, int l, bool live, int64_t row, int C,
+                                                 const float* __restrict__ gamma, const float* __restrict__ beta,
+                                                 float* __restrict__ y, float eps) {
+    s = wave_sum(s, lpr);
+    const float mean = s / (float)C;
+    float q = 0.f;
+#pragma unroll
+    for (int i = 0; i < NV; ++i) {
+        if (i < nv) {
+            f32x4 d = v[i] - mean;
+            q += (d.x * d.x + d.y * d.y) + (d.z * d.z + d.w * d.w);
+        }
+    }
+    q = wave_sum(q, lpr);
+    const float rstd = rsqrtf(q / (float)C + eps);
+    if (!live) return;
+    float* yr = y + row * (int64_t)C;
+#pragma unroll
+    for (int i = 0; i < NV; ++i) {
+        if (i < nv) {
+            const int c4 = l + i * lpr;
+            const f32x4 g = *reinterpret_cast<const f32x4*>(gamma + 4 * c4);
+            const f32x4 b = *reinterpret_cast<const f32x4*>(beta + 4 * c4);
+            const f32x4 o = (v[i] - mean) * rstd * g + b;
+            if (OUT16) {
+                typedef __bf16 bf16x4v __attribute__((ext_vector_type(4)));
+                *reinterpret_cast<bf16x4v*>(reinterpret_cast<__bf16*>(y) + row * (int64_t)C + 4 * c4) = __builtin_convertvector(o, bf16x4v);
+            } else {
+                *reinterpret_cast<f32x4*>(yr + 4 * c4) = o;
+            }
+        }
+    }
+}
+
+}
diff --git a/multilateral-temporal-view-pyramid-transformer-for-video-inpainting-detection_amd/csrc/norm.hip b/multilateral-temporal-view-pyramid-transformer-for-video-inpainting-detection_amd/csrc/norm.hip
--- a/multilateral-temporal-view-pyramid-transformer-for-video-inpainting-detection_amd/csrc/norm.hip
+++ b/multilateral-temporal-view-pyramid-transformer-for-video-inpainting-detection_amd/csrc/norm.hip
@@ -1,9 +1,8 @@
 #include "common.h"
+#include "ln_rows.h"
 using namespace mumpy;
 
 namespace {
-
-constexpr int MAXNV = 16;
 
 template <typename SRC, bool OUT16 = false>
 __global__ __launch_bounds__(256) void ln_rows_kernel(SRC src, const float* __restrict__ gamma,
@@ -15,44 +14,16 @@
     const int sub = lane / lpr, l = lane % lpr;
     const int64_t row = ((int64_t)blockIdx.x * 4 + wave) * rpw + sub;
     const bool live = row < rows;
-    f32x4 v[MAXNV];
+    f32x4 v[LN_MAXNV];
     float s = 0.f;
 #pragma unroll
-    for (int i = 0; i < MAXNV; ++i) {
+    for (int i = 0; i < LN_MAXNV; ++i) {
         if (i < nv) {
             v[i] = live ? *reinterpret_cast<const f32x4*>(src(row, l + i * lpr)) : f32x4{0, 0, 0, 0};
-            s += (v[i].x + v[i].y) + (v[i].z + v[i].w);
+            s += ln_lane_sum(v[i]);
         }
     }
-    s = wave_sum(s, lpr);
-    const float mean = s / (float)C;
-    float q = 0.f;
-#pragma unroll
-    for (int i = 0; i < MAXNV; ++i) {
-        if (i < nv) {
-            f32x4 d = v[i] - mean;
-            q += (d.x * d.x + d.y * d.y) + (d.z * d.z + d.w * d.w);
-        }
-    }
-    q = wave_sum(q, lpr);
-    const float rstd = rsqrtf(q / (float)C + eps);
-    if (!live) return;
-    float* yr = y + row * (int64_t)C;
-#pragma unroll
-    for (int i = 0; i < MAXNV; ++i) {
-        if (i < nv) {
-            const int c4 = l + i * lpr;
-            const f32x4 g = *reinterpret_cast<const f32x4*>(gamma + 4 * c4);
-            const f32x4 b = *reinterpret_cast<const f32x4*>(beta + 4 * c4);
-            const f32x4 o = (v[i] - mean) * rstd * g + b;
-            if (OUT16) {
-                typedef __bf16 bf16x4v __attribute__((ext_vector_type(4)));
-                *reinterpret_cast<bf16x4v*>(reinterpret_cast<__bf16*>(y) + row * (int64_t)C + 4 * c4) = __builtin_convertvector(o, bf16x4v);
-            } else {
-                *reinterpret_cast<f32x4*>(yr + 4 * c4) = o;
-            }
-        }
-    }
+    ln_row_from_regs<LN_MAXNV, OUT16>(v, s, nv, lpr, l, live, row, C, gamma, beta, y, eps);
 }
 
 struct PlainRows {
@@ -77,17 +48,6 @@
         return x + tok * C + c;
     }
 };
-
-bool pick_split(int C, int* lpr, int* nv) {
-    if (C % 4 || C > 4096 || C < 4) return false;
-    const int n4 = C / 4;
-    int l = 64;
-    while (l > 1 && ((n4 % l) || n4 / l < 3)) l >>= 1;
-    if (n4 / l > MAXNV) return false;
-    *lpr = l;
-    *nv = n4 / l;
-    return true;
-}
 
 }
 
diff --git a/multilateral-temporal-view-pyramid-transformer-for-video-inpainting-detection_amd/models/encoder/multiTemporalViewEncoder.py b/multilateral-temporal-view-pyramid-transformer-for-video-inpainting-detection_amd/models/encoder/multiTemporalViewEncoder.py
--- a/multilateral-temporal-view-pyramid-transformer-for-video-inpainting-detection_amd/models/encoder/multiTemporalViewEncoder.py
+++ b/multilateral-temporal-view-pyramid-transformer-for-video-inpainting-detection_amd/models/encoder/multiTemporalViewEncoder.py
@@ -60,7 +60,10 @@
             a = self.attn.attend(ops.layernorm_bf16(x1, self.norm1.weight, self.norm1.bias, self.norm1.eps), b, l1 // w, w, 0, None)
             out = ops.linear_bf16s(a, _w16(self.attn, "proj"), self.attn.proj.bias, out_bf16=False)
             return ops.add(x1, out), out
-        a = self.attn.attend(ops.layernorm(x1, self.norm1.weight, self.norm1.bias, self.norm1.eps), b, l1 // w, w, 0, None)
+        xn = ops.ln_next_of(x1, self.norm1)
+        if xn is None:
+            xn = ops.layernorm(x1, self.norm1.weight, self.norm1.bias, self.norm1.eps)
+        a = self.attn.attend(xn, b, l1 // w, w, 0, None)
         if not need_out:
             return ops.linear(a, self.attn.proj.weight, self.attn.proj.bias, residual=x1), None
         out = ops.linear(a, self.attn.proj.weight, self.attn.proj.bias)
@@ -73,7 +76,7 @@
         b, l1, _ = x1.shape
         return self.cva.crossattn._prep(x1, (b, l1 // w, w))
 
-    def tail(self, x1, x2, prep=None):
+    def tail(self, x1, x2, prep=None, next_norm=None):
         h, w = self.input_resolution
         b, l1, c1 = x1.shape
         hs1 = l1 // w
@@ -85,11 +88,12 @@
             return self.mlp.forward_bf16(ops.layernorm_bf16(x1, self.norm2.weight, self.norm2.bias, self.norm2.eps), x1)
         m = b * l1
         emit = ops.linear_ln_tiles(m, c1, self.mlp.fc2.in_features) > 0 and ops.linear_ln_tiles(m, 3 * c1, c1) > 0
-        return self.mlp(ops.layernorm(x1, self.norm2.weight, self.norm2.bias, self.norm2.eps), residual=x1, emit_stats=emit)
-
-    def forward(self, x1, x2):
+        return self.mlp(ops.layernorm(x1, self.norm2.weight, self.norm2.bias, self.norm2.eps), residual=x1, emit_stats=emit,
+                        ln_next=ops.norm_args(next_norm) if next_norm is not None else None)
+
+    def forward(self, x1, x2, next_norm=None):
         x1, out = self.msa(x1)
-        return self.tail(x1, x2), out
+        return self.tail(x1, x2, next_norm=next_norm), out
 
 
 class CrossThreeViewSwinBlock(nn.Module):
@@ -108,12 +112,12 @@
         self.block3 = CrossSwinBlock(hid[2], hid[2], input_resolution[2], heads[2], window_size=ws[2], last_view=True,
                                      temporal_dims=3, **kw)
 
-    def forward(self, x):
+    def forward(self, x, next_norms=(None, None, None)):
         from mumpy_hip import streams
         if streams.SERIAL:
-            x3, out3 = self.block3(x[2], x[2])
-            x2, out2 = self.block2(x[1], out3)
-            x1, _ = self.block1(x[0], out2)
+            x3, out3 = self.block3(x[2], x[2], next_norms[2])
+            x2, out2 = self.block2(x[1], out3, next_norms[1])
+            x1, _ = self.block1(x[0], out2, next_norms[0])
             return [x1, x2, x3]
         main = torch.cuda.current_stream()
         sa, sb = streams._side_stream(main.device, 0), streams._side_stream(main.device, 1)
@@ -131,7 +135,7 @@
                 prep2 = self.block2.prep(x2a)
                 sa.wait_event(e3)
                 out3.record_stream(sa)
-                x2 = self.block2.tail(x2a, out3, prep2)
+                x2 = self.block2.tail(x2a, out3, prep2, next_norms[1])
             sb.wait_event(fork)
             x[0].record_stream(sb)
             with torch.cuda.stream(sb):
@@ -139,14 +143,14 @@
                 prep1 = self.block1.prep(x1a)
                 sb.wait_event(e2)
                 out2.record_stream(sb)
-                x1 = self.block1.tail(x1a, out2, prep1)
-            x3 = self.block3.tail(x3a, None)
+                x1 = self.block1.tail(x1a, out2, prep1, next_norms[0])
+            x3 = self.block3.tail(x3a, None, next_norm=next_norms[2])
         finally:
             streams._DEPTH[0] -= 1
         main.wait_stream(sa)
         main.wait_stream(sb)
-        x2.record_stream(main)
-        x1.record_stream(main)
+        for t in streams._tensors((x1, x2)):
+            t.record_stream(main)
         return [x1, x2, x3]
 
 
@@ -184,23 +188,30 @@
         self.blocks = nn.ModuleList(blocks)
         self.downsample = downsample(view_configs, cur_stage) if downsample is not None else None
 
-    def _view_chain(self, v, x):
-        for blk in self.blocks[1:]:
-            x = getattr(blk, f"block{v + 1}")(x)
+    def _plain_blocks(self, v):
+        chain = [getattr(blk, f"block{v + 1}") for blk in self.blocks[1:]]
+        return [blk for blk in chain if not isinstance(blk, nn.Identity)]
+
+    def _view_chain(self, v, x, merge_norm=None):
+        chain = self._plain_blocks(v)
+        for i, blk in enumerate(chain):
+            x = blk(x, chain[i + 1].norm1 if i + 1 < len(chain) else None)
         out = x
         if self.downsample is not None:
-            x = getattr(self.downsample, f"downsample{v + 1}")(x)
+            x = getattr(self.downsample, f"downsample{v + 1}")(x, merge_norm)
         return x, out
 
-    def forward(self, x):
-        x = self.blocks[0](x)
+    def forward(self, x, merge_norms=(None, None, None)):
+        firsts = [self._plain_blocks(v) for v in range(3)]
+        x = self.blocks[0](x, [f[0].norm1 if f else None for f in firsts])
         def bg(v):
             from mumpy_hip import streams
             if streams.SERIAL:
-                return self._view_chain(v, x[v])
+                return self._view_chain(v, x[v], merge_norms[v])
             with ops.background():
-                return self._view_chain(v, x[v])
-        res = run_parallel([lambda: bg(0), lambda: bg(1), lambda: self._view_chain(2, x[2])], [(x[0],), (x[1],), (x[2],)])
+                return self._view_chain(v, x[v], merge_norms[v])
+        res = run_parallel([lambda: bg(0), lambda: bg(1), lambda: self._view_chain(2, x[2], merge_norms[2])],
+                           [(x[0],), (x[1],), (x[2],)])
         return [r[0] for r in res], [r[1] for r in res]
 
 
@@ -218,8 +229,9 @@
 
     def forward(self, x):
         outs = []
-        for layer in self.layers:
-            x, o = layer(x)
+        for i, layer in enumerate(self.layers):
+            nxt = self.layers[i + 1].blocks[0] if i + 1 < len(self.layers) else None
+            x, o = layer(x, [nxt.block1.norm1, nxt.block2.norm1, nxt.block3.norm1] if nxt is not None else (None, None, None))
             outs.append(o)
         return x, outs
 
diff --git a/multilateral-temporal-view-pyramid-transformer-for-video-inpainting-detection_amd/models/modules/swinTransformer.py b/multilateral-temporal-view-pyramid-transformer-for-video-inpainting-detection_amd/models/modules/swinTransformer.py
--- a/multilateral-temporal-view-pyramid-transformer-for-video-inpainting-detection_amd/models/modules/swinTransformer.py
+++ b/multilateral-temporal-view-pyramid-transformer-for-video-inpainting-detection_amd/models/modules/swinTransformer.py
@@ -57,16 +57,16 @@
         self.fc2 = nn.Linear(hidden_features or in_features, out_features or in_features)
         self.drop = nn.Dropout(drop)
 
-    def forward(self, x, residual=None, emit_stats=False):
+    def forward(self, x, residual=None, emit_stats=False, ln_next=None):
         h = ops.linear(x, self.fc1.weight, self.fc1.bias, act=ops.ACT_GELU)
-        return ops.linear(h, self.fc2.weight, self.fc2.bias, residual=residual, emit_stats=emit_stats)
-
-    def forward_ln(self, x, stats, norm, emit_stats=False):
+        return ops.linear(h, self.fc2.weight, self.fc2.bias, residual=residual, emit_stats=emit_stats, ln_next=ln_next)
+
+    def forward_ln(self, x, stats, norm, emit_stats=False, ln_next=None):
         d = self.__dict__.setdefault("_ln_fold", Derived())
         wg, cs, bp = d.get((self.fc1.weight, self.fc1.bias, norm.weight, norm.bias),
                            lambda: ops.fold_ln_weights(self.fc1.weight, self.fc1.bias, norm.weight, norm.bias))
         h = ops.linear_ln(x, stats, wg, cs, bp, norm.eps, act=ops.ACT_GELU)
-        return ops.linear(h, self.fc2.weight, self.fc2.bias, residual=x, emit_stats=emit_stats)
+        return ops.linear(h, self.fc2.weight, self.fc2.bias, residual=x, emit_stats=emit_stats, ln_next=ln_next)
 
     def forward_bf16(self, x16, residual):
         w1, w2 = _w16(self, "fc1"), _w16(self, "fc2")
@@ -149,7 +149,7 @@
             mask = build_shift_mask(h * temporal_dim, w, self.window_size, self.shift_size)
         self.register_buffer("attn_mask", mask)
 
-    def forward(self, x):
+    def forward(self, x, next_norm=None):
         h, w = self.input_resolution
         b, l, c = x.shape
         assert l % (h * w) == 0, "input feature has wrong size"
@@ -168,14 +168,18 @@
         if fold1:
             a = self.attn.attend_ln(x, st, self.norm1, b, hs, w, self.shift_size, self.attn_mask)
         else:
-            a = self.attn.attend(ops.layernorm(x, self.norm1.weight, self.norm1.bias, self.norm1.eps), b, hs, w,
-                                 self.shift_size, self.attn_mask)
+            xn = ops.ln_next_of(x, self.norm1)
+            if xn is None:
+                xn = ops.layernorm(x, self.norm1.weight, self.norm1.bias, self.norm1.eps)
+            a = self.attn.attend(xn, b, hs, w, self.shift_size, self.attn_mask)
         x = ops.linear(a, self.attn.proj.weight, self.attn.proj.bias, residual=x, emit_stats=fold2)
         st = ops.ln_stats_of(x)
         emit = ops.linear_ln_tiles(m, c, self.mlp.fc2.in_features) > 0 and ops.linear_ln_tiles(m, 3 * c, c) > 0
+        ln_next = ops.norm_args(next_norm) if next_norm is not None else None
         if st is not None:
-            return self.mlp.forward_ln(x, st, self.norm2, emit_stats=emit)
-        return self.mlp(ops.layernorm(x, self.norm2.weight, self.norm2.bias, self.norm2.eps), residual=x, emit_stats=emit)
+            return self.mlp.forward_ln(x, st, self.norm2, emit_stats=emit, ln_next=ln_next)
+        return self.mlp(ops.layernorm(x, self.norm2.weight, self.norm2.bias, self.norm2.eps), residual=x, emit_stats=emit,
+                        ln_next=ln_next)
 
     def extra_repr(self):
         return (f"dim={self.dim}, input_resolution={self.input_resolution}, num_heads={self.num_heads}, "
@@ -189,13 +193,13 @@
         self.reduction = nn.Linear(4 * dim, 2 * dim, bias=False)
         self.norm = norm_layer(4 * dim)
 
-    def forward(self, x):
+    def forward(self, x, next_norm=None):
         h, w = self.input_resolution
         b, l, c = x.shape
         assert l == h * w, "input feature has wrong size"
         assert h % 2 == 0 and w % 2 == 0, f"x size ({h}*{w}) are not even."
         g = ops.patch_merge_ln(x, self.norm.weight, self.norm.bias, b, h, w, c, self.norm.eps)
-        return ops.linear(g, self.reduction.weight)
+        return ops.linear(g, self.reduction.weight, ln_next=ops.norm_args(next_norm) if next_norm is not None else None)
 
     def extra_repr(self):
         return f"input_resolution={self.input_resolution}, dim={self.dim}"
@@ -249,8 +253,8 @@
         self.downsample = downsample(input_resolution, dim=dim, norm_layer=norm_layer) if downsample is not None else None
 
     def forward(self, x):
-        for blk in self.blocks:
-            x = blk(x)
+        for i, blk in enumerate(self.blocks):
+            x = blk(x, self.blocks[i + 1].norm1 if i + 1 < len(self.blocks) else None)
         return self.downsample(x) if self.downsample is not None else x
 
 
diff --git a/multilateral-temporal-view-pyramid-transformer-for-video-inpainting-detection_amd/mumpy_hip/lib.py b/multilateral-temporal-view-pyramid-transformer-for-video-inpainting-detection_amd/mumpy_hip/lib.py
--- a/multilateral-temporal-view-pyramid-transformer-for-video-inpainting-detection_amd/mumpy_hip/lib.py
+++ b/multilateral-temporal-view-pyramid-transformer-for-video-inpainting-detection_amd/mumpy_hip/lib.py
@@ -21,6 +21,7 @@
     "mumpy_window_attention_bf16mm_fwd": [c_f, c_f, c_f, c_f, c_f, c_i, c_i, c_i, c_i, c_i, c_i, c_fl, c_f],
     "mumpy_linear_ws_fwd": [c_f, c_f, c_f, c_f, c_f, c_l, c_i, c_i, c_i, c_f, c_l, c_f],
     "mumpy_linear_wsz_fwd": [c_f, c_f, c_f, c_f, c_f, c_l, c_i, c_i, c_i, c_f, c_l, c_f],
+    "mumpy_linear_wsz_ln_fwd": [c_f, c_f, c_f, c_f, c_f, c_l, c_i, c_i, c_i, c_f, c_l, c_f, c_f, c_fl, c_f, c_f],
     "mumpy_linear_rd_fwd": [c_f, c_f, c_f, c_f, c_f, c_l, c_i, c_i, c_i, c_f],
     "mumpy_window_attention_bg_fwd": [c_f, c_f, c_f, c_f, c_f, c_i, c_i, c_i, c_i, c_i, c_i, c_fl, c_f],
     "mumpy_linear_workspace_bytes": [c_l, c_i, c_i],
diff --git a/multilateral-temporal-view-pyramid-transformer-for-video-inpainting-detection_amd/mumpy_hip/ops.py b/multilateral-temporal-view-pyramid-transformer-for-video-inpainting-detection_amd/mumpy_hip/ops.py
--- a/multilateral-temporal-view-pyramid-transformer-for-video-inpainting-detection_amd/mumpy_hip/ops.py
+++ b/multilateral-temporal-view-pyramid-transformer-for-video-inpainting-detection_amd/mumpy_hip/ops.py
@@ -200,7 +200,7 @@
     return out
 
 
-def linear(x, weight, bias=None, act=ACT_NONE, residual=None, out=None, emit_stats=False):
+def linear(x, weight, bias=None, act=ACT_NONE, residual=None, out=None, emit_stats=False, ln_next=None):
     x = _chk(x, "x")
     weight = _chk(weight, "weight")
     n, k = weight.shape[0], weight.numel() // weight.shape[0]
@@ -228,6 +228,14 @@
             out._mumpy_ln_stats = stats
             return out
     ws = _kept_workspace(wsb, x.device) if wsb else None
+    if ln_next is not None and LN_FINISH and _STORAGE == "fp32":
+        gamma, beta, eps = ln_next
+        y_ln = torch.empty_like(out)
+        _call("mumpy_linear_wsz_ln_fwd", _p(x), _p(weight), _p(_opt(bias, "bias")), _p(residual), _p(out), m, n, k, act | _MATH,
+              _p(ws), 0 if ws is None else ws.numel() * 4, _p(_chk(gamma, "gamma")), _p(_chk(beta, "beta")), eps, _p(y_ln), _stream(),
+              work=2.0 * m * n * k)
+        out._mumpy_ln_next = (y_ln, gamma, beta)
+        return out
     _call("mumpy_linear_wsz_fwd", _p(x), _p(weight), _p(_opt(bias, "bias")), _p(residual),
           _p(out), m, n, k, act | _MATH, _p(ws), 0 if ws is None else ws.numel() * 4, _stream(), work=2.0 * m * n * k)
     return out
@@ -265,6 +273,20 @@
     if t is None:
         t = _LN_TILES[key] = int(_lib().mumpy_linear_ln_tiles(m, n, k))
     return t
+
+
+LN_FINISH = os.environ.get("MUMPY_LN_FINISH", "1") != "0"
+
+
+def ln_next_of(x, norm):
+    t = getattr(x, "_mumpy_ln_next", None)
+    if t is not None and t[1] is norm.weight and t[2] is norm.bias:
+        return t[0]
+    return None
+
+
+def norm_args(norm):
+    return (norm.weight, norm.bias, norm.eps)
 
 
 def ln_stats_of(x):
diff --git a/multilateral-temporal-view-pyramid-transformer-for-video-inpainting-detection_amd/mumpy_hip/streams.py b/multilateral-temporal-view-pyramid-transformer-for-video-inpainting-detection_amd/mumpy_hip/streams.py
--- a/multilateral-temporal-view-pyramid-transformer-for-video-inpainting-detection_amd/mumpy_hip/streams.py
+++ b/multilateral-temporal-view-pyramid-transformer-for-video-inpainting-detection_amd/mumpy_hip/streams.py
@@ -37,6 +37,9 @@
 def _tensors(obj):
     if isinstance(obj, torch.Tensor):
         yield obj
+        nxt = getattr(obj, "_mumpy_ln_next", None)
+        if nxt is not None:
+            yield nxt[0]
     elif isinstance(obj, (list, tuple)):
         for o in obj:
             yield from _tensors(o)
```

New measurement: 378.5 clips/s, median of 2. No clear change (+0.6%).
